# UltronAI/Depth-VO-Feat

Measured on AMD Instinct MI355X. Metric: KITTI 256x832 stereo-seq samples/sec fwd+bwd, higher is better.
Workload: dtype f32

## Files before the change

depth-vo-feat_amd/csrc/conv.hip:

```cpp
#include "dvf_common.h"
#include "conv_op.h"
#include "conv_pipe_host.h"
#include "conv_gather.h"
#include "conv_wgrad.h"
#include "wgrad_pipe.h"

namespace {

__device__ __forceinline__ float act_grad(float g, float yv, int act, float alpha, float beta) {
    if (act == DVF_ACT_RELU) return (yv > 0.f) ? g : 0.f;
    if (act == DVF_ACT_SIGMOID_AFFINE) {
        const float sg = (yv - beta) / alpha;
        return g * alpha * sg * (1.f - sg);
    }
    return g;
}

template <bool VEC>
__global__ __launch_bounds__(256) void act_bwd_kernel(const float *__restrict__ dy, const float *__restrict__ y,
                                                      float *__restrict__ dpre, float *dbias, int C, int HW, int act,
                                                      float alpha, float beta, int chunks, float *part = nullptr, int nper = 0) {
    __shared__ float red[4];
    const int plane = blockIdx.x / chunks, chunk = blockIdx.x - plane * chunks;
    const int c = plane % C;
// ... 117 lines not shown
    }
    return best;
}

struct GatherPlan {
    GatherArgs a;
    int MT, NT, CKH;
    size_t lds;
    dim3 grid;
    int64_t ws_floats;
    bool reduce_kpar;
};

int plan_gather(const ConvOp &op, GatherPlan &pl) {
    const ClassSpec *cls = op.cls;
    const int ncls = op.ncls, Tmax = op.Tmax, TAmax = op.TAmax, TBmax = op.TBmax, OHc = op.OHc, OWc = op.OWc;
    if (ncls < 1 || ncls > 4) return DVF_ERR_INVALID_ARG;
    GatherArgs &a = pl.a;
    a = GatherArgs{};
    for (int s = 0; s < op.nseg; ++s) a.segC[s] = op.segC[s];
    a.nseg = op.nseg; a.w_mode = op.w_mode;
    a.Mtot = op.Mtot; a.Rtot = op.Rtot; a.KK = op.KK; a.m_base = op.m_base; a.M = op.M;
    a.N = op.N; a.IH = op.IH; a.IW = op.IW; a.OH = op.OH; a.OW = op.OW;
    a.act = op.act; a.alpha = op.alpha; a.beta = op.beta;
    a.ncls = ncls; a.OS = cls[0].OS; a.IS = cls[0].IS;
    for (int i = 0, tap0 = 0; i < ncls; ++i) {
        const ClassSpec &c = cls[i];
        const int T = c.TA * c.TB;
        if (tap0 + T > 52) return DVF_ERR_INVALID_ARG;
        a.cls[i] = ClassDev{c.py, c.px, c.by, c.bx, c.TA, c.TB, c.OHc, c.OWc, tap0};
        for (int t = 0; t < T; ++t) a.tapmap[tap0 + t] = c.tapmap[t];
        tap0 += T;
    }
    const int maxBW = ((64 - 1) * cls[0].IS + TBmax > 128) ? 32 : 64;
    const int MT = a.M > 32 ? 2 : 1;
    int NT = 2;
    TilePlan tp = plan_tiles(OHc, OWc, NT, maxBW);
    int64_t nblk = (int64_t)cdiv(OWc, tp.TGX << tp.lsw) * cdiv(OHc, tp.TGY << tp.lsh) * cdiv(a.M, 32 * MT) * a.N * ncls;
    if (nblk < 768) {
        NT = 1;
        tp = plan_tiles(OHc, OWc, NT, maxBW);
        nblk = (int64_t)cdiv(OWc, tp.TGX << tp.lsw) * cdiv(OHc, tp.TGY << tp.lsh) * cdiv(a.M, 32 * MT) * a.N * ncls;
    }
    const int mtiles = cdiv(a.M, 32 * MT);
    a.lsw = tp.lsw; a.lsh = tp.lsh; a.TGX = tp.TGX;
    a.BW = tp.TGX << tp.lsw; a.BH = tp.TGY << tp.lsh;
    if ((a.BW - 1) * a.IS + TBmax > 128) return DVF_ERR_UNSUPPORTED;
    a.tilesX = cdiv(OWc, a.BW);
    a.tilesY = cdiv(OHc, a.BH);
    const int PH = (a.BH - 1) * a.IS + TAmax, PW = (a.BW - 1) * a.IS + TBmax, PWH = (PW + 1) / 2;
    a.PSmax = PH * ((a.IS == 2) ? 2 * PWH : PW);
    a.Tmax = Tmax;
    const int COTP = 32 * MT + 1;
    int maxc = 0;
    for (int s = 0; s < a.nseg; ++s) maxc = a.segC[s] > maxc ? a.segC[s] : maxc;
    auto lds_bytes = [&](int CK) {
        const int WD = (a.w_mode == 0 ? CK : 32 * MT) * a.KK;
        return ((size_t)CK * a.PSmax + (size_t)Tmax * CK * COTP + WD + Tmax + 64) * 4;
    };
    int CK = 16;
    static const size_t g_lds_cap = (dvf_tune("DVF_G_LDS_KB") ? atoi(dvf_tune("DVF_G_LDS_KB")) : 40) * 1024;
    while (CK > 2 && lds_bytes(CK) > g_lds_cap) CK >>= 1;
    while (CK > 2 && CK / 2 >= maxc) CK >>= 1;
    if (lds_bytes(CK) > 64 * 1024) return DVF_ERR_UNSUPPORTED;
    a.WD = (a.w_mode == 0 ? CK : 32 * MT) * a.KK;
    a.NCH = 0;
    for (int s = 0; s < a.nseg; ++s) a.NCH += cdiv(a.segC[s], CK);
    int KS = 1;
    if (nblk < 384) KS = (int)((512 + nblk - 1) / nblk);
    if (KS > a.NCH) KS = a.NCH;
    if (KS < 1) KS = 1;
    if ((int64_t)a.N * KS * ncls > 65535) return DVF_ERR_UNSUPPORTED;
    a.KS = KS;
    for (int s2 = 0; s2 < a.nseg; ++s2)
        if ((int64_t)a.N * a.segC[s2] * a.IH * a.IW * 4 >= ((int64_t)1 << 31) - 16) return DVF_ERR_UNSUPPORTED;
    if ((int64_t)a.Mtot * a.Rtot * a.KK * 4 >= ((int64_t)1 << 31) - 16) return DVF_ERR_UNSUPPORTED;
    pl.MT = MT; pl.NT = NT; pl.CKH = CK / 2; pl.lds = lds_bytes(CK);
    pl.grid = dim3(a.tilesX * a.tilesY, mtiles, a.N * KS * ncls);
    pl.ws_floats = (op.covers && KS > 1) ? (int64_t)KS * a.N * a.M * a.OH * a.OW : 0;
    pl.reduce_kpar = false;
    return DVF_OK;
}

template <int MT, int NT>
int launch_gather_ck(const GatherArgs &a, const GatherPlan &pl, hipStream_t st) {
    switch (pl.CKH) {
        case 1: conv_gather_kernel<MT, NT, 1><<<pl.grid, 256, pl.lds, st>>>(a); break;
        case 2: conv_gather_kernel<MT, NT, 2><<<pl.grid, 256, pl.lds, st>>>(a); break;
        case 4: conv_gather_kernel<MT, NT, 4><<<pl.grid, 256, pl.lds, st>>>(a); break;
        case 8: conv_gather_kernel<MT, NT, 8><<<pl.grid, 256, pl.lds, st>>>(a); break;
        default: return DVF_ERR_UNSUPPORTED;
    }
    DVF_LAUNCH_CHECK();
    return DVF_OK;
}

int run_gather(const ConvOp &op, const GatherPlan &pl, const ConvIO &io, const float *w, float *ws, int64_t ws_floats,
               hipStream_t st) {
    GatherArgs a = pl.a;
    for (int s = 0; s < a.nseg; ++s) a.in[s] = io.in[s];
    a.w = w; a.bias = io.bias; a.mask = io.mask;
    int rc = prepare_output(a, out_mode_of(op.covers, a.KS, ws, ws_floats, pl.ws_floats), io.out, ws, st);
    if (rc) return rc;
    if (const char *e = dvf_tune("DVF_DBG")) a.dbg = atoi(e);
    if (pl.MT == 2 && pl.NT == 2) rc = launch_gather_ck<2, 2>(a, pl, st);
    else if (pl.MT == 2) rc = launch_gather_ck<2, 1>(a, pl, st);
    else if (pl.NT == 2) rc = launch_gather_ck<1, 2>(a, pl, st);
    else rc = launch_gather_ck<1, 1>(a, pl, st);
    if (rc) return rc;
    dvf_plan_note(DVF_K_GATHER, pl.MT, pl.NT, 1, 2 * pl.CKH, 0, a.KS, 1, 1, 256, (int)pl.lds, a.out_mode | (a.ncls << 4));
    return finish_output(a, pl.reduce_kpar, ws, io.out, st);
}

enum FwdDirect { FWD_NONE, FWD_HEAD, FWD_HEAD_WIDE, FWD_DCONVT };
FwdDirect fwd_direct(const dvf_conv_desc *d, int nseg) {
    if (dvf_head_applicable(d, nseg)) return FWD_HEAD;
    if (dvf_head_wide_applicable(d, nseg)) return FWD_HEAD_WIDE;
    if (dvf_dconvt_applicable(d, nseg)) return FWD_DCONVT;
    return FWD_NONE;
}

int fwd_unpacked(const dvf_conv_desc *d, const ConvOp &op, const ConvIO &io, const int *seg_channels, int nseg, const float *w,
                 float *ws, int64_t ws_floats, hipStream_t st) {
    switch (fwd_direct(d, nseg)) {
        case FWD_HEAD: return dvf_head_fwd(d, io.in[0], w, io.bias, io.out, st);
        case FWD_HEAD_WIDE: return dvf_head_fwd_segs(d, io.in, seg_channels, nseg, w, io.bias, io.out, st);
        case FWD_DCONVT: return dvf_dconvt_fwd(d, io.in[0], w, io.bias, io.out, st);
        case FWD_NONE: break;
    }
    GatherPlan pl;
    const int rc = plan_gather(op, pl);
    return rc ? rc : run_gather(op, pl, io, w, ws, ws_floats, st);
}

int dgrad_unpacked(const dvf_conv_desc *d, const ConvOp &op, const ConvIO &io, const float *w, float *ws, int64_t ws_floats,
                   hipStream_t st) {
    if (dvf_head_seg_dgrad_applicable(d, op.M))
        return dvf_head_seg_dgrad(d, io.in[0], w, io.out, op.m_base, op.M, st, io.mask);
    GatherPlan pl;
    const int rc = plan_gather(op, pl);
    return rc ? rc : run_gather(op, pl, io, w, ws, ws_floats, st);
}

int64_t unpacked_ws_floats(const ConvOp &op, bool direct) {
    if (direct) return 0;
    GatherPlan pl;
    const int rc = plan_gather(op, pl);
    return rc ? rc : pl.ws_floats;
}

struct DgradSeg {
    int s, off;
    ConvOp op;
    bool packed;
    PipePlan plan;
    int64_t packed_off;
};

template <class F>
int for_each_dgrad_seg(const dvf_conv_desc *d, const int *seg_channels, int nseg, bool use_pipe, F visit) {
    DgradSeg v;
    v.off = 0; v.packed_off = 0;
    for (v.s = 0; v.s < nseg; ++v.s) {
        int rc = make_dgrad_op(d, v.off, seg_channels[v.s], v.op);
        v.packed = false;
        if (use_pipe) {
            if (rc) return rc;
            rc = plan_pipe(v.op, v.plan);
            if (rc && rc != DVF_ERR_UNSUPPORTED) return rc;
            v.packed = !rc;
        }
        rc = visit(v);
        if (rc) return rc;
        if (v.packed) v.packed_off += v.plan.packed_floats;
        v.off += seg_channels[v.s];
    }
    return DVF_OK;
}

int64_t conv_sizes(const dvf_conv_desc *d, const int *seg_channels, int nseg, int op_kind, bool want_ws) {
    int rc = check_desc(d);
    if (rc) return rc;
    rc = check_segs(d, seg_channels, nseg);
    if (rc) return rc;
    if (op_kind == 0) {
        if (!want_ws && dvf_dconvt_applicable(d, nseg)) return DVF_ERR_UNSUPPORTED;
        ConvOp op;
        PipePlan pl;
        rc = make_fwd_op(d, seg_channels, nseg, op);
        if (rc) return rc;
        rc = plan_pipe(op, pl);
        if (rc == DVF_ERR_UNSUPPORTED && want_ws) return unpacked_ws_floats(op, fwd_direct(d, nseg) != FWD_NONE);
        return rc ? rc : (want_ws ? pl.ws_floats : pl.packed_floats);
    }
    if (op_kind != 1) return DVF_ERR_INVALID_ARG;
    int64_t total = 0, wmax = 0;
    int nsup = 0;
    rc = for_each_dgrad_seg(d, seg_channels, nseg, true, [&](const DgradSeg &v) -> int {
        int64_t wf = 0;
        if (v.packed) {
            total += v.plan.packed_floats;
            wf = v.plan.ws_floats;
            ++nsup;
        } else if (want_ws) {
            wf = unpacked_ws_floats(v.op, dvf_head_seg_dgrad_applicable(d, v.op.M));
            if (wf < 0) return (int)wf;
        }
        wmax = wf > wmax ? wf : wmax;
        return DVF_OK;
    });
    if (rc) return rc;
    if (!nsup && !want_ws) return DVF_ERR_UNSUPPORTED;
    return want_ws ? wmax : total;
}

WgradArgs wgrad_args(const dvf_conv_desc *d, const float *const *in_segs, const int *seg_channels, int s, const float *dpre,
                     float *dw) {
    int off = 0;
    for (int i = 0; i < s; ++i) off += seg_channels[i];
    const int segc = s < 0 ? d->C_in : seg_channels[s];
    WgradArgs a{};
    a.KK = d->KH * d->KW; a.KH = d->KH; a.KW = d->KW; a.N = d->N; a.S = d->stride; a.pad = d->pad; a.G = dw;
    if (!d->transposed) {
        a.P = dpre; a.PCtot = d->C_out; a.m_base = 0; a.M = d->C_out; a.GH = d->H_out; a.GW = d->W_out;
// ... 227 lines not shown
                float beta, int accumulate_dbias, float *ws, int64_t ws_floats, void *stream) {
    if (!dy || (act != DVF_ACT_NONE && !y) || N <= 0 || C <= 0 || HW <= 0) return DVF_ERR_INVALID_ARG;
    if (!dpre && !dbias) return DVF_OK;
    hipStream_t st = dvf_stream(stream);
    if (dbias && !accumulate_dbias && hipMemsetAsync(dbias, 0, sizeof(float) * C, st) != hipSuccess) return DVF_ERR_LAUNCH;
    const bool vec = (HW % 4 == 0) && ((reinterpret_cast<uintptr_t>(dy) | reinterpret_cast<uintptr_t>(y) |
                                        reinterpret_cast<uintptr_t>(dpre)) % 16 == 0);
    const bool sums_only = !dpre && act == DVF_ACT_NONE;
    const int chunks = sums_only ? bias_sum_chunks(N, C, HW) : act_bwd_chunks(N, C, HW, dbias != nullptr);
    const int64_t planes = (int64_t)N * C;
    float *part = (dbias && ws && ws_floats >= dvf_act_bwd_ws_floats(N, C, HW)) ? ws : nullptr;
    if (sums_only) {
        const int per = ((vec ? HW >> 2 : HW) + chunks - 1) / chunks;
        const int threads = per <= 256 ? 64 : per <= 8192 ? 256 : 1024;
        if (vec) bias_sum_kernel<true><<<(unsigned)(planes * chunks), threads, 0, st>>>(dy, dbias, C, HW, chunks, part, N * chunks);
        else bias_sum_kernel<false><<<(unsigned)(planes * chunks), threads, 0, st>>>(dy, dbias, C, HW, chunks, part, N * chunks);
    } else if (vec) act_bwd_kernel<true><<<(unsigned)(planes * chunks), 256, 0, st>>>(dy, y, dpre, dbias, C, HW, act, alpha, beta, chunks, part, N * chunks);
    else act_bwd_kernel<false><<<(unsigned)(planes * chunks), 256, 0, st>>>(dy, y, dpre, dbias, C, HW, act, alpha, beta, chunks, part, N * chunks);
    DVF_LAUNCH_CHECK();
    if (part) {
        bias_finish_kernel<<<C, 64, 0, st>>>(part, dbias, N * chunks);
        DVF_LAUNCH_CHECK();
    }
    return DVF_OK;
}


int64_t dvf_conv2d_packed_floats(const dvf_conv_desc *d, const int *seg_channels, int nseg, int op_kind) {
    return conv_sizes(d, seg_channels, nseg, op_kind, false);
}

int64_t dvf_conv2d_ws_floats(const dvf_conv_desc *d, const int *seg_channels, int nseg, int op_kind) {
    return conv_sizes(d, seg_channels, nseg, op_kind, true);
}

int dvf_conv2d_pack(const dvf_conv_desc *d, const int *seg_channels, int nseg, int op_kind, const float *w, float *packed,
                    void *stream) {
    int rc = check_desc(d);
    if (rc) return rc;
    rc = check_segs(d, seg_channels, nseg);
    if (rc) return rc;
    if (!w || !packed) return DVF_ERR_INVALID_ARG;
    hipStream_t st = dvf_stream(stream);
    if (op_kind == 0) {
        ConvOp op;
        PipePlan pl;
        rc = make_fwd_op(d, seg_channels, nseg, op);
        if (!rc) rc = plan_pipe(op, pl);
        return rc ? rc : launch_pack(op, pl, w, packed, st);
    }
    if (op_kind != 1) return DVF_ERR_INVALID_ARG;
    return for_each_dgrad_seg(d, seg_channels, nseg, true, [&](const DgradSeg &v) -> int {
        return v.packed ? launch_pack(v.op, v.plan, w, packed + v.packed_off, st) : DVF_OK;
    });
}

int dvf_conv2d_fwd(const dvf_conv_desc *d, const float *const *in_segs, const int *seg_channels, int nseg,
                   const float *packed, const float *w, const float *bias, float *out, float *ws, int64_t ws_floats,
                   void *stream) {
    dvf_plan_reset();
    int rc = check_desc(d);
    if (rc) return rc;
    rc = check_segs(d, seg_channels, nseg);
    if (rc) return rc;
    if (!in_segs || !w || !out) return DVF_ERR_INVALID_ARG;
    for (int s = 0; s < nseg; ++s)
        if (!in_segs[s]) return DVF_ERR_INVALID_ARG;
    hipStream_t st = dvf_stream(stream);
    const ConvIO io{in_segs, bias, out, nullptr};
    ConvOp op;
    rc = make_fwd_op(d, seg_channels, nseg, op);
    if (packed && !rc) {
        PipePlan pl;
        rc = plan_pipe(op, pl);
        if (!rc) rc = run_pipe(op, pl, io, packed, ws, ws_floats, st);
        if (rc != DVF_ERR_UNSUPPORTED) return rc;
    }
    return fwd_unpacked(d, op, io, seg_channels, nseg, w, ws, ws_floats, st);
}

int dvf_conv2d_dgrad(const dvf_conv_desc *d, const float *dpre, const float *packed, const float *w, float *const *din_segs,
                     const int *seg_channels, int nseg, float *ws, int64_t ws_floats, const float *const *mask_segs,
                     void *stream) {
    dvf_plan_reset();
    int rc = check_desc(d);
    if (rc) return rc;
    rc = check_segs(d, seg_channels, nseg);
    if (rc) return rc;
    if (!dpre || !w || !din_segs) return DVF_ERR_INVALID_ARG;
    hipStream_t st = dvf_stream(stream);
    auto mask = [&](int s) -> const float * { return mask_segs ? mask_segs[s] : nullptr; };
    if (dvf_head_dgrad_applicable(d, nseg) || (dvf_head_applicable(d, nseg) && !packed))
        return din_segs[0] ? dvf_head_dgrad(d, dpre, w, din_segs[0], st, mask(0)) : DVF_OK;
    return for_each_dgrad_seg(d, seg_channels, nseg, packed != nullptr, [&](const DgradSeg &v) -> int {
        if (!din_segs[v.s]) return DVF_OK;
        const ConvIO io{&dpre, nullptr, din_segs[v.s], mask(v.s)};
        int r = v.packed ? run_pipe(v.op, v.plan, io, packed + v.packed_off, ws, ws_floats, st) : DVF_ERR_UNSUPPORTED;
        if (r == DVF_ERR_UNSUPPORTED) r = dgrad_unpacked(d, v.op, io, w, ws, ws_floats, st);
        return r;
    });
}

int dvf_conv2d_pack_jobs(const dvf_conv_desc *d, const int *seg_channels, int nseg, int op_kind, const float *w, float *packed,
                         void *jobs_host, int max_jobs, int *blocks_out, int *lds_bytes_out) {
    static_assert(sizeof(PackArgs) <= DVF_PACK_JOB_BYTES, "DVF_PACK_JOB_BYTES too small");
    int rc = check_desc(d);
    if (rc) return rc;
    rc = check_segs(d, seg_channels, nseg);
    if (rc) return rc;
    if (!w || !packed || !jobs_host || !blocks_out || max_jobs < 1) return DVF_ERR_INVALID_ARG;
    char *out = static_cast<char *>(jobs_host);
    int njobs = 0;
    auto emit = [&](const ConvOp &op, const PipePlan &pl, float *dst) {
        const PackArgs job = pack_job(op, pl, w, dst, &blocks_out[njobs]);
        memset(out + (size_t)njobs * DVF_PACK_JOB_BYTES, 0, DVF_PACK_JOB_BYTES);
        memcpy(out + (size_t)njobs * DVF_PACK_JOB_BYTES, &job, sizeof(job));
        if (lds_bytes_out && (int)pl.pack_lds > *lds_bytes_out) *lds_bytes_out = (int)pl.pack_lds;
        ++njobs;
    };
    if (op_kind == 0) {
        ConvOp op;
        PipePlan pl;
        rc = make_fwd_op(d, seg_channels, nseg, op);
        if (!rc) rc = plan_pipe(op, pl);
        if (rc) return rc;
        emit(op, pl, packed);
        return njobs;
    }
    if (op_kind != 1) return DVF_ERR_INVALID_ARG;
    rc = for_each_dgrad_seg(d, seg_channels, nseg, true, [&](const DgradSeg &v) -> int {
        if (njobs >= max_jobs) return DVF_ERR_INVALID_ARG;
        if (v.packed) emit(v.op, v.plan, packed + v.packed_off);
        return DVF_OK;
    });
    return rc ? rc : njobs;
}

int dvf_conv2d_pack_batch(const void *jobs_dev, const int *block_prefix_dev, const int *block_job_dev, int njobs,
                          int total_blocks, int lds_bytes, void *stream) {
    if (!jobs_dev || !block_prefix_dev || njobs < 1 || total_blocks < 1 || lds_bytes < 4 || lds_bytes > 64 * 1024)
        return DVF_ERR_INVALID_ARG;
    static_assert(DVF_PACK_JOB_BYTES % alignof(PackArgs) == 0, "job stride");
    static_assert(sizeof(PackArgs) == DVF_PACK_JOB_BYTES, "job stride");
    conv_pack_batch_kernel<<<total_blocks, 256, lds_bytes, dvf_stream(stream)>>>(
        static_cast<const PackArgs *>(jobs_dev), block_prefix_dev, block_job_dev, njobs);
    DVF_LAUNCH_CHECK();
    return DVF_OK;
}

#ifdef DVF_TUNING
int dvf_tuning_read_stamps(unsigned long long *out, int max_blocks) {
    if (!out || !g_stamp_buf) return 0;
    const int nb = g_stamp_blocks < max_blocks ? g_stamp_blocks : max_blocks;
    if (hipDeviceSynchronize() != hipSuccess) return DVF_ERR_LAUNCH;
    if (hipMemcpy(out, g_stamp_buf, (size_t)nb * 64, hipMemcpyDeviceToHost) != hipSuccess) return DVF_ERR_LAUNCH;
    return nb;
}
#endif

}
```

depth-vo-feat_amd/csrc/conv_epilogue.h:

```cpp
#pragma once
#include "dvf_common.h"

namespace dvfp {

typedef float f32x16 __attribute__((ext_vector_type(16)));

enum OutMode {
    OUT_FUSED = 0,
    OUT_ATOMIC = 1,
    OUT_WS = 2
};

template <int ACT>
__device__ __forceinline__ float apply_act(float t, float alpha, float beta) {
    if constexpr (ACT == DVF_ACT_RELU) return fmaxf(t, 0.f);
    else if constexpr (ACT == DVF_ACT_SIGMOID_AFFINE) return alpha * (1.f / (1.f + expf(-t))) + beta;
    else return t;
}
__device__ __forceinline__ float apply_act(float v, int act, float alpha, float beta) {
    if (act == DVF_ACT_RELU) return apply_act<DVF_ACT_RELU>(v, alpha, beta);
    if (act == DVF_ACT_SIGMOID_AFFINE) return apply_act<DVF_ACT_SIGMOID_AFFINE>(v, alpha, beta);
    return v;
}

template <int MT, int NT, class Pix, class Bias>
__device__ __forceinline__ void store_tile(const f32x16 (&acc)[MT][NT], float *out, const float *mask, int out_mode, int act,
                                           float alpha, float beta, int m0, int kh, int M, int64_t HW, Pix pix, Bias bias_at) {
    auto store_all = [&](auto modec, auto actc, auto fullc) __attribute__((always_inline)) {
        constexpr int MODE = decltype(modec)::value, ACT = decltype(actc)::value;
        constexpr bool FULL = decltype(fullc)::value;
        float bv[MT][16];
        if constexpr (MODE == 0) {
#pragma unroll
            for (int m = 0; m < MT; ++m)
#pragma unroll
                for (int r = 0; r < 16; ++r) bv[m][r] = bias_at(m * 32 + (r & 3) + 8 * (r >> 2));
        }
#pragma unroll
        for (int i = 0; i < NT; ++i) {
            int64_t off;
            const bool pok = pix(i, off);
            float *pbase = out + off;
            float mk[MT][16];
            if constexpr (MODE == 3) {
#pragma unroll
                for (int m = 0; m < MT; ++m)
#pragma unroll
                    for (int r = 0; r < 16; ++r) {
                        const int ml = m * 32 + (r & 3) + 8 * (r >> 2);
                        const bool ok = pok && (FULL || m0 + 4 * kh + ml < M);
                        mk[m][r] = mask[ok ? off + (int64_t)ml * HW : 0];
                    }
            }
            if (pok) {
#pragma unroll
                for (int m = 0; m < MT; ++m) {
#pragma unroll
                    for (int r = 0; r < 16; ++r) {
                        const int ml = m * 32 + (r & 3) + 8 * (r >> 2);
                        if (FULL || m0 + 4 * kh + ml < M) {
                            float *op = pbase + (int64_t)ml * HW;
                            const float v = acc[m][i][r];
                            if constexpr (MODE == 3) *op = mk[m][r] > 0.f ? v : 0.f;
                            else if constexpr (MODE == 0) *op = apply_act<ACT>(v + bv[m][r], alpha, beta);
                            else if constexpr (MODE == 1) atomicAdd(op, v);
                            else *op = v;
                        }
                    }
                }
            }
        }
    };
    using std::integral_constant;
    auto by_full = [&](auto modec, auto actc) __attribute__((always_inline)) {
        if (m0 + 32 * MT <= M) store_all(modec, actc, std::true_type{});
        else store_all(modec, actc, std::false_type{});
    };
    if (out_mode == OUT_FUSED && mask) by_full(integral_constant<int, 3>{}, integral_constant<int, DVF_ACT_NONE>{});
    else if (out_mode == OUT_WS) by_full(integral_constant<int, 2>{}, integral_constant<int, DVF_ACT_NONE>{});
    else if (out_mode == OUT_ATOMIC) by_full(integral_constant<int, 1>{}, integral_constant<int, DVF_ACT_NONE>{});
    else if (act == DVF_ACT_RELU) by_full(integral_constant<int, 0>{}, integral_constant<int, DVF_ACT_RELU>{});
    else if (act == DVF_ACT_SIGMOID_AFFINE) by_full(integral_constant<int, 0>{}, integral_constant<int, DVF_ACT_SIGMOID_AFFINE>{});
    else by_full(integral_constant<int, 0>{}, integral_constant<int, DVF_ACT_NONE>{});
}

}
```

depth-vo-feat_amd/csrc/conv_gather.h:

```cpp
#pragma once
#include "dvf_common.h"
#include "conv_pipe.h"

namespace {

using dvfp::f32x16;
using dvfp::tensor_rsrc;
using dvfp::OOB;
using dvfp::bload;
using dvfp::store_tile;

struct ClassDev { int py, px, by, bx, TA, TB, OHc, OWc, tap0; };

struct GatherArgs {
    const float *in[DVF_MAX_SEGS];
    int segC[DVF_MAX_SEGS];
    int nseg;
    const float *w;
    int w_mode;
    int Mtot, Rtot, KK, m_base, M;
    const float *bias;
    float *out;
    int N, IH, IW, OH, OW;
    int OS, IS;
    int ncls;
    ClassDev cls[4];
    int act;
    float alpha, beta;
    int KS, NCH, out_mode, dbg;
    int64_t ws_slice;
    int lsw, lsh, TGX, BW, BH, tilesX, tilesY;
    int PSmax, Tmax, WD;
    int tapmap[52];
    const float *mask;
};

template <int MT, int NT, int CKH>
__global__ __launch_bounds__(256) void conv_gather_kernel(const GatherArgs a) {
    constexpr int CK = 2 * CKH, COTP = 32 * MT + 1;
    extern __shared__ __attribute__((aligned(16))) float smem[];
    float *patch = smem;
    float *wl = smem + CK * a.PSmax;
    int *wdec = reinterpret_cast<int *>(wl + a.Tmax * CK * COTP);
    int *tapB = wdec + a.WD;
    int *inv = tapB + a.Tmax;
    const int tid = threadIdx.x, lane = tid & 63, nl = lane & 31, kh = lane >> 5;
    const int wave = __builtin_amdgcn_readfirstlane(tid >> 6);
    const int zc = blockIdx.z % a.ncls, zr = blockIdx.z / a.ncls;
    const int n = zr / a.KS, ks = zr - n * a.KS;
    const ClassDev c = a.cls[zc];
    const int tX = blockIdx.x % a.tilesX, tY = blockIdx.x / a.tilesX;
    const int oy0 = tY * a.BH, ox0 = tX * a.BW;
    if (oy0 >= c.OHc || ox0 >= c.OWc) return;
    const int m0 = blockIdx.y * (32 * MT);
    const int SW = 1 << a.lsw, SH = 1 << a.lsh;
    const int pxl = nl & (SW - 1), pyl = nl >> a.lsw;
    const int T = c.TA * c.TB;
    const int PH = (a.BH - 1) * a.IS + c.TA, PW = (a.BW - 1) * a.IS + c.TB, PWH = (PW + 1) >> 1;
    const int RS = (a.IS == 2) ? 2 * PWH : PW, PS = PH * RS;

    for (int e = tid; e < 64; e += 256) inv[e] = -1;
    __syncthreads();
    for (int t = tid; t < T; t += 256) {
        inv[a.tapmap[c.tap0 + t]] = t;
        const int ta = t / c.TB, tb = t - ta * c.TB;
        tapB[t] = ta * RS + ((a.IS == 2) ? ((tb & 1) * PWH + (tb >> 1)) : tb);
    }
    __syncthreads();
    {
        const int nE = (a.w_mode == 0 ? CK : 32 * MT) * a.KK;
        for (int e = tid; e < nE; e += 256) {
            const int hi = e / a.KK, t = inv[e - hi * a.KK];
            int d = -1;
            if (t >= 0) d = (hi << 24) | (a.w_mode == 0 ? (t * CK + hi) * COTP : t * CK * COTP + hi);
            wdec[e] = d;
        }
    }

    int boff[NT], opy[NT], opx[NT];
#pragma unroll
    for (int i = 0; i < NT; ++i) {
        const int q = wave * NT + i, tx = q % a.TGX, ty = q / a.TGX;
        opy[i] = ty * SH + pyl;
        opx[i] = tx * SW + pxl;
        boff[i] = kh * PS + (opy[i] * a.IS) * RS + opx[i];
    }
    f32x16 acc[MT][NT];
#pragma unroll
    for (int m = 0; m < MT; ++m)
#pragma unroll
        for (int i = 0; i < NT; ++i)
#pragma unroll
            for (int r = 0; r < 16; ++r) acc[m][i][r] = 0.f;

    const int iy0 = oy0 * a.IS + c.by, ix0 = ox0 * a.IS + c.bx;
    const bool npass2 = PW > 64;
    unsigned pcol_off[2];
    int pcol_dst[2];
#pragma unroll
    for (int ps = 0; ps < 2; ++ps) {
        const int cc = lane + 64 * ps, ix = ix0 + cc;
        pcol_off[ps] = (cc < PW && ix >= 0 && ix < a.IW) ? ((unsigned)ix << 2) : OOB;
        pcol_dst[ps] = (cc < PW) ? ((a.IS == 2) ? ((cc & 1) * PWH + (cc >> 1)) : cc) : -1;
    }
    const __amdgpu_buffer_rsrc_t rs_w = tensor_rsrc(a.w);
    const int g_begin = (int)(((int64_t)a.NCH * ks) / a.KS), g_end = (int)(((int64_t)a.NCH * (ks + 1)) / a.KS);
    int seg = 0, seg_first = 0, r_seg = 0;
    for (int g = g_begin; g < g_end; ++g) {
        while (true) {
            const int nchs = (a.segC[seg] + CK - 1) / CK;
            if (g < seg_first + nchs) break;
            seg_first += nchs;
            r_seg += a.segC[seg];
            ++seg;
        }
        const int c0 = (g - seg_first) * CK;
        const int nch = min(CK, a.segC[seg] - c0);
        __syncthreads();
        if (!DVF_DBG(a, 1)) {
            const __amdgpu_buffer_rsrc_t rs_in = tensor_rsrc(a.in[seg]);
// ... 44 lines not shown
                        const bool mok = m0 + m < a.M;
                        v[k] = bload(rs_w, mok ? voff : OOB, mok ? wb + (unsigned)m * rowstep : 0u);
                    }
                    if (use) {
#pragma unroll
                        for (int k = 0; k < 8 * MT; ++k) wl[off + wave + 4 * k] = v[k];
                    }
                }
            } else {
                const int nE = 32 * MT * a.KK;
                const unsigned wb = (unsigned)((r0 * a.Mtot + a.m_base + m0) * a.KK) << 2;
                const unsigned rowstep = (unsigned)(a.Mtot * a.KK) << 2;
                constexpr int RK = (CK + 3) / 4;
                for (int e0 = lane; e0 < nE; e0 += 256) {
                    int d[4];
                    float v[4][RK];
#pragma unroll
                    for (int jj = 0; jj < 4; ++jj) {
                        const int e = e0 + 64 * jj;
                        d[jj] = (e < nE) ? wdec[e] : -1;
                    }
#pragma unroll
                    for (int jj = 0; jj < 4; ++jj) {
                        const int e = e0 + 64 * jj;
                        const unsigned voff = ((d[jj] >= 0) && (m0 + (d[jj] >> 24) < a.M)) ? ((unsigned)e << 2) : OOB;
#pragma unroll
                        for (int k = 0; k < RK; ++k) {
                            const int rr = wave + 4 * k;
                            const bool rok = rr < nch;
                            v[jj][k] = bload(rs_w, rok ? voff : OOB, rok ? wb + (unsigned)rr * rowstep : 0u);
                        }
                    }
#pragma unroll
                    for (int jj = 0; jj < 4; ++jj) {
                        if (d[jj] < 0) continue;
#pragma unroll
                        for (int k = 0; k < RK; ++k) {
                            const int rr = wave + 4 * k;
                            if (rr < CK) wl[(d[jj] & 0xFFFFFF) + rr * COTP] = v[jj][k];
                        }
                    }
                }
            }
        }
        __syncthreads();
        if (!DVF_DBG(a, 4)) {
            float af[2][CKH][MT], bf[2][CKH][NT];
            auto load = [&](auto bufc, int t) {
                constexpr int buf = decltype(bufc)::value;
                const int tb_off = tapB[t];
                const int wo = (t * CK + kh) * COTP + nl;
#pragma unroll
                for (int cp = 0; cp < CKH; ++cp) {
#pragma unroll
                    for (int m = 0; m < MT; ++m) af[buf][cp][m] = wl[wo + cp * 2 * COTP + m * 32];
#pragma unroll
                    for (int i = 0; i < NT; ++i) bf[buf][cp][i] = patch[boff[i] + tb_off + cp * 2 * PS];
                }
            };
            auto mma = [&](auto bufc) {
                constexpr int buf = decltype(bufc)::value;
#pragma unroll
                for (int cp = 0; cp < CKH; ++cp)
#pragma unroll
                    for (int m = 0; m < MT; ++m)
#pragma unroll
                        for (int i = 0; i < NT; ++i)
                            acc[m][i] = __builtin_amdgcn_mfma_f32_32x32x2f32(af[buf][cp][m], bf[buf][cp][i], acc[m][i], 0, 0, 0);
            };
            using B0 = std::integral_constant<int, 0>;
            using B1 = std::integral_constant<int, 1>;
            load(B0{}, 0);
            for (int t = 0; t < T; t += 2) {
                if (t + 1 < T) load(B1{}, t + 1);
                mma(B0{});
                if (t + 1 < T) {
                    if (t + 2 < T) load(B0{}, t + 2);
                    mma(B1{});
                }
            }
        }
    }
    const int64_t HWo = (int64_t)a.OH * a.OW;
    store_tile<MT, NT>(
        acc, a.out + (a.out_mode == dvfp::OUT_WS ? (int64_t)ks * a.ws_slice : 0), a.mask, a.out_mode, a.act, a.alpha, a.beta, m0, kh, a.M, HWo,
        [&](int i, int64_t &off) __attribute__((always_inline)) {
            const int oy = oy0 + opy[i], ox = ox0 + opx[i];
            const int Y = oy * a.OS + c.py, X = ox * a.OS + c.px;
            off = ((int64_t)n * a.M + m0 + 4 * kh) * HWo + (int64_t)Y * a.OW + X;
            return (oy < c.OHc) && (ox < c.OWc) && (Y < a.OH) && (X < a.OW);
        },
        [&](int ml) __attribute__((always_inline)) {
            const int mm = m0 + ml + 4 * kh;
            return (a.bias && mm < a.M) ? a.bias[mm] : 0.f;
        });
}

}
```

depth-vo-feat_amd/csrc/conv_head.h:

```cpp
#pragma once
#include "dvf_common.h"
bool dvf_head_applicable(const dvf_conv_desc *d, int nseg);
bool dvf_head_fwd_applicable(const dvf_conv_desc *d, int nseg);
bool dvf_head_dgrad_applicable(const dvf_conv_desc *d, int nseg);
int dvf_head_fwd(const dvf_conv_desc *d, const float *in, const float *w, const float *bias, float *out, hipStream_t st);
bool dvf_head_wide_applicable(const dvf_conv_desc *d, int nseg);
int dvf_head_fwd_segs(const dvf_conv_desc *d, const float *const *in_segs, const int *seg_channels, int nseg, const float *w,
                      const float *bias, float *out, hipStream_t st);
int dvf_head_dgrad(const dvf_conv_desc *d, const float *dpre, const float *w, float *din, hipStream_t st, const float *mask = nullptr);
int dvf_head_wgrad(const dvf_conv_desc *d, const float *in, const float *dpre, float *dw, int accumulate, hipStream_t st,
                   float *ws = nullptr, int64_t ws_floats = 0);
int64_t dvf_head_wgrad_ws_floats(const dvf_conv_desc *d);
bool dvf_head_seg_dgrad_applicable(const dvf_conv_desc *d, int segc);
int dvf_head_seg_dgrad(const dvf_conv_desc *d, const float *dpre, const float *w, float *din, int seg_off, int segc,
                       hipStream_t st, const float *mask = nullptr);
bool dvf_dconvt_applicable(const dvf_conv_desc *d, int nseg);
int dvf_dconvt_fwd(const dvf_conv_desc *d, const float *in, const float *w, const float *bias, float *out, hipStream_t st);
```

depth-vo-feat_amd/csrc/conv_head.hip:

```cpp
#include "conv_head.h"
#include "conv_epilogue.h"

namespace {

using dvfp::apply_act;

constexpr int HT_W = 64, HT_H = 4;
constexpr int HP_W = HT_W + 2, HP_H = HT_H + 2;
constexpr int HCK = 8;

__device__ __forceinline__ void stage_tile(float *lds, const float *__restrict__ src, int64_t plane, int nch, int H, int W,
                                           int y0, int x0) {
    for (int e = threadIdx.x; e < nch * HP_H * HP_W; e += 256) {
        const int ch = e / (HP_H * HP_W), r = e - ch * (HP_H * HP_W), py = r / HP_W, px = r - py * HP_W;
        const int y = y0 + py - 1, x = x0 + px - 1;
        lds[e] = (y >= 0 && y < H && x >= 0 && x < W) ? src[ch * plane + (int64_t)y * W + x] : 0.f;
    }
}

template <int ROWS, int MO, class WK>
__device__ __forceinline__ void taps9(const float (&v)[ROWS + 2][3], WK wk, float (&acc)[ROWS][MO]) {
#pragma unroll
    for (int m = 0; m < MO; ++m)
#pragma unroll
        for (int k = 0; k < 9; ++k) {
            const float w = wk(m, k);
#pragma unroll
            for (int r = 0; r < ROWS; ++r) acc[r][m] = fmaf(w, v[k / 3 + r][k % 3], acc[r][m]);
        }
}

constexpr int FT_H = 8;
constexpr int HEAD_MAX_SEGS = 3;
struct HeadSegs {
    const float *p[HEAD_MAX_SEGS];
    int c[HEAD_MAX_SEGS];
    int n;
};
template <int MO, int HCKT, int FTH>
__global__ __launch_bounds__(256) void head_fwd_kernel(const HeadSegs in, const float *__restrict__ w,
                                                       const float *__restrict__ bias, float *__restrict__ out, int C, int H,
                                                       int W, int tilesX, int act, float alpha, float beta, int ws_m, int ws_c,
                                                       int flip, const float *__restrict__ mask) {
    constexpr int ROWS = FTH / 4, FPH = FTH + 2, FPN = FPH * HP_W, FLD = (FPN + 255) / 256;
    extern __shared__ __attribute__((aligned(16))) float wsh[];
    float *tile = wsh + ((MO * C * 9 + 3) & ~3);
    for (int e = threadIdx.x; e < MO * C * 9; e += 256) {
        const int m = e / (C * 9), r = e - m * (C * 9), c = r / 9, k = r - c * 9;
        const float wv = w[(int64_t)m * ws_m + (int64_t)c * ws_c + (flip ? 8 - k : k)];
        if (MO == 16) wsh[(c * MO + m) * 9 + k] = wv;
        else wsh[e] = wv;
    }
    const int n = blockIdx.y, tY = blockIdx.x / tilesX, tX = blockIdx.x - tY * tilesX;
    const int y0 = tY * FTH, x0 = tX * HT_W;
    const int lx = threadIdx.x & (HT_W - 1), ly = (threadIdx.x >> 6) * ROWS;
    const int64_t plane = (int64_t)H * W;
    int soff[FLD];
#pragma unroll
    for (int i = 0; i < FLD; ++i) {
        const int e = threadIdx.x + 256 * i, py = e / HP_W, px = e - py * HP_W;
        const int y = y0 + py - 1, x = x0 + px - 1;
        soff[i] = (e < FPN && y >= 0 && y < H && x >= 0 && x < W) ? y * W + x : -1;
    }
    float acc[ROWS][MO];
#pragma unroll
    for (int m = 0; m < MO; ++m)
#pragma unroll
        for (int r = 0; r < ROWS; ++r) acc[r][m] = bias ? bias[m] : 0.f;
    float stg[HCKT][FLD];
    static_assert(HEAD_MAX_SEGS == 3, "segment select below");
    auto seg_ptr = [&](int sg) { return sg == 0 ? in.p[0] : sg == 1 ? in.p[1] : in.p[2]; };
    auto seg_ch = [&](int sg) { return sg == 0 ? in.c[0] : sg == 1 ? in.c[1] : in.c[2]; };
    auto issue = [&](int sg, int cs) {
        const int sc = seg_ch(sg), nch = min(HCKT, sc - cs);
        const float *src = seg_ptr(sg) + ((int64_t)n * sc + cs) * plane;
#pragma unroll
        for (int ch = 0; ch < HCKT; ++ch)
#pragma unroll
            for (int i = 0; i < FLD; ++i) stg[ch][i] = (ch < nch && soff[i] >= 0) ? src[ch * plane + soff[i]] : 0.f;
    };
    issue(0, 0);
    int sg = 0, cs = 0, cg = 0;
    while (sg < in.n) {
        const int nch = min(HCKT, seg_ch(sg) - cs);
        int sg2 = sg, cs2 = cs + HCKT;
        if (cs2 >= seg_ch(sg)) { ++sg2; cs2 = 0; }
        __syncthreads();
#pragma unroll
        for (int ch = 0; ch < HCKT; ++ch)
#pragma unroll
            for (int i = 0; i < FLD; ++i) {
                const int e = threadIdx.x + 256 * i;
                if (e < FPN) tile[ch * FPN + e] = stg[ch][i];
            }
        __syncthreads();
        if (sg2 < in.n) issue(sg2, cs2);
        auto hood = [&](int ch, float (&v)[ROWS + 2][3]) __attribute__((always_inline)) {
            const float *t = tile + ch * FPN + ly * HP_W + lx;
#pragma unroll
            for (int a = 0; a < ROWS + 2; ++a)
#pragma unroll
                for (int b = 0; b < 3; ++b) v[a][b] = t[a * HP_W + b];
        };
        if constexpr (MO != 16) {
            auto wlds = [&](int c) __attribute__((always_inline)) {
                return [=](int m, int k) __attribute__((always_inline)) { return wsh[(m * C + c) * 9 + k]; };
            };
            float part[3][ROWS][MO];
#pragma unroll
            for (int q = 0; q < 3; ++q)
#pragma unroll
                for (int r = 0; r < ROWS; ++r)
#pragma unroll
                    for (int m = 0; m < MO; ++m) part[q][r][m] = 0.f;
            int ch = 0;
            for (; ch + 4 <= nch; ch += 4) {
                float v4[4][ROWS + 2][3];
#pragma unroll
                for (int q = 0; q < 4; ++q) hood(ch + q, v4[q]);
#pragma unroll
                for (int q = 0; q < 4; ++q)
#pragma unroll
                    for (int m = 0; m < MO; ++m) {
                        const float *wm = wsh + (m * C + cg + ch + q) * 9;
#pragma unroll
                        for (int k = 0; k < 9; ++k) {
                            const float wk = wm[k];
#pragma unroll
                            for (int r = 0; r < ROWS; ++r) {
                                if (q == 0) acc[r][m] = fmaf(wk, v4[q][k / 3 + r][k % 3], acc[r][m]);
                                else part[q - 1][r][m] = fmaf(wk, v4[q][k / 3 + r][k % 3], part[q - 1][r][m]);
                            }
                        }
                    }
            }
            for (; ch < nch; ++ch) {
                float v[ROWS + 2][3];
                hood(ch, v);
                taps9<ROWS, MO>(v, wlds(cg + ch), acc);
            }
#pragma unroll
            for (int r = 0; r < ROWS; ++r)
#pragma unroll
                for (int m = 0; m < MO; ++m) acc[r][m] += (part[0][r][m] + part[1][r][m]) + part[2][r][m];
        } else {
            for (int ch = 0; ch < nch; ++ch) {
                float v[ROWS + 2][3];
                hood(ch, v);
                typedef float f4h __attribute__((ext_vector_type(4)));
                const f4h *wq = reinterpret_cast<const f4h *>(wsh + (cg + ch) * (MO * 9));
                f4h wr[MO * 9 / 4];
#pragma unroll
                for (int q = 0; q < MO * 9 / 4; ++q) wr[q] = wq[q];
                taps9<ROWS, MO>(v, [&](int m, int k) __attribute__((always_inline)) { return wr[(m * 9 + k) >> 2][(m * 9 + k) & 3]; }, acc);
            }
        }
        cg += nch; sg = sg2; cs = cs2;
    }
    const int x = x0 + lx;
#pragma unroll
    for (int r = 0; r < ROWS; ++r) {
        const int y = y0 + ly + r;
        if (y < H && x < W) {
            if (mask) {
#pragma unroll
                for (int m = 0; m < MO; ++m) {
                    const int64_t idx = ((int64_t)n * MO + m) * plane + (int64_t)y * W + x;
                    out[idx] = mask[idx] > 0.f ? acc[r][m] : 0.f;
                }
            } else {
#pragma unroll
                for (int m = 0; m < MO; ++m)
                    out[((int64_t)n * MO + m) * plane + (int64_t)y * W + x] = apply_act(acc[r][m], act, alpha, beta);
            }
        }
    }
}

template <int MO>
__global__ __launch_bounds__(256) void head_dgrad_kernel(const float *__restrict__ dpre, const float *__restrict__ w,
                                                         float *__restrict__ din, int C, int H, int W, int tilesX,
                                                         const float *__restrict__ mask) {
    __shared__ float tile[MO * HP_H * HP_W];
    extern __shared__ __attribute__((aligned(16))) float wsh[];
    constexpr int WPC = (MO * 9 + 3) & ~3;
    for (int e = threadIdx.x; e < C * MO * 9; e += 256) {
        const int c = e / (MO * 9), r = e - c * (MO * 9), m = r / 9, k = r - m * 9;
        wsh[c * WPC + r] = w[((int64_t)m * C + c) * 9 + k];
    }
    const int n = blockIdx.y, tY = blockIdx.x / tilesX, tX = blockIdx.x - tY * tilesX;
    const int y0 = tY * HT_H, x0 = tX * HT_W;
    const int lx = threadIdx.x & (HT_W - 1), ly = threadIdx.x >> 6;
    const int64_t plane = (int64_t)H * W;
    stage_tile(tile, dpre + (int64_t)n * MO * plane, plane, MO, H, W, y0, x0);
    __syncthreads();
    float g[MO][9];
#pragma unroll
    for (int m = 0; m < MO; ++m)
#pragma unroll
        for (int a = 0; a < 3; ++a)
#pragma unroll
            for (int b = 0; b < 3; ++b) g[m][a * 3 + b] = tile[m * (HP_H * HP_W) + (ly + 2 - a) * HP_W + (lx + 2 - b)];
    const int y = y0 + ly, x = x0 + lx;
    if (y >= H || x >= W) return;
    const int64_t base = (int64_t)n * C * plane + (int64_t)y * W + x;
    float *dst = din + base;
    const float *mk = mask ? mask + base : nullptr;
    for (int c0 = 0; c0 < C; c0 += 4) {
        float sv[4], mv[4];
#pragma unroll
        for (int q = 0; q < 4; ++q) {
            const int c = min(c0 + q, C - 1);
            mv[q] = mk ? mk[c * plane] : 1.f;
            const float *wc = wsh + c * WPC;
            float s = 0.f;
#pragma unroll
            for (int m = 0; m < MO; ++m)
#pragma unroll
                for (int k = 0; k < 9; ++k) s = fmaf(wc[m * 9 + k], g[m][k], s);
            sv[q] = s;
        }
#pragma unroll
        for (int q = 0; q < 4; ++q)
            if (c0 + q < C) dst[(c0 + q) * plane] = (mv[q] > 0.f) ? sv[q] : 0.f;
    }
}

template <bool VEC>
__device__ __forceinline__ void hw_load4(const float *__restrict__ p, int x0, int W, bool ok, float (&v)[4]) {
    if (VEC) {
        typedef float f4 __attribute__((ext_vector_type(4)));
        f4 t = {0.f, 0.f, 0.f, 0.f};
        if (ok) t = *reinterpret_cast<const f4 *>(p);
#pragma unroll
        for (int j = 0; j < 4; ++j) v[j] = t[j];
    } else {
#pragma unroll
        for (int j = 0; j < 4; ++j) v[j] = (ok && x0 + j < W) ? p[j] : 0.f;
    }
}

template <int MO, int CCH, bool VEC>
__global__ __launch_bounds__(256) void head_wgrad_kernel(const float *__restrict__ in, const float *__restrict__ dpre,
                                                         float *dw, int C, int H, int W, int RS, int xgroups, int segs,
                                                         int64_t units, float *part = nullptr) {
    constexpr int A = CCH * 9 * MO;
    __shared__ float red[4 * A];
    const int c0 = blockIdx.x * CCH;
    const int64_t plane = (int64_t)H * W;
    const int upi = segs * xgroups;
    float acc[CCH][9][MO];
#pragma unroll
    for (int c = 0; c < CCH; ++c)
#pragma unroll
        for (int t = 0; t < 9; ++t)
#pragma unroll
            for (int m = 0; m < MO; ++m) acc[c][t][m] = 0.f;
    for (int64_t ub = blockIdx.y; ub * 256 < units; ub += gridDim.y) {
        const int64_t u = ub * 256 + threadIdx.x;
        const bool live = u < units;
        const int n = live ? (int)(u / upi) : 0, q = live ? (int)(u - (int64_t)n * upi) : 0;
        const int seg = q / xgroups, xg = q - seg * xgroups;
        const int y0 = seg * RS, y1 = min(H, y0 + RS), x0 = xg * 4;
        const float *ip = in + ((int64_t)n * C + c0) * plane + x0;
        const float *dp = dpre + (int64_t)n * MO * plane + x0;
        const bool lok = x0 > 0, rok = x0 + 4 < W;
        auto load_in = [&](int r, float (&x)[CCH][6]) __attribute__((always_inline)) {
            const bool ok = live && r >= 0 && r < H;
            const int64_t ro = (int64_t)r * W;
#pragma unroll
            for (int c = 0; c < CCH; ++c) {
                const bool okc = ok && c0 + c < C;
                const float *p = ip + c * plane + ro;
                float v[4];
                hw_load4<VEC>(p, x0, W, okc, v);
                x[c][0] = (okc && lok) ? p[-1] : 0.f;
#pragma unroll
                for (int j = 0; j < 4; ++j) x[c][1 + j] = v[j];
                x[c][5] = (okc && rok) ? p[4] : 0.f;
            }
        };
        auto load_dp = [&](int y, float (&g)[MO][4]) __attribute__((always_inline)) {
            const bool ok = live && y >= y0 && y < y1;
#pragma unroll
            for (int m = 0; m < MO; ++m) hw_load4<VEC>(dp + m * plane + (int64_t)y * W, x0, W, ok, g[m]);
        };
        float d[3][MO][4], dn[MO][4], xc[CCH][6], xn[CCH][6];
#pragma unroll
        for (int m = 0; m < MO; ++m)
#pragma unroll
            for (int j = 0; j < 4; ++j) d[0][m][j] = d[1][m][j] = 0.f;
        load_dp(y0, d[2]);
        load_in(y0 - 1, xc);
        for (int i = 0; i < RS + 2; ++i) {
            const int r = y0 - 1 + i;
            load_in(i + 1 < RS + 2 ? r + 1 : H, xn);
            load_dp(r + 2, dn);
#pragma unroll
            for (int c = 0; c < CCH; ++c)
#pragma unroll
                for (int ta = 0; ta < 3; ++ta)
#pragma unroll
                    for (int tb = 0; tb < 3; ++tb)
#pragma unroll
                        for (int m = 0; m < MO; ++m)
#pragma unroll
                            for (int j = 0; j < 4; ++j)
// ... 78 lines not shown
            for (int a = 0; a < K; ++a) {
                const int dy = (a + 1) & 1;
                const int ry = 1 + ((dy + 1 - a) >> 1);
#pragma unroll
                for (int b = 0; b < K; ++b) {
                    const int dx = (b + 1) & 1;
                    const int rx = 1 + ((dx + 1 - b) >> 1);
                    const int f = co * K * K + a * K + b;
                    acc[dy][dx][co] = fmaf(wq[f >> 2][f & 3], v[ry][rx], acc[dy][dx][co]);
                }
            }
        }
        ip += plane;
    }
    if (!inside) return;
    const int64_t oplane = (int64_t)OH * OW;
    float *op = out + (int64_t)n * CO * oplane;
#pragma unroll
    for (int dy = 0; dy < 2; ++dy) {
        const int Y = 2 * y + dy;
        if (Y >= OH) continue;
        const int X = 2 * x;
#pragma unroll
        for (int co = 0; co < CO; ++co) {
            float r0 = apply_act(acc[dy][0][co], act, alpha, beta), r1 = apply_act(acc[dy][1][co], act, alpha, beta);
            float *q = op + co * oplane + (int64_t)Y * OW + X;
            if (X + 1 < OW && (OW & 1) == 0) {
                typedef float f2 __attribute__((ext_vector_type(2)));
                f2 t; t.x = r0; t.y = r1;
                *reinterpret_cast<f2 *>(q) = t;
            } else {
                if (X < OW) q[0] = r0;
                if (X + 1 < OW) q[1] = r1;
            }
        }
    }
}

}

bool dvf_head_applicable(const dvf_conv_desc *d, int nseg) {
    return nseg == 1 && !d->transposed && d->KH == 3 && d->KW == 3 && d->stride == 1 && d->pad == 1 && d->C_out >= 1 &&
           d->C_out <= 4 && d->H_out == d->H_in && d->W_out == d->W_in && d->C_in >= 4 && d->C_in * d->C_out <= 1024 &&
           dvf_tune("DVF_NO_HEAD") == nullptr;
}
bool dvf_head_fwd_applicable(const dvf_conv_desc *d, int nseg) {
    static const int maxc = dvf_tune("DVF_HEAD_FWD_MAXC") ? atoi(dvf_tune("DVF_HEAD_FWD_MAXC")) : 127;
    return dvf_head_applicable(d, nseg) && d->C_in <= maxc;
}
bool dvf_head_dgrad_applicable(const dvf_conv_desc *d, int nseg) {
    static const int maxc = dvf_tune("DVF_HEAD_DGRAD_MAXC") ? atoi(dvf_tune("DVF_HEAD_DGRAD_MAXC")) : 32;
    return dvf_head_applicable(d, nseg) && d->C_in <= maxc;
}

bool dvf_dconvt_applicable(const dvf_conv_desc *d, int nseg) {
    const bool k3 = d->KH == 3 && d->KW == 3, k4 = d->KH == 4 && d->KW == 4;
    return nseg == 1 && d->transposed && d->stride == 2 && d->pad == 1 && (k3 || k4) && d->C_out == 16 &&
           d->C_in >= 8 && d->C_in <= 64 && d->H_out <= 2 * d->H_in && d->W_out <= 2 * d->W_in &&
           (int64_t)d->H_in * d->W_in >= 64 * 64 && (int64_t)d->N * d->C_out * d->H_out * d->W_out < ((int64_t)1 << 31) &&
           dvf_tune("DVF_NO_DCONVT") == nullptr;
}

int dvf_dconvt_fwd(const dvf_conv_desc *d, const float *in, const float *w, const float *bias, float *out, hipStream_t st) {
    const dim3 grid(cdiv(d->W_in, 64), cdiv(d->H_in, 4), d->N);
    const size_t lds = (size_t)d->C_in * d->C_out * d->KH * d->KW * 4;
    if ((reinterpret_cast<uintptr_t>(w) & 15) != 0 || lds > 64 * 1024) return DVF_ERR_UNSUPPORTED;
#define DCONVT(CO, K) dconvt_s2_fwd_kernel<CO, K><<<grid, 256, lds, st>>>(in, w, bias, out, d->C_in, d->H_in, d->W_in, d->H_out, d->W_out, d->act, d->alpha, d->beta)
    if (d->KH == 3) DCONVT(16, 3);
    else DCONVT(16, 4);
#undef DCONVT
    DVF_LAUNCH_CHECK();
    dvf_plan_note(DVF_K_DCONVT_FWD, d->C_out, d->KH);
    return DVF_OK;
}

#define HEAD_CASE(N, ...) case N: { constexpr int MO = N; __VA_ARGS__; } break;
#define HEAD_DISPATCH(MOV, CALL, ...)             \
    switch (MOV) {                               \
        HEAD_CASE(1, CALL) HEAD_CASE(2, CALL) HEAD_CASE(3, CALL) HEAD_CASE(4, CALL) __VA_ARGS__ \
        default: return DVF_ERR_UNSUPPORTED;     \
    }

static int head_fwd_launch(int MOv, const HeadSegs &in, const float *w, const float *bias, float *out, int C, int N, int H, int W,
                           int act, float alpha, float beta, int ws_m, int ws_c, int flip, const float *mask, hipStream_t st) {
    const bool lowres = (int64_t)N * H * W <= (int64_t)4 * 64 * 208 && MOv <= 4 && C >= 32;
    const int FTH = lowres ? 4 : FT_H, HCKT = lowres ? 32 : HCK;
    const int tilesX = cdiv(W, HT_W), tilesY = cdiv(H, FTH);
    const dim3 grid(tilesX * tilesY, N);
    const size_t lds = ((size_t)((MOv * C * 9 + 3) & ~3) + (size_t)HCKT * (FTH + 2) * HP_W) * 4;
#define HEAD_FWD_GO(HC, FH) head_fwd_kernel<MO, HC, FH><<<grid, 256, lds, st>>>(in, w, bias, out, C, H, W, tilesX, act, alpha, beta, ws_m, ws_c, flip, mask)
    if (lowres) {
        static bool big[5] = {false, false, false, false, false};
        HEAD_DISPATCH(MOv, {
            if (lds > 64 * 1024 && !big[MO]) {
                if (hipFuncSetAttribute(reinterpret_cast<const void *>(&head_fwd_kernel<MO, 32, 4>), hipFuncAttributeMaxDynamicSharedMemorySize, 160 * 1024) != hipSuccess) return DVF_ERR_LAUNCH;
                big[MO] = true;
            }
            HEAD_FWD_GO(32, 4); });
    } else {
        HEAD_DISPATCH(MOv, (HEAD_FWD_GO(8, 8)), HEAD_CASE(16, (HEAD_FWD_GO(8, 8))));
    }
#undef HEAD_FWD_GO
    DVF_LAUNCH_CHECK();
    return DVF_OK;
}

int dvf_head_fwd(const dvf_conv_desc *d, const float *in, const float *w, const float *bias, float *out, hipStream_t st) {
    const int one = d->C_in;
    return dvf_head_fwd_segs(d, &in, &one, 1, w, bias, out, st);
}

bool dvf_head_wide_applicable(const dvf_conv_desc *d, int nseg) {
    return nseg >= 1 && nseg <= HEAD_MAX_SEGS && !d->transposed && d->KH == 3 && d->KW == 3 && d->stride == 1 && d->pad == 1 &&
           d->C_out == 16 && d->C_in <= 24 && d->H_out == d->H_in && d->W_out == d->W_in &&
           (int64_t)d->H_in * d->W_in >= 64 * 64 && dvf_tune("DVF_NO_HEAD") == nullptr && dvf_tune("DVF_NO_WIDE_HEAD") == nullptr;
}

int dvf_head_fwd_segs(const dvf_conv_desc *d, const float *const *in_segs, const int *seg_channels, int nseg, const float *w,
                      const float *bias, float *out, hipStream_t st) {
    HeadSegs in{};
    for (int s = 0; s < HEAD_MAX_SEGS; ++s) { in.p[s] = s < nseg ? in_segs[s] : in_segs[0]; in.c[s] = s < nseg ? seg_channels[s] : 0; }
    in.n = nseg;
    const int rc = head_fwd_launch(d->C_out, in, w, bias, out, d->C_in, d->N, d->H_in, d->W_in, d->act, d->alpha, d->beta,
                                   d->C_in * 9, 9, 0, nullptr, st);
    if (rc) return rc;
    dvf_plan_note(DVF_K_HEAD_FWD, d->C_out, nseg);
    return DVF_OK;
}

bool dvf_head_seg_dgrad_applicable(const dvf_conv_desc *d, int segc) {
    const bool narrow = segc >= 1 && segc <= 4 && d->C_out >= 4 && d->C_out * segc <= 1024;
    const bool wide = segc == 16 && d->C_out <= 24 && (int64_t)d->H_in * d->W_in >= 64 * 64 &&
                      dvf_tune("DVF_NO_WIDE_HEAD") == nullptr;
    return !d->transposed && d->KH == 3 && d->KW == 3 && d->stride == 1 && d->pad == 1 && (narrow || wide) &&
           d->H_out == d->H_in && d->W_out == d->W_in && dvf_tune("DVF_NO_HEAD") == nullptr;
}

int dvf_head_seg_dgrad(const dvf_conv_desc *d, const float *dpre, const float *w, float *din, int seg_off, int segc,
                       hipStream_t st, const float *mask) {
    const float *wseg = w + (int64_t)seg_off * 9;
    HeadSegs in{};
    for (int s = 0; s < HEAD_MAX_SEGS; ++s) { in.p[s] = dpre; in.c[s] = s == 0 ? d->C_out : 0; }
    in.n = 1;
    const int rc = head_fwd_launch(segc, in, wseg, nullptr, din, d->C_out, d->N, d->H_in, d->W_in, DVF_ACT_NONE, 1.f, 0.f, 9,
                                   d->C_in * 9, 1, mask, st);
    if (rc) return rc;
    dvf_plan_note(DVF_K_HEAD_SEG_DGRAD, segc);
    return DVF_OK;
}

int dvf_head_dgrad(const dvf_conv_desc *d, const float *dpre, const float *w, float *din, hipStream_t st, const float *mask) {
    const int tilesX = cdiv(d->W_in, HT_W), tilesY = cdiv(d->H_in, HT_H);
    const dim3 grid(tilesX * tilesY, d->N);
    HEAD_DISPATCH(d->C_out, (head_dgrad_kernel<MO><<<grid, 256, (size_t)d->C_in * ((MO * 9 + 3) & ~3) * 4, st>>>(
                                dpre, w, din, d->C_in, d->H_in, d->W_in, tilesX, mask)));
    DVF_LAUNCH_CHECK();
    dvf_plan_note(DVF_K_HEAD_DGRAD, d->C_out);
    return DVF_OK;
}

struct HeadWgradGrid { int cch, RS, xgroups, segs, chunks, groups; int64_t units; };
static HeadWgradGrid head_wgrad_grid(const dvf_conv_desc *d) {
    HeadWgradGrid g;
    g.xgroups = cdiv(d->W_in, 4);
    auto blocks = [&](int cch, int rs) {
        return (int64_t)cdiv(d->C_in, cch) * (((int64_t)d->N * cdiv(d->H_in, rs) * g.xgroups + 255) / 256);
    };
    const int min_blocks = 400, max_blocks = 1024;
    g.cch = (d->C_out <= 2 && blocks(4, 8) >= 512) ? 4 : 2;
    g.RS = 8;
    if (const char *t = dvf_tune("DVF_HEAD_WG_CCH")) g.cch = (atoi(t) == 4 && d->C_out <= 2) ? 4 : 2;
    while (g.RS > 2 && blocks(g.cch, g.RS) < min_blocks) g.RS >>= 1;
    if (const char *t = dvf_tune("DVF_HEAD_WG_RS")) g.RS = atoi(t) > 0 ? atoi(t) : g.RS;
    g.segs = cdiv(d->H_in, g.RS);
    g.units = (int64_t)d->N * g.segs * g.xgroups;
    g.chunks = cdiv(d->C_in, g.cch);
    const int64_t nub = (g.units + 255) / 256;
    int64_t groups = max_blocks / g.chunks;
    if (groups < 1) groups = 1;
    if (groups > nub) groups = nub;
    g.groups = (int)groups;
    return g;
}

int64_t dvf_head_wgrad_ws_floats(const dvf_conv_desc *d) {
    return (int64_t)head_wgrad_grid(d).groups * d->C_out * d->C_in * 9;
}

int dvf_head_wgrad(const dvf_conv_desc *d, const float *in, const float *dpre, float *dw, int accumulate, hipStream_t st,
                   float *ws, int64_t ws_floats) {
    if (!accumulate && hipMemsetAsync(dw, 0, sizeof(float) * (size_t)d->C_out * d->C_in * 9, st) != hipSuccess)
        return DVF_ERR_LAUNCH;
    const HeadWgradGrid g = head_wgrad_grid(d);
    const dim3 grid(g.chunks, g.groups);
    float *part = (ws && ws_floats >= dvf_head_wgrad_ws_floats(d)) ? ws : nullptr;
    const bool vec = d->W_in % 4 == 0 && ((reinterpret_cast<uintptr_t>(in) | reinterpret_cast<uintptr_t>(dpre)) & 15) == 0;
#define HEAD_WGRAD_GO(CCH, VEC) head_wgrad_kernel<MO, CCH, VEC><<<grid, 256, 0, st>>>(in, dpre, dw, d->C_in, d->H_in, d->W_in, g.RS, g.xgroups, g.segs, g.units, part)
    HEAD_DISPATCH(d->C_out, {
        if (MO <= 2 && g.cch == 4) { if (vec) HEAD_WGRAD_GO((MO <= 2 ? 4 : 2), true); else HEAD_WGRAD_GO((MO <= 2 ? 4 : 2), false); }
        else { if (vec) HEAD_WGRAD_GO(2, true); else HEAD_WGRAD_GO(2, false); } });
#undef HEAD_WGRAD_GO
    DVF_LAUNCH_CHECK();
    if (part) {
        const int n = d->C_out * d->C_in * 9;
        head_wgrad_finish_kernel<<<(n + 255) / 256, 256, 0, st>>>(part, dw, n, g.groups);
        DVF_LAUNCH_CHECK();
    }
    dvf_plan_note(DVF_K_HEAD_WGRAD, d->C_out, part ? 1 : 0);
    return DVF_OK;
}
```

depth-vo-feat_amd/csrc/conv_op.h:

```cpp
#pragma once
#include "dvf_common.h"
#include "conv_head.h"

namespace {

inline int ilog2(int v) { int l = 0; while ((1 << l) < v) ++l; return l; }
inline int roundup(int v, int q) { return (v + q - 1) / q * q; }

struct ClassSpec { int OS, py, px, IS, by, bx, TA, TB, OHc, OWc; int tapmap[49]; };

struct ConvOp {
    int nseg, segC[DVF_MAX_SEGS];
    int w_mode;
    int Mtot, Rtot, KK, m_base, M;
    int N, IH, IW, OH, OW;
    int act;
    float alpha, beta;
    ClassSpec cls[4];
    int ncls;
    bool covers;
    int Tmax, TAmax, TBmax, OHc, OWc;
    bool head_fwd;
};

struct ConvIO {
    const float *const *in;
    const float *bias;
    float *out;
    const float *mask;
};

int check_desc(const dvf_conv_desc *d) {
    if (!d) return DVF_ERR_INVALID_ARG;
    if (d->N <= 0 || d->C_in <= 0 || d->C_out <= 0 || d->H_in <= 0 || d->W_in <= 0 || d->H_out <= 0 || d->W_out <= 0)
        return DVF_ERR_INVALID_ARG;
    if (d->KH < 1 || d->KW < 1 || d->KH > 7 || d->KW > 7 || (d->stride != 1 && d->stride != 2) || d->pad < 0)
        return DVF_ERR_INVALID_ARG;
    return DVF_OK;
}

int check_segs(const dvf_conv_desc *d, const int *seg_channels, int nseg) {
    if (nseg < 1 || nseg > DVF_MAX_SEGS || !seg_channels) return DVF_ERR_INVALID_ARG;
    int tot = 0;
    for (int s = 0; s < nseg; ++s) {
        if (seg_channels[s] <= 0) return DVF_ERR_INVALID_ARG;
        tot += seg_channels[s];
    }
    return tot == d->C_in ? DVF_OK : DVF_ERR_INVALID_ARG;
}

int class_taps(int c, int S, int pad, int K, int *taps, int *base) {
    int amax = -1;
    for (int a = K - 1; a >= 0; --a)
        if ((c + pad - a) % S == 0) { amax = a; break; }
    if (amax < 0) { *base = 0; return 0; }
    int cnt = 0;
    for (int a = amax; a >= 0; a -= S) taps[cnt++] = a;
    *base = (c + pad - amax) / S;
    return cnt;
}

int scatter_classes(int S, int pad, int KH, int KW, int OH, int OW, ClassSpec *cls, bool *covers_all) {
    int n = 0;
    *covers_all = true;
    for (int cy = 0; cy < S; ++cy)
        for (int cx = 0; cx < S; ++cx) {
            int ta[7], tb[7], by, bx;
            const int na = class_taps(cy, S, pad, KH, ta, &by), nb = class_taps(cx, S, pad, KW, tb, &bx);
            const int OHc = (OH - cy + S - 1) / S, OWc = (OW - cx + S - 1) / S;
            if (OHc <= 0 || OWc <= 0) continue;
            if (na == 0 || nb == 0) { *covers_all = false; continue; }
            ClassSpec &c = cls[n++];
            c = ClassSpec{S, cy, cx, 1, by, bx, na, nb, OHc, OWc, {0}};
            for (int i = 0; i < na; ++i)
                for (int j = 0; j < nb; ++j) c.tapmap[i * nb + j] = ta[i] * KW + tb[j];
        }
    for (int i = 1; i < n; ++i)
        for (int j = i; j > 0 && cls[j].TA * cls[j].TB > cls[j - 1].TA * cls[j - 1].TB; --j) {
            const ClassSpec t = cls[j]; cls[j] = cls[j - 1]; cls[j - 1] = t;
        }
    return n;
}

int set_classes(const dvf_conv_desc *d, bool gather, ConvOp &op) {
    if (gather) {
        op.ncls = 1; op.covers = true;
        op.cls[0] = ClassSpec{1, 0, 0, d->stride, -d->pad, -d->pad, d->KH, d->KW, op.OH, op.OW, {0}};
        for (int t = 0; t < op.KK; ++t) op.cls[0].tapmap[t] = t;
    } else {
        op.ncls = scatter_classes(d->stride, d->pad, d->KH, d->KW, op.OH, op.OW, op.cls, &op.covers);
    }
    op.Tmax = op.TAmax = op.TBmax = op.OHc = op.OWc = 0;
    for (int i = 0; i < op.ncls; ++i) {
        const ClassSpec &c = op.cls[i];
        op.Tmax = max(op.Tmax, c.TA * c.TB); op.TAmax = max(op.TAmax, c.TA); op.TBmax = max(op.TBmax, c.TB);
        op.OHc = max(op.OHc, c.OHc); op.OWc = max(op.OWc, c.OWc);
    }
    return op.ncls >= 1 ? DVF_OK : DVF_ERR_UNSUPPORTED;
}

int make_fwd_op(const dvf_conv_desc *d, const int *seg_channels, int nseg, ConvOp &op) {
    op = ConvOp{};
    for (int s = 0; s < nseg; ++s) op.segC[s] = seg_channels[s];
    op.nseg = nseg; op.M = d->C_out;
    op.N = d->N; op.IH = d->H_in; op.IW = d->W_in; op.OH = d->H_out; op.OW = d->W_out;
    op.act = d->act; op.alpha = d->alpha; op.beta = d->beta;
    op.KK = d->KH * d->KW; op.m_base = 0; op.Mtot = d->C_out; op.Rtot = d->C_in;
    op.head_fwd = !dvf_head_fwd_applicable(d, nseg) && dvf_head_applicable(d, nseg);
    op.w_mode = d->transposed ? 1 : 0;
    return set_classes(d, !d->transposed, op);
}

// ... 13 lines not shown
```

depth-vo-feat_amd/csrc/conv_pipe.h:

```cpp
#pragma once
#include "dvf_common.h"
#include "conv_epilogue.h"

namespace dvfp {

#ifdef DVF_TUNING
#define DVF_STAMP(a, var) do { if ((a).stamps) asm volatile("s_memtime %0\n\ts_waitcnt lgkmcnt(0)" : "=s"(var) :: "memory"); } while (0)
#define DVF_STAMP_RT(a, var) do { if ((a).stamps) asm volatile("s_memrealtime %0\n\ts_waitcnt lgkmcnt(0)" : "=s"(var) :: "memory"); } while (0)
#define DVF_STAMPS_ON 1
#else
#define DVF_STAMP(a, var) do { } while (0)
#define DVF_STAMP_RT(a, var) do { } while (0)
#define DVF_STAMPS_ON 0
#endif

typedef __attribute__((address_space(3))) void lds_void_t;

__device__ __forceinline__ __amdgpu_buffer_rsrc_t tensor_rsrc(const void *p) {
    const uint64_t v = reinterpret_cast<uint64_t>(p);
    const unsigned lo = __builtin_amdgcn_readfirstlane((unsigned)v), hi = __builtin_amdgcn_readfirstlane((unsigned)(v >> 32));
    return __builtin_amdgcn_make_buffer_rsrc(reinterpret_cast<void *>(((uint64_t)hi << 32) | lo), 0, 0x7FFFFFF0, 0x00020000);
}
constexpr unsigned OOB = 0x80000000u;
__device__ __forceinline__ float bload(__amdgpu_buffer_rsrc_t r, unsigned voff, unsigned soff) {
    return __builtin_bit_cast(float, __builtin_amdgcn_raw_buffer_load_b32(r, voff, soff, 0));
}

struct PClass { int py, px, by, bx, TA, TB, OHc, OWc, SL, NTG; unsigned wp_off; };

struct PipeArgs {
    const float *in[DVF_MAX_SEGS];
    int segC[DVF_MAX_SEGS];
    int nseg;
    const float *wp;
    const float *bias;
    float *out;
    int M, N, IH, IW, OH, OW;
    int OS, IS, ncls;
    PClass cls[4];
    int act;
    float alpha, beta;
    int KS, NCH, out_mode, NG;
    int64_t ws_slice;
    int lsw, lsh, TGX, TGY, BW, BH, BN, tilesX, tilesY;
    int x4;
    int blk;
    int SLmax, PSRmax, NST;
    int dbg;
    unsigned long long *stamps;
    const float *mask;
};

__host__ __device__ inline int pipe_row_stride(int RSu, int SW, int SH, int IS) {
    if (SH == 1 || SW >= 32 || (SW % IS) != 0) return RSu;
    const int mod = 32 / IS, want = (SW / IS) % mod;
    const int padded = RSu + ((want - RSu % mod) + mod) % mod;
    return (padded * 8 <= RSu * 9) ? padded : RSu;
}

struct PipeGeo { int PH, PW, PWH, RS, PSR, NPI, XA; };
__host__ __device__ inline PipeGeo pipe_geo(int BH, int BW, int BN, int IS, int TA, int TB, int SW, int SH, int x4 = 0, int bx = 0) {
    PipeGeo g;
    g.PH = (BH - 1) * IS + TA;
    g.PW = (BW - 1) * IS + TB;
    g.PWH = (g.PW + 1) >> 1;
    g.XA = 0;
    if (x4) {
        g.XA = ((bx % 4) + 4) % 4;
        int rs = (g.XA + g.PW + 3) & ~3;
        if (SH > 1 && SW < 32 && (SW & 3) == 0) {
            int padded = rs;
            while (((padded * IS) & 31) != ((SW * IS) & 31) && padded < rs + 32) padded += 4;
            if (((padded * IS) & 31) == ((SW * IS) & 31) && padded * 8 <= rs * 9) rs = padded;
        }
        g.RS = rs;
        g.PSR = (BN * g.PH * g.RS + 255) & ~255;
        g.NPI = g.PSR >> 8;
        return g;
    }
    g.RS = pipe_row_stride(IS == 2 ? 2 * g.PWH : g.PW, SW, SH, IS);
    g.PSR = (BN * g.PH * g.RS + 63) & ~63;
    g.NPI = g.PSR >> 6;
    return g;
}

template <int V> struct fvec;
template <> struct fvec<1> { typedef float type; };
template <> struct fvec<2> { typedef float type __attribute__((ext_vector_type(2))); };
template <> struct fvec<4> { typedef float type __attribute__((ext_vector_type(4))); };

constexpr int PIPE_THREADS = 384;
constexpr int PIPE_THREADS_4P = 512;
constexpr int PIPE_MAXNPI = 32;

template <int MT, int NT, int WM, int CKH, int TBU, int BLK = 0>
__global__ __launch_bounds__(PIPE_THREADS_4P) void conv_pipe_kernel(const PipeArgs a) {
    constexpr int CK = 2 * CKH, VW = CKH >= 4 ? 4 : CKH, CPG = CKH / VW, MTW = MT * WM;
    constexpr int UNITF = TBU * MTW * 64 * VW;
    typedef typename fvec<VW>::type avec;
    extern __shared__ __attribute__((aligned(16))) float smem[];
    const int stage_floats = a.SLmax + CK * a.PSRmax;
    const int tid = threadIdx.x, lane = tid & 63, nl = lane & 31, kh = lane >> 5;
    const int wave = __builtin_amdgcn_readfirstlane(tid >> 6);
    const int zper = gridDim.z / a.ncls;
    const int zc = blockIdx.z / zper, zr = blockIdx.z - zc * zper;
    const int ng = zr / a.KS, ks = zr - ng * a.KS;
    const PClass c = a.cls[zc];
    const int tX = blockIdx.x % a.tilesX, tY = blockIdx.x / a.tilesX;
    const int oy0 = tY * a.BH, ox0 = tX * a.BW, n0 = ng * a.BN;
    if (oy0 >= c.OHc || ox0 >= c.OWc) return;
    const int mb = blockIdx.y;
    const int SW = 1 << a.lsw, SH = 1 << a.lsh;
    const PipeGeo geo = pipe_geo(a.BH, a.BW, a.BN, a.IS, c.TA, TBU, SW, SH, a.x4, c.bx);
    const int RS = geo.RS, PSR = geo.PSR, PWH = geo.PWH;
    const int g_begin = (int)(((int64_t)a.NCH * ks) / a.KS), g_end = (int)(((int64_t)a.NCH * (ks + 1)) / a.KS);
    unsigned long long t_entry = 0, r_entry = 0;
    const int lin_block = (blockIdx.z * gridDim.y + blockIdx.y) * gridDim.x + blockIdx.x;
    DVF_STAMP(a, t_entry);
    DVF_STAMP_RT(a, r_entry);

    if (wave >= 4) {
        auto U = [](int v) __attribute__((always_inline)) { return __builtin_amdgcn_readfirstlane(v); };
        __builtin_amdgcn_s_setprio(3);
        const int nprod = U((int)(blockDim.x >> 6) - 4), pidx = wave - 4;
        const int par = U(nprod == 2 ? pidx : (pidx >> 1));
        const int half = U(nprod == 2 ? 0 : (pidx & 1)), nhalf = U(nprod == 2 ? 1 : 2);
        const int NWP = U(c.SL >> 8);
        const int iy0 = U(oy0 * a.IS + c.by), ix0 = U(ox0 * a.IS + c.bx);
        const int sfl = U(stage_floats), PSRu = U(PSR), NPIu = U(geo.NPI), SLu = U(c.SL), SLmaxu = U(a.SLmax);
        const unsigned wbase = (unsigned)U((int)(c.wp_off + (unsigned)(mb * a.NCH) * (unsigned)c.SL));
        const __amdgpu_buffer_rsrc_t rs_w = tensor_rsrc(a.wp);
        auto issue_w = [&](int g, int st) __attribute__((always_inline)) {
            if (DVF_DBG(a, 2)) return;
            float *wl = smem + st * sfl;
            unsigned so = ((wbase + (unsigned)g * (unsigned)SLu) << 2) + ((unsigned)half << 10);
            float *dst = wl + (half << 8);
            for (int p = half; p < NWP; p += nhalf) {
                __builtin_amdgcn_raw_ptr_buffer_load_lds(rs_w, (lds_void_t *)dst, 16, (unsigned)lane << 4, so, 0, 0);
                so += (unsigned)nhalf << 10;
                dst += nhalf << 8;
            }
        };
        const int D = U(a.NST - 1), nchunks = U(g_end - g_begin), g0 = U(g_begin);
        auto stage_of = [&](int x) __attribute__((always_inline)) { return D == 1 ? (x & 1) : x % 3; };
        if DVF_DBG(a, 8) return;
        for (int x = 0; x < D; ++x)
            if (x < nchunks && (x & 1) == par) issue_w(g0 + x, stage_of(x));

        unsigned pvf[PIPE_MAXNPI];
        unsigned pbn4[PIPE_MAXNPI / 4];
#pragma unroll
        for (int q = 0; q < PIPE_MAXNPI / 4; ++q) pbn4[q] = 0u;
        {
            const int per_img = geo.PH * RS;
            const float inv_img = 1.0f / (float)per_img, inv_rs = 1.0f / (float)RS;
#pragma unroll
            for (int kk = 0; kk < PIPE_MAXNPI; ++kk) {
                pvf[kk] = OOB;
                if (kk < NPIu) {
                    const int p = a.x4 ? (((kk << 6) + lane) << 2) : ((kk << 6) + lane);
                    int bn = (int)((float)p * inv_img);
                    bn += (p - bn * per_img >= per_img) - (p - bn * per_img < 0);
                    const int rem = p - bn * per_img;
                    int row = (int)((float)rem * inv_rs);
                    row += (rem - row * RS >= RS) - (rem - row * RS < 0);
                    const int col = rem - row * RS;
                    int cs = col - geo.XA;
                    bool ok = (bn < a.BN) && (n0 + bn < a.N);
                    if (a.IS == 2 && !a.x4) {
                        cs = col < PWH ? 2 * col : 2 * (col - PWH) + 1;
                        ok = ok && (col < 2 * PWH);
                    }
                    if (!a.x4) ok = ok && (cs < geo.PW);
                    const int iy = iy0 + row, ix = ix0 + cs;
                    ok = ok && (iy >= 0) && (iy < a.IH) && (ix >= 0) && (ix < a.IW);
                    pvf[kk] = ok ? (unsigned)((iy * a.IW + ix) << 2) : OOB;
                    pbn4[kk >> 2] |= (ok ? (unsigned)bn : 0u) << ((kk & 3) * 8);
                }
// ... 209 lines not shown
                if constexpr (u == 0) { load_bj(nbufc, std::integral_constant<int, 2>{}); __builtin_amdgcn_sched_barrier(0); }
            }
            if constexpr (VW > 3) {
                mma_j(bufc, TP{}, uc, std::integral_constant<int, 3>{});
                __builtin_amdgcn_sched_barrier(0);
                if constexpr (u == 0) { load_bj(nbufc, std::integral_constant<int, 3>{}); __builtin_amdgcn_sched_barrier(0); }
            }
        };
        auto unit = [&](auto bufc, auto nbufc, auto pbc) {
            step(bufc, nbufc, pbc, std::integral_constant<int, 0>{});
            if constexpr (TBE > 1) step(bufc, nbufc, pbc, std::integral_constant<int, 1>{});
            if constexpr (TBE > 2) step(bufc, nbufc, pbc, std::integral_constant<int, 2>{});
            if constexpr (TBE > 3) step(bufc, nbufc, pbc, std::integral_constant<int, 3>{});
            if constexpr (TBE > 4) step(bufc, nbufc, pbc, std::integral_constant<int, 4>{});
            if constexpr (TBE > 5) step(bufc, nbufc, pbc, std::integral_constant<int, 5>{});
            if constexpr (TBE > 6) step(bufc, nbufc, pbc, std::integral_constant<int, 6>{});
            advance();
        };
        load_b(B0{});
        load_a(B0{}, 0, std::integral_constant<int, 0>{});
        advance();
        __builtin_amdgcn_sched_barrier(0);
        for (int k = 0; k < NU; k += 2) {
            unit(B0{}, B1{}, std::integral_constant<int, 0>{});
            if (k + 1 < NU) unit(B1{}, B0{}, std::integral_constant<int, TBE & 1>{});
        }
    };

    unsigned long long t_loop0 = 0, t_loop1 = 0, tb0 = 0, tb1 = 0, w_bar = 0;
    DVF_STAMP(a, t_loop0);
    if (!DVF_DBG(a, 8)) {
        int st = 0, since = 0;
        for (int g = g_begin; g < g_end; ++g) {
            DVF_STAMP(a, tb0);
            __syncthreads();
            DVF_STAMP(a, tb1);
            w_bar += tb1 - tb0;
            if (!DVF_DBG(a, 4)) {
                using TBfull = std::integral_constant<int, TBU>;
                using TBless = std::integral_constant<int, (TBU > 1 ? TBU - 1 : 1)>;
                if (a.IS == 2 && !a.x4) consume(st, std::integral_constant<int, 2>{}, TBfull{});
                else if (TBU > 1 && c.TB == TBU - 1 && !DVF_DBG(a, 64)) consume(st, std::integral_constant<int, 1>{}, TBless{});
                else consume(st, std::integral_constant<int, 1>{}, TBfull{});
            }
            if constexpr (BLK) {
                if (++since == a.blk) {
                    since = 0;
#pragma unroll
                    for (int m = 0; m < MT; ++m)
#pragma unroll
                        for (int i = 0; i < NT; ++i) {
                            asum[m][i] += acc[m][i];
#pragma unroll
                            for (int r = 0; r < 16; ++r) acc[m][i][r] = 0.f;
                        }
                }
            }
            st = (st + 1 == a.NST) ? 0 : st + 1;
        }
    }
    if constexpr (BLK) {
#pragma unroll
        for (int m = 0; m < MT; ++m)
#pragma unroll
            for (int i = 0; i < NT; ++i) acc[m][i] += asum[m][i];
    }

    DVF_STAMP(a, t_loop1);
    auto stamp_out = [&]() {
        if (DVF_STAMPS_ON && a.stamps && wave == 0) {
            unsigned long long t_end = 0, r_end = 0;
            asm volatile("s_waitcnt vmcnt(0)" ::: "memory");
            DVF_STAMP(a, t_end);
            DVF_STAMP_RT(a, r_end);
            if (lane == 0) {
                unsigned long long *o = a.stamps + 8 * lin_block;
                o[0] = t_loop0 - t_entry; o[1] = t_loop1 - t_loop0; o[2] = w_bar; o[3] = t_end - t_loop1; o[4] = r_end - r_entry;
            }
        }
    };
    if DVF_DBG(a, 16) { stamp_out(); return; }
    const int m0 = mb * (32 * MTW) + wm * (32 * MT);
    const int64_t HW = (int64_t)a.OH * a.OW;
    if (a.mask && a.out_mode == OUT_FUSED) {
        float *outp = a.out;
#pragma unroll
        for (int i = 0; i < NT; ++i) {
            const int oy = oy0 + opy[i], ox = ox0 + opx[i], n = n0 + opn[i];
            const int Y = oy * a.OS + c.py, X = ox * a.OS + c.px;
            const bool pok = (oy < c.OHc) && (ox < c.OWc) && (Y < a.OH) && (X < a.OW) && (opn[i] < a.BN) && (n < a.N);
            const int64_t base = ((int64_t)n * a.M + m0 + 4 * kh) * HW + (int64_t)Y * a.OW + X;
            float mk[MT][16];
#pragma unroll
            for (int m = 0; m < MT; ++m)
#pragma unroll
                for (int r = 0; r < 16; ++r) {
                    const int ml = m * 32 + (r & 3) + 8 * (r >> 2);
                    const bool ok = pok && (m0 + 4 * kh + ml < a.M);
                    mk[m][r] = a.mask[ok ? base + (int64_t)ml * HW : 0];
                }
#pragma unroll
            for (int m = 0; m < MT; ++m) {
#pragma unroll
                for (int r = 0; r < 16; ++r) {
                    const int ml = m * 32 + (r & 3) + 8 * (r >> 2);
                    if (pok && m0 + 4 * kh + ml < a.M) {
                        outp[base + (int64_t)ml * HW] = mk[m][r] > 0.f ? acc[m][i][r] : 0.f;
                    }
                }
            }
        }
        stamp_out();
        return;
    }
    store_tile<MT, NT>(
        acc, a.out + (a.out_mode == OUT_WS ? (int64_t)ks * a.ws_slice : 0), nullptr, a.out_mode, a.act, a.alpha, a.beta, m0, kh, a.M, HW,
        [&](int i, int64_t &off) __attribute__((always_inline)) {
            const int oy = oy0 + opy[i], ox = ox0 + opx[i], n = n0 + opn[i];
            const int Y = oy * a.OS + c.py, X = ox * a.OS + c.px;
            off = ((int64_t)n * a.M + m0 + 4 * kh) * HW + (int64_t)Y * a.OW + X;
            return (oy < c.OHc) && (ox < c.OWc) && (Y < a.OH) && (X < a.OW) && (opn[i] < a.BN) && (n < a.N);
        },
        [&](int ml) __attribute__((always_inline)) { return bias_lds[wm * (32 * MT) + 4 * kh + ml]; });
    stamp_out();
}

template <int MT, int NT, int WM>
int launch_pipe_family(const PipeArgs &a, int CKH, int TBU, dim3 grid, size_t lds, hipStream_t st, int threads);

template <int MT, int NT, int WM, int CKH, int TBU>
constexpr bool pipe_has_blk() {
#ifdef DVF_TUNING
    return true;
#else
    return MT == 2 && NT == 1 && WM == 1 && CKH >= 4 && TBU >= 2 && TBU <= 4;
#endif
}

template <int MT, int NT, int WM, int CKH, int TBU, int BLK>
inline int launch_pipe_blk(const PipeArgs &a, dim3 grid, size_t lds, hipStream_t st, int threads) {
    static bool big_lds = false;
    if (lds > 64 * 1024 && !big_lds) {
        if (hipFuncSetAttribute(reinterpret_cast<const void *>(&conv_pipe_kernel<MT, NT, WM, CKH, TBU, BLK>),
                                hipFuncAttributeMaxDynamicSharedMemorySize, 160 * 1024) != hipSuccess)
            return DVF_ERR_LAUNCH;
        big_lds = true;
    }
    conv_pipe_kernel<MT, NT, WM, CKH, TBU, BLK><<<grid, threads, lds, st>>>(a);
    return hipGetLastError() == hipSuccess ? DVF_OK : DVF_ERR_LAUNCH;
}

template <int MT, int NT, int WM, int CKH, int TBU>
inline int launch_pipe_one(const PipeArgs &a, dim3 grid, size_t lds, hipStream_t st, int threads) {
    if (a.blk) {
        if constexpr (pipe_has_blk<MT, NT, WM, CKH, TBU>()) return launch_pipe_blk<MT, NT, WM, CKH, TBU, 1>(a, grid, lds, st, threads);
        else return DVF_ERR_UNSUPPORTED;
    }
    return launch_pipe_blk<MT, NT, WM, CKH, TBU, 0>(a, grid, lds, st, threads);
}

template <int MT, int NT, int WM, int CKH>
inline int launch_pipe_tbu(const PipeArgs &a, int TBU, dim3 grid, size_t lds, hipStream_t st, int threads) {
    switch (TBU) {
        case 1: return launch_pipe_one<MT, NT, WM, CKH, 1>(a, grid, lds, st, threads);
        case 2: return launch_pipe_one<MT, NT, WM, CKH, 2>(a, grid, lds, st, threads);
        case 3: return launch_pipe_one<MT, NT, WM, CKH, 3>(a, grid, lds, st, threads);
        case 4: return launch_pipe_one<MT, NT, WM, CKH, 4>(a, grid, lds, st, threads);
        case 5: if constexpr (CKH <= 4 && WM == 1) return launch_pipe_one<MT, NT, WM, CKH, 5>(a, grid, lds, st, threads); else return DVF_ERR_UNSUPPORTED;
        case 7: if constexpr (CKH <= 4 && WM == 1) return launch_pipe_one<MT, NT, WM, CKH, 7>(a, grid, lds, st, threads); else return DVF_ERR_UNSUPPORTED;
        default: return DVF_ERR_UNSUPPORTED;
    }
}

#define DVF_PIPE_FAMILY(MT, NT, WM)                                                                              \
    template <>                                                                                                  \
    int launch_pipe_family<MT, NT, WM>(const PipeArgs &a, int CKH, int TBU, dim3 grid, size_t lds, hipStream_t st, int threads) { \
        switch (CKH) {                                                                                           \
            case 2: return launch_pipe_tbu<MT, NT, WM, 2>(a, TBU, grid, lds, st, threads);                                \
            case 4: return launch_pipe_tbu<MT, NT, WM, 4>(a, TBU, grid, lds, st, threads);                                \
            case 8: return launch_pipe_tbu<MT, NT, WM, 8>(a, TBU, grid, lds, st, threads);                                \
            default: return DVF_ERR_UNSUPPORTED;                                                                 \
        }                                                                                                        \
    }

}
```

depth-vo-feat_amd/csrc/conv_pipe_host.h:

```cpp
#pragma once
#include <string.h>
#include "dvf_common.h"
#include "conv_pipe.h"
#include "conv_op.h"

namespace {

using dvfp::PClass;
using dvfp::PipeArgs;
using dvfp::PipeGeo;
using dvfp::pipe_geo;
using dvfp::PIPE_MAXNPI;
using dvfp::OUT_FUSED;
using dvfp::OUT_ATOMIC;
using dvfp::OUT_WS;

struct alignas(8) PackArgsBody {
    const float *w;
    float *wp;
    int w_mode;
    int Mtot, Rtot, KK, m_base, M;
    int nseg, segC[DVF_MAX_SEGS];
    int ncls, NCH, CK, MB, VW, TBU;
    int TB[4], TA[4];
// ... 60 lines not shown
                if (i0 + j * 256 < total) S[si[j]] = v[j];
        }
    }
    __syncthreads();
    const int CKH = a.CK >> 1, CPG = CKH / a.VW, LV = 64 * a.VW;
    if (a.VW == 4) {
        typedef float f4 __attribute__((ext_vector_type(4)));
        const int lane = tid & 63, kh = lane >> 5, m = lane & 31;
        for (int c = 0; c < a.ncls; ++c) {
            const int TB = a.TB[c], NKU = a.TA[c] * CPG * a.TBU;
            float *dst = a.wp + a.wp_off[c] + (int64_t)(mb * a.NCH + g) * a.SL[c] + (int64_t)mtw * 256 + lane * 4;
            int ku = tid >> 6, u = ku, cpg = 0, ta = 0;
            while (u >= a.TBU) { u -= a.TBU; if (++cpg == CPG) { cpg = 0; ++ta; } }
            for (; ku < NKU; ku += 4) {
                f4 v = {0.f, 0.f, 0.f, 0.f};
                if (u < TB && m < mvalid) {
                    const float *src = S + m * SR + a.tapmap[c][ta * TB + u];
#pragma unroll
                    for (int j = 0; j < 4; ++j) {
                        const int rl = 2 * (cpg * 4 + j) + kh;
                        if (rl < nch) v[j] = src[rl * a.KK];
                    }
                }
                *reinterpret_cast<f4 *>(dst + (int64_t)ku * MTW * 256) = v;
                u += 4;
                while (u >= a.TBU) { u -= a.TBU; if (++cpg == CPG) { cpg = 0; ++ta; } }
            }
        }
        return;
    }
    const int x = tid & (LV - 1), kstep = 256 / LV;
    const int lane = x / a.VW, j = x - lane * a.VW, kh = lane >> 5, m = lane & 31;
    for (int c = 0; c < a.ncls; ++c) {
        const int TB = a.TB[c], NKU = a.TA[c] * CPG * a.TBU;
        float *dst = a.wp + a.wp_off[c] + (int64_t)(mb * a.NCH + g) * a.SL[c] + (int64_t)mtw * LV + x;
        int ku = tid / LV, u = ku, cpg = 0, ta = 0;
        while (u >= a.TBU) { u -= a.TBU; if (++cpg == CPG) { cpg = 0; ++ta; } }
        for (; ku < NKU; ku += kstep) {
            const int rl = 2 * (cpg * a.VW + j) + kh;
            float v = 0.f;
            if (u < TB && rl < nch && m < mvalid) v = S[m * SR + rl * a.KK + a.tapmap[c][ta * TB + u]];
            dst[(int64_t)ku * MTW * LV] = v;
            u += kstep;
            while (u >= a.TBU) { u -= a.TBU; if (++cpg == CPG) { cpg = 0; ++ta; } }
        }
    }
}

__global__ __launch_bounds__(256) void conv_pack_kernel(const PackArgs a) {
    extern __shared__ float S[];
    pack_block(a, blockIdx.x, blockIdx.y, S);
}

__global__ __launch_bounds__(256) void conv_pack_batch_kernel(const PackArgs *jobs, const int *prefix, const int *block_job,
                                                              int njobs) {
    extern __shared__ float S[];
    const int b = blockIdx.x;
    int lo = 0;
    if (block_job) {
        lo = block_job[b];
    } else {
        int hi = njobs;
        while (hi - lo > 1) {
            const int mid = (lo + hi) >> 1;
            if (prefix[mid] <= b) lo = mid; else hi = mid;
        }
    }
    const PackArgs &a = jobs[lo];
    const int local = b - prefix[lo];
    pack_block(a, local % a.NCH, local / a.NCH, S);
}

__global__ void bias_act_kernel(float *y, const float *bias, int C, int64_t HW, int64_t total, int act, float alpha,
                                float beta) {
    for (int64_t i = (int64_t)blockIdx.x * blockDim.x + threadIdx.x; i < total; i += (int64_t)gridDim.x * blockDim.x) {
        const int c = (int)((i / HW) % C);
        float v = y[i];
        if (bias) v += bias[c];
        y[i] = dvfp::apply_act(v, act, alpha, beta);
    }
}

__global__ void splitk_reduce_kernel(const float *ws, float *out, const float *bias, int KS, int64_t slice, int C, int64_t HW,
                                     int act, float alpha, float beta) {
    for (int64_t i = (int64_t)blockIdx.x * blockDim.x + threadIdx.x; i < slice; i += (int64_t)gridDim.x * blockDim.x) {
        float v = ws[i];
        for (int k = 1; k < KS; ++k) v += ws[i + k * slice];
        if (bias) v += bias[(int)((i / HW) % C)];
        out[i] = dvfp::apply_act(v, act, alpha, beta);
    }
}

__global__ __launch_bounds__(256) void splitk_reduce_mask_kernel(const float *ws, float *out, const float *mask, int KS,
                                                                 int64_t slice, int HW, int chunks) {
    const int plane = blockIdx.x / chunks, chunk = blockIdx.x - plane * chunks;
    const int per = (HW + chunks - 1) / chunks;
    const int lo = chunk * per, hi = min(HW, lo + per);
    const int64_t base = (int64_t)plane * HW;
    for (int e = lo + threadIdx.x; e < hi; e += 256) {
        const int64_t i = base + e;
        float v = ws[i];
        for (int k = 1; k < KS; ++k) v += ws[i + k * slice];
        out[i] = mask[i] > 0.f ? v : 0.f;
    }
}

__global__ __launch_bounds__(256) void splitk_reduce_kpar_kernel(const float *ws, float *out, const float *bias, const float *mask,
                                                                 int KS, int64_t slice, int C, int HW, int act, float alpha,
                                                                 float beta) {
    __shared__ float part[3][64];
    const int lane = threadIdx.x & 63, kq = threadIdx.x >> 6;
    const int k0 = (KS * kq) >> 2, k1 = (KS * (kq + 1)) >> 2;
    const int64_t i0 = (int64_t)blockIdx.x * 64, i = i0 + lane;
    float v = 0.f;
    if (i < slice) {
        const float *p = ws + i + (int64_t)k0 * slice;
#pragma unroll 8
        for (int k = k0; k < k1; ++k, p += slice) v += *p;
    }
    if (kq) part[kq - 1][lane] = v;
    __syncthreads();
    if (kq) return;
    if (i >= slice) return;
    v = ((v + part[0][lane]) + part[1][lane]) + part[2][lane];
    if (mask) {
        out[i] = mask[i] > 0.f ? v : 0.f;
        return;
    }
    if (bias) v += bias[(int)((i / HW) % C)];
    out[i] = dvfp::apply_act(v, act, alpha, beta);
}

inline int out_mode_of(bool covers, int KS, const float *ws, int64_t ws_floats, int64_t plan_ws_floats) {
    if (!covers) return OUT_ATOMIC;
    if (KS <= 1) return OUT_FUSED;
    return (ws && ws_floats >= plan_ws_floats) ? OUT_WS : OUT_ATOMIC;
}

template <class Args>
int prepare_output(Args &a, int mode, float *out, float *ws, hipStream_t st) {
    const int64_t total = (int64_t)a.N * a.M * a.OH * a.OW;
    a.out_mode = mode;
    a.out = out;
    if (mode == OUT_WS) { a.out = ws; a.ws_slice = total; }
    if (mode == OUT_ATOMIC && hipMemsetAsync(out, 0, sizeof(float) * total, st) != hipSuccess) return DVF_ERR_LAUNCH;
    return DVF_OK;
}

template <class Args>
int finish_output(const Args &a, bool kpar, const float *ws, float *out, hipStream_t st) {
    const int64_t HW = (int64_t)a.OH * a.OW, total = (int64_t)a.N * a.M * HW, nb = (total + 255) / 256;
    if (a.out_mode == OUT_WS && kpar) {
        splitk_reduce_kpar_kernel<<<(unsigned)((total + 63) / 64), 256, 0, st>>>(ws, out, a.bias, a.mask, a.KS, total, a.M, (int)HW,
                                                                                a.act, a.alpha, a.beta);
        DVF_LAUNCH_CHECK();
    } else if (a.out_mode == OUT_WS && a.mask) {
        int chunks = 1;
        const int64_t planes = (int64_t)a.N * a.M;
        while (planes * chunks < 1024 && HW / (chunks * 2) >= 256) chunks *= 2;
        splitk_reduce_mask_kernel<<<(unsigned)(planes * chunks), 256, 0, st>>>(ws, out, a.mask, a.KS, total, (int)HW, chunks);
        DVF_LAUNCH_CHECK();
    } else if (a.out_mode == OUT_WS) {
        splitk_reduce_kernel<<<(int)(nb > 4096 ? 4096 : nb), 256, 0, st>>>(ws, out, a.bias, a.KS, total, a.M, HW, a.act,
                                                                          a.alpha, a.beta);
        DVF_LAUNCH_CHECK();
    } else if (a.out_mode == OUT_ATOMIC && (a.bias || a.act != DVF_ACT_NONE)) {
        bias_act_kernel<<<(int)(nb > 2048 ? 2048 : nb), 256, 0, st>>>(out, a.bias, a.M, HW, total, a.act, a.alpha, a.beta);
        DVF_LAUNCH_CHECK();
    }
    if (a.out_mode == OUT_ATOMIC && a.mask)
        return dvf_act_bwd(out, a.mask, out, nullptr, a.N, a.M, (int)HW, DVF_ACT_RELU, 1.f, 0.f, 1, nullptr, 0, st);
    return DVF_OK;
}

#ifdef DVF_TUNING
constexpr size_t STAMP_MAX_BLOCKS = 16384;
unsigned long long *g_stamp_buf = nullptr;
int g_stamp_blocks = 0;
#endif
struct PipePlan {
    PipeArgs a;
    int MT, NT, WM, CKH, TBU, threads;
    size_t lds;
    dim3 grid;
    int64_t packed_floats;
    int64_t ws_floats;
    bool reduce_kpar;
    size_t pack_lds;
};

struct PipeOverride { int on, MT, NT, WM, CK, KS, BN, NST; };
inline PipeOverride pipe_override() {
    PipeOverride o{0, 0, 0, 0, 0, 0, 0, 0};
    if (const char *e = dvf_tune("DVF_PIPE_PLAN"))
        if (sscanf(e, "%d,%d,%d,%d,%d,%d,%d", &o.MT, &o.NT, &o.WM, &o.CK, &o.KS, &o.BN, &o.NST) >= 1) o.on = 1;
    return o;
}

struct PipeTiles { int lsw, lsh, TGX, TGY, TGN, BN; double cov; };
inline PipeTiles pipe_tiles(int OHc, int OWc, int N, int ntile, int BNwant, int IS, int TBmax) {
    PipeTiles best{5, 0, 1, ntile, 1, 1, 1e30};
    for (int lsn = 0; lsn <= 5; ++lsn) {
        const int SN = 1 << lsn;
        for (int lsw = 5 - lsn; lsw >= 0; --lsw) {
            const int lsh = 5 - lsn - lsw, SW = 1 << lsw, SH = 1 << lsh;
            for (int TGN = 1; TGN <= ntile; TGN *= 2) {
                const int BN = SN * TGN;
                if (BN != BNwant) continue;
                for (int TGX = 1; TGX * TGN <= ntile; TGX *= 2) {
                    const int TGY = ntile / (TGX * TGN), BW = TGX * SW, BH = TGY * SH;
                    if ((BW - 1) * IS + TBmax > 160) continue;
                    const double cov = (double)cdiv(OWc, BW) * BW * cdiv(OHc, BH) * BH * cdiv(N, BN) * BN;
                    const double narrow = (SW >= 16 ? 0.0 : (SW == 8 ? 0.12 : 0.3)) + (BW >= 32 ? 0.0 : 0.08);
                    const double cost = cov * (1.0 + narrow + 0.02 * lsh + 0.02 * lsn) + 1e-3 * (BW + BH);
                    if (cost < best.cov) best = PipeTiles{lsw, lsh, TGX, TGY, TGN, BN, cost};
                }
            }
        }
    }
    return best;
}


int plan_pipe(const ConvOp &op, PipePlan &pl) {
    if (op.ncls < 1) return DVF_ERR_UNSUPPORTED;
    const ClassSpec *cls = op.cls;
    const int ncls = op.ncls, Tmax = op.Tmax, TAmax = op.TAmax, TBmax = op.TBmax, OHc = op.OHc, OWc = op.OWc;
    const bool head_fwd = op.head_fwd;
    PipeArgs &a = pl.a;
    a = PipeArgs{};
    for (int s = 0; s < op.nseg; ++s) a.segC[s] = op.segC[s];
    a.nseg = op.nseg; a.M = op.M;
    a.N = op.N; a.IH = op.IH; a.IW = op.IW; a.OH = op.OH; a.OW = op.OW;
    a.act = op.act; a.alpha = op.alpha; a.beta = op.beta;
    a.ncls = ncls; a.OS = cls[0].OS; a.IS = cls[0].IS;
    const PipeOverride ov = pipe_override();
    static const int smallm = dvf_tune("DVF_PIPE_SMALLM") ? atoi(dvf_tune("DVF_PIPE_SMALLM")) : 0;
    int ctot = 0;
    for (int s = 0; s < a.nseg; ++s) ctot += a.segC[s];
    static const int headc = dvf_tune("DVF_PIPE_HEADC") ? atoi(dvf_tune("DVF_PIPE_HEADC")) : 128;
    const bool wide_head = head_fwd && a.M <= 4 && ncls == 1 && ctot >= headc && Tmax == 9;
    const bool small_ok = a.M > 16 || wide_head || (!(smallm & 8) && a.M <= 16 && ncls > 1) ||
                          ((smallm & 2) && a.M <= 16) || ((smallm & 4) && a.M > 16);
    if (a.M <= 32 && !ov.on && !small_ok) return DVF_ERR_UNSUPPORTED;
    if (ov.on && ov.KS < 0) return DVF_ERR_UNSUPPORTED;
    int maxc = 0;
    for (int s = 0; s < a.nseg; ++s) maxc = a.segC[s] > maxc ? a.segC[s] : maxc;
// ... 46 lines not shown
        Depth d{0, 0, 3, 0, 0};
        for (int i = 0; i < ncls; ++i) {
            const PipeGeo g = pipe_geo(a.BH, a.BW, a.BN, a.IS, cls[i].TA, TBU, SW, SH, x4, cls[i].bx);
            if (g.NPI > PIPE_MAXNPI) return d;
            d.PSRmax = g.PSR > d.PSRmax ? g.PSR : d.PSRmax;
        }
        auto lds_bytes = [&](int CK) { return ((size_t)d.NST * (slab(CK, TAmax) + (size_t)CK * d.PSRmax) + MB) * 4; };
        int CK = TBU >= 5 ? 8 : 16;
        while (CK > 4 && lds_bytes(CK) > PIPE_LDS_BUDGET) CK >>= 1;
        while (CK > 4 && CK / 2 >= maxc) CK >>= 1;
        if (lds_bytes(CK) > PIPE_LDS_BUDGET) {
            d.NST = 2;
            if (lds_bytes(CK) > PIPE_LDS_BUDGET && PIPE_LDS_BUDGET < 150 * 1024) {
                d.NST = 3;
                if (lds_bytes(CK) > 150 * 1024) d.NST = 2;
                if (lds_bytes(CK) > 150 * 1024) return d;
            }
        }
        if (ov.on && ov.CK) { CK = ov.CK; d.NST = 3; if (lds_bytes(CK) > 150 * 1024) d.NST = 2; }
        if (ov.on && ov.NST) d.NST = ov.NST;
        if ((CK != 4 && CK != 8 && CK != 16) || lds_bytes(CK) > 150 * 1024) return d;
        d.ok = 1; d.CK = CK; d.lds = lds_bytes(CK);
        return d;
    };
    int want_x4 = (a.IW % 4 == 0 && (a.BW * a.IS) % 4 == 0) ? 1 : 0;
    if (const char *e = dvf_tune("DVF_PIPE_X4")) want_x4 = want_x4 && atoi(e) != 0;
    const Depth d1 = depth_for(0), d4 = want_x4 ? depth_for(1) : Depth{0, 0, 3, 0, 0};
    static const bool x4_force = dvf_tune("DVF_PIPE_X4") && atoi(dvf_tune("DVF_PIPE_X4")) == 2;
    const bool use4 = d4.ok && (!d1.ok || x4_force || (d4.CK >= d1.CK && d4.NST >= d1.NST));
    const Depth dd = use4 ? d4 : d1;
    if (!dd.ok) return DVF_ERR_UNSUPPORTED;
    a.x4 = use4 ? 1 : 0;
    a.PSRmax = dd.PSRmax;
    const int CK = dd.CK, NST = dd.NST;
    a.NST = NST;
    a.SLmax = slab(CK, TAmax);
    a.NCH = 0;
    for (int s = 0; s < a.nseg; ++s) a.NCH += cdiv(a.segC[s], CK);
    const int mblocks = cdiv(a.M, MB);
    unsigned off = 0;
    for (int i = 0; i < ncls; ++i) {
        const ClassSpec &c = cls[i];
        const int SL = slab(CK, c.TA);
        a.cls[i] = PClass{c.py, c.px, c.by, c.bx, c.TA, c.TB, c.OHc, c.OWc, SL, c.TA, off};
        const int64_t nf = (int64_t)mblocks * a.NCH * SL;
        if ((int64_t)off + nf >= ((int64_t)1 << 29)) return DVF_ERR_UNSUPPORTED;
        off += (unsigned)nf;
    }
    pl.packed_floats = off;
    int KS = KS0;
    if (ov.on && ov.KS) KS = ov.KS;
    if (KS > a.NCH) KS = a.NCH;
    if (KS < 1) KS = 1;
    if ((int64_t)a.NG * KS * ncls > 65535) return DVF_ERR_UNSUPPORTED;
    a.KS = KS;
    pl.ws_floats = (op.covers && KS > 1) ? (int64_t)KS * a.N * a.M * a.OH * a.OW : 0;
    pl.reduce_kpar = KS >= 8 && (int64_t)a.OH * a.OW < ((int64_t)1 << 30);
    for (int s2 = 0; s2 < a.nseg; ++s2)
        if ((int64_t)a.N * a.segC[s2] * a.IH * a.IW * 4 >= ((int64_t)1 << 31) - 16) return DVF_ERR_UNSUPPORTED;
    pl.MT = MT; pl.NT = NT; pl.WM = WM; pl.CKH = CK / 2; pl.TBU = TBU; pl.lds = dd.lds;
    pl.pack_lds = (size_t)32 * ((CK * op.KK) | 1) * sizeof(float);
    if (pl.pack_lds > 64 * 1024) return DVF_ERR_UNSUPPORTED;
    pl.grid = dim3(a.tilesX * a.tilesY, mblocks, a.NG * KS * ncls);
    {
        const int per_chunk = CK * TAmax * TBmax;
        const int64_t kseq = (int64_t)cdiv(a.NCH, KS) * per_chunk;
        static const int blk_knob = dvf_tune("DVF_PIPE_BLK") ? atoi(dvf_tune("DVF_PIPE_BLK")) : -1;
        static const int blk_terms = dvf_tune("DVF_PIPE_BLKT") ? atoi(dvf_tune("DVF_PIPE_BLKT")) : 0;
        const bool deep = MT == 2 && NT == 1 && WM == 1 && CK >= 8 && TBU >= 2 && TBU <= 4 && kseq >= 512 &&
                          ((int64_t)pl.grid.x * pl.grid.y * pl.grid.z <= 256 || pl.lds > 76 * 1024);
        int every = blk_terms > 0 ? (blk_terms + per_chunk / 2) / per_chunk : 1;
        if (every < 1) every = 1;
        a.blk = blk_knob == 0 ? 0 : blk_knob > 0 ? blk_knob : blk_terms > 0 ? (kseq >= 384 ? every : 0) : (deep ? 1 : 0);
    }
    {
        const int64_t nblocks_total = (int64_t)pl.grid.x * pl.grid.y * pl.grid.z;
        static const bool no4p = dvf_tune("DVF_PIPE_NO4P") != nullptr;
        static const int mt1_4p = dvf_tune("DVF_PIPE_MT1_4P") ? atoi(dvf_tune("DVF_PIPE_MT1_4P")) : 1;
        pl.threads = (!no4p && (pl.lds > 76 * 1024 || nblocks_total <= 256 || (MT == 1 && mt1_4p))) ? dvfp::PIPE_THREADS_4P : dvfp::PIPE_THREADS;
    }
    return DVF_OK;
}

int launch_pipe(const PipeArgs &a, const PipePlan &pl, hipStream_t st) {
    using dvfp::launch_pipe_family;
    if (pl.WM == 2) {
        if (pl.NT != 1) return DVF_ERR_UNSUPPORTED;
        return pl.MT == 2 ? launch_pipe_family<2, 1, 2>(a, pl.CKH, pl.TBU, pl.grid, pl.lds, st, pl.threads)
                          : launch_pipe_family<1, 1, 2>(a, pl.CKH, pl.TBU, pl.grid, pl.lds, st, pl.threads);
    }
    if (pl.WM != 1) return DVF_ERR_UNSUPPORTED;
    if (pl.MT == 2 && pl.NT == 2) return DVF_ERR_UNSUPPORTED;
    if (pl.MT == 2) return launch_pipe_family<2, 1, 1>(a, pl.CKH, pl.TBU, pl.grid, pl.lds, st, pl.threads);
    if (pl.NT == 2) return launch_pipe_family<1, 2, 1>(a, pl.CKH, pl.TBU, pl.grid, pl.lds, st, pl.threads);
    return launch_pipe_family<1, 1, 1>(a, pl.CKH, pl.TBU, pl.grid, pl.lds, st, pl.threads);
}

int run_pipe(const ConvOp &op, const PipePlan &pl, const ConvIO &io, const float *packed, float *ws, int64_t ws_floats,
             hipStream_t st) {
    PipeArgs a = pl.a;
    for (int s = 0; s < a.nseg; ++s) {
        a.in[s] = io.in[s];
        if (a.x4 && (reinterpret_cast<uintptr_t>(a.in[s]) & 15)) return DVF_ERR_UNSUPPORTED;
    }
    a.wp = packed; a.bias = io.bias; a.mask = io.mask;
    const int mode = out_mode_of(op.covers, a.KS, ws, ws_floats, pl.ws_floats);
    int rc = prepare_output(a, mode, io.out, ws, st);
    if (rc) return rc;
    if (const char *e = dvf_tune("DVF_DBG")) a.dbg = atoi(e);
    a.stamps = nullptr;
#ifdef DVF_TUNING
    if (dvf_tune("DVF_STAMPS")) {
        const size_t nb = (size_t)pl.grid.x * pl.grid.y * pl.grid.z;
        if (!g_stamp_buf && hipMalloc(&g_stamp_buf, STAMP_MAX_BLOCKS * 64) != hipSuccess) return DVF_ERR_LAUNCH;
        if (nb <= STAMP_MAX_BLOCKS) {
            if (hipMemsetAsync(g_stamp_buf, 0, nb * 64, st) != hipSuccess) return DVF_ERR_LAUNCH;
            a.stamps = g_stamp_buf;
            g_stamp_blocks = (int)nb;
        }
    }
#endif
    dvf_plan_note(DVF_K_PIPE, pl.MT, pl.NT, pl.WM, 2 * pl.CKH, pl.TBU, a.KS, a.BN, a.NST, pl.threads, (int)pl.lds, mode | (a.ncls << 4) | (a.x4 << 8) | ((a.blk ? 1 : 0) << 9));
    if (dvf_tune("DVF_PIPE_DEBUG"))
        fprintf(stderr, "[pipe] M %d chunks %d N %d out %dx%d cls %d | MT %d NT %d WM %d CK %d TBU %d KS %d BN %d tile %dx%d "
                "(sub %dx%d) grid %ux%ux%u lds %zu x%d mode %d\n", a.M, a.NCH, a.N, a.OH, a.OW, a.ncls, pl.MT, pl.NT, pl.WM,
                2 * pl.CKH, pl.TBU, a.KS, a.BN, a.BH, a.BW, 1 << a.lsh, 1 << a.lsw, pl.grid.x, pl.grid.y, pl.grid.z, pl.lds, a.NST, mode);
    rc = launch_pipe(a, pl, st);
    return rc ? rc : finish_output(a, pl.reduce_kpar, ws, io.out, st);
}

PackArgs pack_job(const ConvOp &op, const PipePlan &pl, const float *w, float *packed, int *blocks) {
    const PipeArgs &a = pl.a;
    PackArgs p{};
    p.w = w; p.wp = packed; p.w_mode = op.w_mode; p.Mtot = op.Mtot; p.Rtot = op.Rtot; p.KK = op.KK;
    p.m_base = op.m_base; p.M = a.M; p.nseg = a.nseg;
    for (int s = 0; s < a.nseg; ++s) p.segC[s] = a.segC[s];
    p.ncls = op.ncls; p.NCH = a.NCH; p.CK = 2 * pl.CKH; p.MB = 32 * pl.MT * pl.WM; p.VW = pl.CKH >= 4 ? 4 : pl.CKH;
    p.TBU = pl.TBU;
    for (int c = 0; c < op.ncls; ++c) {
        p.SL[c] = a.cls[c].SL;
        p.TB[c] = op.cls[c].TB;
        p.TA[c] = op.cls[c].TA;
        p.wp_off[c] = a.cls[c].wp_off;
        for (int t = 0; t < op.cls[c].TA * op.cls[c].TB; ++t) p.tapmap[c][t] = (signed char)op.cls[c].tapmap[t];
    }
    *blocks = a.NCH * cdiv(a.M, p.MB) * (p.MB >> 5);
    return p;
}

int launch_pack(const ConvOp &op, const PipePlan &pl, const float *w, float *packed, hipStream_t st) {
    int blocks;
    const PackArgs p = pack_job(op, pl, w, packed, &blocks);
    conv_pack_kernel<<<dim3(p.NCH, blocks / p.NCH), 256, pl.pack_lds, st>>>(p);
    DVF_LAUNCH_CHECK();
    return DVF_OK;
}

}
```

depth-vo-feat_amd/csrc/conv_pipe_inst_a.hip:

```cpp
#include "conv_pipe.h"
namespace dvfp {
DVF_PIPE_FAMILY(1, 1, 1)
DVF_PIPE_FAMILY(1, 2, 1)
}
```

depth-vo-feat_amd/csrc/conv_pipe_inst_b.hip:

```cpp
#include "conv_pipe.h"
namespace dvfp {
DVF_PIPE_FAMILY(2, 1, 1)
}
```

depth-vo-feat_amd/csrc/conv_pipe_inst_c.hip:

```cpp
#include "conv_pipe.h"
namespace dvfp {
DVF_PIPE_FAMILY(1, 1, 2)
DVF_PIPE_FAMILY(2, 1, 2)
}
```

depth-vo-feat_amd/dvf/conv.py:

```python
import ctypes
import math
import weakref

import torch
import torch.nn as nn

from . import lib as L


def _c(t):
    return t if (t.dtype == torch.float32 and t.is_contiguous()) else t.float().contiguous()


class _NullCtx:
    def __enter__(self):
        return self

    def __exit__(self, *exc):
        return False


_NULL = _NullCtx()


# ... 62 lines not shown
            g["blocks"] += list(nb[:n])
            g["lds"] = max(g["lds"], lds.value)
        dev = live[0][1].device
        t.setdefault("keep", []).append(t.get("launches"))
        t["launches"] = []
        for _, g in sorted(groups.items()):
            blocks = g["blocks"]
            prefix = [0]
            for b in blocks:
                prefix.append(prefix[-1] + b)
            t["launches"].append({
                "jobs": torch.frombuffer(bytearray(b"".join(g["blobs"])), dtype=torch.uint8).to(dev),
                "prefix": torch.tensor(prefix, dtype=torch.int32, device=dev),
                "block_job": torch.repeat_interleave(torch.arange(len(blocks), dtype=torch.int32),
                                                     torch.tensor(blocks, dtype=torch.int64)).to(dev),
                "njobs": len(blocks), "total": prefix[-1], "lds": g["lds"]})
        t["key"] = key
    for q in t["launches"]:
        L.check(lib.dvf_conv2d_pack_batch(q["jobs"].data_ptr(), q["prefix"].data_ptr(), q["block_job"].data_ptr(), q["njobs"],
                                          q["total"], q["lds"], L.stream()), "dvf_conv2d_pack_batch")
    for r, w in live:
        r[4][1] = _stamp(w)


def _packed_weights(weight, holder, desc, segc, kind, pkey=None, segarr=None):
    cache = holder.__dict__.get("_dvf_pack")
    if cache is None:
        cache = holder.__dict__["_dvf_pack"] = {}
    if pkey is None:
        pkey = (desc.N, desc.H_in, desc.W_in, desc.H_out, desc.W_out, desc.stride, desc.pad, desc.transposed, tuple(segc))
    key = (kind, pkey)
    ent = cache.get(key)
    if ent is None:
        lib = L.lib()
        if segarr is None:
            segarr = L.int_array(segc)
        nf = lib.dvf_conv2d_packed_floats(ctypes.byref(desc), segarr, len(segc), kind)
        wsf = max(int(lib.dvf_conv2d_ws_floats(ctypes.byref(desc), segarr, len(segc), kind)), 0)
        if nf == L.ERR_UNSUPPORTED:
            cache[key] = ent = [None, None, wsf]
        else:
            if nf < 0:
                L.check(int(nf), "dvf_conv2d_packed_floats")
            cache[key] = ent = [torch.zeros(int(nf), device=weight.device, dtype=torch.float32), None, wsf]
            _PACK_REGISTRY.append([weakref.ref(holder), desc, list(segc), kind, ent])
    buf = ent[0]
    if buf is None:
        return None, (_workspace(ent[2], weight.device) if ent[2] else None)
    stamp = (holder.data_ptr(), holder._version, getattr(holder, "_dvf_epoch", 0), L.PACK_EPOCH)
    if ent[1] != stamp:
        with L.timed("conv_pack", 0.0, 8.0 * weight.numel()):
            L.check(L.lib().dvf_conv2d_pack(ctypes.byref(desc), L.int_array(segc), len(segc), kind, L.dev(weight, "weight"),
                                            L.dev(buf), L.stream()), "dvf_conv2d_pack")
        ent[1] = stamp
    return buf, (_workspace(ent[2], weight.device) if ent[2] else None)


DETERMINISTIC = False


def set_deterministic(on=True):
    global DETERMINISTIC
    DETERMINISTIC = bool(on)


def _bias_sums(lib, dy, y, dpre, dbias, N, C, HW, act, alpha, beta, accumulate):
    ws = _workspace(int(lib.dvf_act_bwd_ws_floats(N, C, HW)), dy.device) if (DETERMINISTIC and dbias is not None) else None
    L.check(lib.dvf_act_bwd(L.dev(dy, "grad_out"), L.dev(y), L.dev(dpre), L.dev(dbias), N, C, HW, act, alpha, beta,
                            1 if accumulate else 0, L.dev(ws), ws.numel() if ws is not None else 0, L.stream()), "dvf_act_bwd")


def _wgrad_ws_floats(holder, desc, segc):
    cache = holder.__dict__.setdefault("_dvf_wgws", {})
    key = (desc.N, desc.H_in, desc.W_in, desc.H_out, desc.W_out, desc.stride, desc.pad, desc.transposed, tuple(segc))
    n = cache.get(key)
    if n is None:
        n = int(L.lib().dvf_conv2d_wgrad_ws_floats(ctypes.byref(desc), L.int_array(segc), len(segc)))
        cache[key] = n = max(n, 0)
    return n


GEOM_LOG = None
FUSE_RELU_BWD = True


class ReluTag:
    __slots__ = ()


class _Geo:
    __slots__ = ("desc", "dref", "segc", "segarr", "nseg", "cin0", "cout", "oh", "ow", "macs", "tag", "pkey")

    def __init__(self, weight, cfg, inputs):
        k, stride, pad, opad, transposed, act, alpha, beta, out_hw = cfg[:9]
        N, _, H, W = inputs[0].shape
        self.segc = segc = [int(x.shape[1]) for x in inputs]
        self.nseg, self.cin0 = len(segc), segc[0]
        self.segarr = L.int_array(segc)
        cin = sum(segc)
        self.cout = cout = weight.shape[1] if transposed else weight.shape[0]
        if (weight.shape[0] if transposed else weight.shape[1]) != cin:
            raise ValueError(f"weight {tuple(weight.shape)} does not match {cin} input channels")
        oh, ow = conv_out_size(H, k, stride, pad, opad, transposed), conv_out_size(W, k, stride, pad, opad, transposed)
        if out_hw is not None:
            oh, ow = min(oh, out_hw[0]), min(ow, out_hw[1])
        self.oh, self.ow = oh, ow
        self.desc = L.ConvDesc(N, cin, H, W, cout, oh, ow, k, k, stride, pad, 1 if transposed else 0, act, alpha, beta)
        self.dref = ctypes.byref(self.desc)
        taps = k * k / (stride * stride) if transposed else k * k
        self.macs = float(N) * cout * oh * ow * cin * taps
        self.tag = f"{'T' if transposed else 'C'}{k}x{k}s{stride} {cin}->{cout} in{H}x{W} out{oh}x{ow} N{N}"
        self.pkey = (N, H, W, oh, ow, stride, pad, 1 if transposed else 0, tuple(segc))


class ConvFn(torch.autograd.Function):

    @staticmethod
    def forward(ctx, weight, bias, cfg, *inputs):
        k, stride, pad, opad, transposed, act, alpha, beta, out_hw = cfg[:9]
        ctx.out_tag = cfg[9] if len(cfg) > 9 else None
        ctx.in_tags = [getattr(x, "_dvf_relu_tag", None) for x in inputs]
        ctx.wparam = weight if getattr(weight, "_dvf_grad", None) is not None else None
        ctx.bparam = bias if (bias is not None and getattr(bias, "_dvf_grad", None) is not None) else None
        ctx.holder = weight
        inputs = [_c(x) for x in inputs]
        weight = _c(weight)
        bias = _c(bias) if bias is not None else None
        x0 = inputs[0]
        N, _, H, W = x0.shape
        gkey = (cfg[:9], N, H, W) if len(inputs) == 1 else (cfg[:9], N, H, W) + tuple(x.shape[1] for x in inputs[1:])
        geos = ctx.holder.__dict__.get("_dvf_geo")
        if geos is None:
            geos = ctx.holder.__dict__["_dvf_geo"] = {}
        g = geos.get(gkey)
        if g is None:
            g = geos[gkey] = _Geo(weight, cfg, inputs)
        elif g.cin0 != x0.shape[1]:
            raise ValueError(f"weight {tuple(weight.shape)} does not match {sum(int(x.shape[1]) for x in inputs)} input channels")
        if g.nseg > 1:
            for x in inputs:
                if x.shape[0] != N or x.shape[2] != H or x.shape[3] != W:
                    raise ValueError(f"virtual concat needs equal N,H,W; got {[tuple(t.shape) for t in inputs]}")
        desc, segc, cout, oh, ow = g.desc, g.segc, g.cout, g.oh, g.ow
        if GEOM_LOG is not None:
            GEOM_LOG.append((tuple(segc), cout, tuple(cfg[:9]), (N, H, W), tuple(ctx.needs_input_grad[3:])))
        out = torch.empty((N, cout, oh, ow), device=weight.device, dtype=torch.float32)
        ctx.macs, ctx.tag, ctx.geo = g.macs, g.tag, g
        packed, ws = _packed_weights(weight, ctx.holder, desc, segc, 0, g.pkey, g.segarr)
        if not x0.is_cuda:
            L.dev(x0, "input")
        inarr = (ctypes.c_void_p * g.nseg)(*[x.data_ptr() for x in inputs])
        wsp, wsn = (ws.data_ptr(), ws.numel()) if ws is not None else (None, 0)
        bp = bias.data_ptr() if bias is not None else None
        lib = L.lib()
        with (L.timed("conv_fwd", 2 * g.macs, tag=g.tag) if L.TIMER is not None else _NULL):
            rc = lib.dvf_conv2d_fwd(g.dref, inarr, g.segarr, g.nseg, packed.data_ptr() if packed is not None else None,
                                    weight.data_ptr(), bp, out.data_ptr(), wsp, wsn, L.stream_raw())
            if rc != 0:
                L.check(rc, "dvf_conv2d_fwd")
        if L.PLAN_LOG is not None:
            L.note_plans("fwd")
        ctx.save_for_backward(weight, out, *inputs)
        ctx.desc, ctx.segc, ctx.has_bias, ctx.inarr = desc, segc, bias is not None, inarr
        return out

    @staticmethod
    def backward(ctx, gout):
        weight, out, *inputs = ctx.saved_tensors
        desc, segc, g = ctx.desc, ctx.segc, ctx.geo
        lib = L.lib()
        gout = _c(gout)
        N, cout, oh, ow = out.shape
        nig = ctx.needs_input_grad
        need_w, need_b = nig[0], ctx.has_bias and nig[1]
        need_in = nig[3:]
        timing = L.TIMER is not None
        st = L.stream_raw()
        acc_b = need_b and ctx.bparam is not None
        dbias = (ctx.bparam._dvf_grad if acc_b else torch.empty(cout, device=out.device)) if need_b else None
        fused_out = ctx.out_tag is not None
        if fused_out:
            dpre = gout
        elif desc.act != L.ACT_NONE:
            dpre = torch.empty_like(gout)
            with (L.timed("act_bwd", 0.0, 12.0 * gout.numel()) if timing else _NULL):
                _bias_sums(lib, gout, out, dpre, dbias, N, cout, oh * ow, desc.act, desc.alpha, desc.beta, acc_b)
        else:
            dpre = gout
            if need_b:
                _bias_sums(lib, gout, None, None, dbias, N, cout, oh * ow, L.ACT_NONE, 1.0, 0.0, acc_b)
        if not dpre.is_cuda:
            L.dev(dpre, "grad_out")
        dprep = dpre.data_ptr()
        any_in = True in need_in
        gins = [torch.empty_like(x) if need else None for x, need in zip(inputs, need_in)] if any_in else [None] * g.nseg
        if any_in:
            packed, ws = _packed_weights(weight, ctx.holder, desc, segc, 1, g.pkey, g.segarr)
            wsp, wsn = (ws.data_ptr(), ws.numel()) if ws is not None else (None, 0)
            pp = packed.data_ptr() if packed is not None else None
            ginarr = (ctypes.c_void_p * g.nseg)(*[t.data_ptr() if t is not None else None for t in gins])
            masked = [t is not None and need for t, need in zip(ctx.in_tags, need_in)]
            if timing:
                frac = sum(c for c, need in zip(segc, need_in) if need) / float(sum(segc))
            marr = None
            if True in masked:
                marr = (ctypes.c_void_p * g.nseg)(*[x.data_ptr() if m else None for x, m in zip(inputs, masked)])
            with (L.timed("conv_dgrad", 2 * g.macs * frac, tag=g.tag) if timing else _NULL):
                rc = lib.dvf_conv2d_dgrad(g.dref, dprep, pp, weight.data_ptr(), ginarr, g.segarr, g.nseg, wsp, wsn, marr, st)
                if rc != 0:
                    L.check(rc, "dvf_conv2d_dgrad")
            if L.PLAN_LOG is not None:
                L.note_plans("dgrad")
        dw = None
        if fused_out and need_b and not need_w:
            _bias_sums(lib, dpre, None, None, dbias, N, cout, oh * ow, L.ACT_NONE, 1.0, 0.0, acc_b)
        if need_w:
            arena = ctx.wparam is not None
            dw = ctx.wparam._dvf_grad if arena else torch.empty_like(weight)
            side = ctx.wparam._dvf_owner.fork_wgrad(dpre, *inputs) if arena else None
            wst = side._dvf_raw if side is not None else st
            with (torch.cuda.stream(side) if (side is not None and timing) else _NULL):
                with (L.timed("conv_wgrad", 2 * g.macs, tag=g.tag) if timing else _NULL):
                    wsf = _wgrad_ws_floats(ctx.wparam if arena else weight, desc, segc) if DETERMINISTIC else 0
                    wws = _workspace(wsf, dpre.device, wst, side) if wsf > 0 else None
                    rc = lib.dvf_conv2d_wgrad(g.dref, ctx.inarr, g.segarr, g.nseg, dprep, dw.data_ptr(), 1 if arena else 0,
                                              dbias.data_ptr() if (fused_out and need_b) else None, 1 if acc_b else 0,
                                              wws.data_ptr() if wws is not None else None,
                                              wws.numel() if wws is not None else 0, wst)
                    if rc != 0:
                        L.check(rc, "dvf_conv2d_wgrad")
                    if L.PLAN_LOG is not None:
                        L.note_plans("wgrad")
            if arena:
                ctx.wparam._dvf_owner.grad_ready(ctx.wparam)
                dw = None
        if acc_b:
            ctx.bparam._dvf_owner.grad_ready(ctx.bparam)
            dbias = None
        return (dw, dbias, None, *gins)


class Upsample2xFn(torch.autograd.Function):

    @staticmethod
    def forward(ctx, x, out_hw):
        x = _c(x)
        N, C, H, W = x.shape
        oh, ow = min(2 * H, out_hw[0]), min(2 * W, out_hw[1])
        out = torch.empty((N, C, oh, ow), device=x.device, dtype=torch.float32)
        L.check(L.lib().dvf_resize_bilinear_fwd(L.dev(x, "input"), L.dev(out), N * C, H, W, oh, ow, 0.5, 0.5, L.stream()),
                "dvf_resize_bilinear_fwd")
        ctx.shape = (N, C, H, W, oh, ow)
        return out

    @staticmethod
    def backward(ctx, gout):
        N, C, H, W, oh, ow = ctx.shape
        gin = torch.empty((N, C, H, W), device=gout.device, dtype=torch.float32)
        L.check(L.lib().dvf_upsample2x_bwd(L.dev(_c(gout), "grad_out"), L.dev(gin), N * C, H, W, oh, ow, L.stream()),
                "dvf_upsample2x_bwd")
        return gin, None


class RecipFn(torch.autograd.Function):

    @staticmethod
    def forward(ctx, x, eps):
        x = _c(x)
        y = torch.empty_like(x)
        L.check(L.lib().dvf_recip_fwd(L.dev(x, "input"), L.dev(y), eps, x.numel(), L.stream()), "dvf_recip_fwd")
        ctx.save_for_backward(y)
        return y

    @staticmethod
    def backward(ctx, gy):
        (y,) = ctx.saved_tensors
        gx = torch.empty_like(y)
        L.check(L.lib().dvf_recip_bwd(L.dev(_c(gy), "grad_out"), L.dev(y), L.dev(gx), y.numel(), L.stream()),
                "dvf_recip_bwd")
        return gx, None


class SpatialMeanFn(torch.autograd.Function):

    @staticmethod
    def forward(ctx, x, scale):
        x = _c(x)
        N, C, H, W = x.shape
        out = torch.empty((N, C), device=x.device, dtype=torch.float32)
        L.check(L.lib().dvf_spatial_mean_fwd(L.dev(x, "input"), L.dev(out), N * C, H * W, scale, L.stream()),
                "dvf_spatial_mean_fwd")
        ctx.shape, ctx.scale = (N, C, H, W), scale
        return out

    @staticmethod
# ... 140 lines not shown
```

depth-vo-feat_amd/dvf/lib.py:

```python
import ctypes
import os

import torch

_HERE = os.path.dirname(os.path.abspath(__file__))
LIB_PATH = os.environ.get("DVF_LIB") or os.path.join(_HERE, "libdvf_hip.so")
_lib = None

c_fp = ctypes.c_void_p
c_i = ctypes.c_int
c_u32 = ctypes.c_uint32
c_f = ctypes.c_float
c_i64 = ctypes.c_int64
c_pp = ctypes.POINTER(ctypes.c_void_p)



class ConvDesc(ctypes.Structure):
    _fields_ = [(n, ctypes.c_int) for n in ("N", "C_in", "H_in", "W_in", "C_out", "H_out", "W_out", "KH", "KW",
                                             "stride", "pad", "transposed", "act")] + \
               [("alpha", ctypes.c_float), ("beta", ctypes.c_float)]


c_desc = ctypes.POINTER(ConvDesc)
c_ip = ctypes.POINTER(ctypes.c_int)

ROT_QUAT, PAD_BORDER, ALIGN_CORNERS, POSE_SE3, PIXEL_COORDS, CAFFE_ABSLOSS = 1, 2, 4, 8, 16, 32
ACT_NONE, ACT_RELU, ACT_SIGMOID_AFFINE = 0, 1, 2
MAX_VIEWS, MAX_SEGS = 4, 5
DM_MEDIAN_SCALE, DM_RECLAMP = 1, 2

SIGNATURES = {
    "dvf_version": (c_i, []),
    "dvf_error_string": (ctypes.c_char_p, [c_i]),
    "dvf_build_has_tuning": (c_i, []),
    "dvf_conv2d_last_plans": (c_i, [c_ip, c_i]),
    "dvf_inverse_warp_fwd": (c_i, [c_fp] * 6 + [c_i] * 4 + [c_u32, c_fp]),
    "dvf_inverse_warp_bwd": (c_i, [c_fp] * 10 + [c_i] * 4 + [c_u32, c_fp]),
    "dvf_pose_ws_floats": (c_i64, [c_i, c_i]),
    "dvf_inverse_warp_ordered_ws_floats": (c_i64, [c_i] * 3),
    "dvf_inverse_warp_bwd_ordered": (c_i, [c_fp] * 10 + [c_i] * 4 + [c_u32, c_fp]),
    "dvf_pose_vec2mat_fwd": (c_i, [c_fp, c_fp, c_i, c_u32, c_fp]),
    "dvf_pose_vec2mat_bwd": (c_i, [c_fp] * 4 + [c_i, c_u32, c_fp]),
    "dvf_pixel2cam_fwd": (c_i, [c_fp] * 3 + [c_i] * 3 + [c_fp]),
    "dvf_pixel2cam_bwd": (c_i, [c_fp] * 3 + [c_i] * 3 + [c_fp]),
    "dvf_cam2pixel_fwd": (c_i, [c_fp] * 4 + [c_i] * 3 + [c_u32, c_fp]),
    "dvf_cam2pixel_bwd": (c_i, [c_fp] * 6 + [c_i] * 3 + [c_u32, c_fp]),
    "dvf_photo_loss_fwd": (c_i, [c_fp, c_pp, c_i] + [c_fp] * 8 + [c_i] * 4 + [c_f, c_u32, c_fp]),
    "dvf_photo_partials_floats": (c_i64, [c_i] * 4),
    "dvf_photo_pose_ws_floats": (c_i64, [c_i] * 4),
    "dvf_photo_loss_bwd": (c_i, [c_fp, c_pp, c_i] + [c_fp] * 9 + [c_pp, c_fp, c_fp] + [c_i] * 4 + [c_f, c_u32, c_fp]),
    "dvf_imresize_u8": (c_i, [c_fp, c_i, c_i, c_i, c_fp, c_fp, c_i, c_fp, c_fp, c_i, c_fp, c_fp, c_fp, c_i, c_i, c_fp]),
    "dvf_augment_frames": (c_i, [c_pp, c_pp, c_i, c_fp] + [c_i] * 4 + [c_f, c_fp]),
    "dvf_augment_geometry": (c_i, [c_fp] * 9 + [c_i] * 3 + [c_fp]),
    "dvf_edge_smooth_fwd": (c_i, [c_fp] * 4 + [c_i] * 4 + [c_f, c_f, c_f, c_i, c_fp]),
    "dvf_edge_smooth_partials_floats": (c_i64, [c_i] * 3),
    "dvf_edge_smooth_bwd": (c_i, [c_fp] * 4 + [c_i] * 4 + [c_f, c_f, c_f, c_fp]),
    "dvf_ssim_partials_floats": (c_i64, [c_i] * 3),
    "dvf_ssim_loss_fwd": (c_i, [c_fp] * 3 + [c_i64, c_fp, c_fp] + [c_i] * 4 + [c_f] * 4 + [c_i, c_fp]),
    "dvf_ssim_loss_bwd": (c_i, [c_fp] * 3 + [c_i64] + [c_fp] * 4 + [c_i] * 4 + [c_f] * 4 + [c_fp]),
    "dvf_minreproj_partials_floats": (c_i64, [c_i] * 4),
    "dvf_minreproj_fwd": (c_i, [c_fp, c_pp, c_i, c_i] + [c_fp] * 4 + [c_i] * 4 + [c_f] * 4 + [c_i, c_fp]),
    "dvf_minreproj_bwd": (c_i, [c_fp, c_pp, c_i, c_i, c_fp, c_fp, c_fp, c_pp] + [c_i] * 4 + [c_f] * 4 + [c_fp]),
    "dvf_norm_smooth_partials_floats": (c_i64, [c_i] * 3),
    "dvf_norm_smooth_fwd": (c_i, [c_fp] * 5 + [c_i] * 4 + [c_f, c_f, c_f, c_i, c_fp]),
    "dvf_norm_smooth_bwd": (c_i, [c_fp] * 5 + [c_i] * 4 + [c_f, c_f, c_f, c_fp]),
    "dvf_smooth_loss_fwd": (c_i, [c_fp] * 3 + [c_i] * 3 + [c_f, c_i, c_fp]),
    "dvf_smooth_partials_floats": (c_i64, [c_i] * 3),
    "dvf_smooth_loss_bwd": (c_i, [c_fp] * 3 + [c_i] * 3 + [c_f, c_fp]),
    "dvf_conv2d_fwd": (c_i, [c_desc, c_pp, c_ip, c_i] + [c_fp] * 5 + [c_i64, c_fp]),
    "dvf_conv2d_dgrad": (c_i, [c_desc, c_fp, c_fp, c_fp, c_pp, c_ip, c_i, c_fp, c_i64, c_pp, c_fp]),
    "dvf_conv2d_wgrad": (c_i, [c_desc, c_pp, c_ip, c_i, c_fp, c_fp, c_i, c_fp, c_i, c_fp, c_i64, c_fp]),
    "dvf_conv2d_wgrad_ws_floats": (c_i64, [c_desc, c_ip, c_i]),
    "dvf_conv2d_packed_floats": (c_i64, [c_desc, c_ip, c_i, c_i]),
    "dvf_conv2d_pack": (c_i, [c_desc, c_ip, c_i, c_i, c_fp, c_fp, c_fp]),
    "dvf_conv2d_ws_floats": (c_i64, [c_desc, c_ip, c_i, c_i]),
    "dvf_conv2d_pack_jobs": (c_i, [c_desc, c_ip, c_i, c_i, c_fp, c_fp, c_fp, c_i, c_ip, c_ip]),
    "dvf_conv2d_pack_batch": (c_i, [c_fp, c_fp, c_fp, c_i, c_i, c_i, c_fp]),
    "dvf_act_bwd": (c_i, [c_fp] * 4 + [c_i] * 4 + [c_f, c_f, c_i, c_fp, c_i64, c_fp]),
    "dvf_act_bwd_ws_floats": (c_i64, [c_i, c_i, c_i]),
    "dvf_resize_bilinear_fwd": (c_i, [c_fp, c_fp] + [c_i] * 5 + [c_f, c_f, c_fp]),
    "dvf_upsample2x_bwd": (c_i, [c_fp, c_fp] + [c_i] * 5 + [c_fp]),
    "dvf_upsample_int_fwd": (c_i, [c_fp, c_fp] + [c_i] * 5 + [c_f, c_fp]),
    "dvf_upsample_int_bwd": (c_i, [c_fp] * 3 + [c_i] * 5 + [c_fp]),
    "dvf_recip_fwd": (c_i, [c_fp, c_fp, c_f, c_i64, c_fp]),
    "dvf_recip_bwd": (c_i, [c_fp, c_fp, c_fp, c_i64, c_fp]),
    "dvf_spatial_mean_fwd": (c_i, [c_fp, c_fp, c_i, c_i, c_f, c_fp]),
    "dvf_spatial_mean_bwd": (c_i, [c_fp, c_fp, c_i, c_i, c_f, c_fp]),
    "dvf_area_downsample": (c_i, [c_fp, c_fp] + [c_i] * 5 + [c_fp]),
    "dvf_dwconvt4x4s2_fwd": (c_i, [c_fp] * 5 + [c_i] * 4 + [c_fp]),
    "dvf_dwconvt4x4s2_bwd": (c_i, [c_fp] * 6 + [c_i] * 4 + [c_fp]),
    "dvf_bce_ones_fwd": (c_i, [c_fp, c_fp, c_fp, c_i64, c_i, c_fp]),
    "dvf_bce_ones_bwd": (c_i, [c_fp, c_fp, c_fp, c_i64, c_fp]),
    "dvf_adam_step": (c_i, [c_fp] * 4 + [c_i64, c_fp, c_i] + [c_f] * 5 + [c_fp]),
    "dvf_depth_metrics_ws_floats": (c_i64, [c_i] * 3),
    "dvf_depth_metrics": (c_i, [c_fp] * 4 + [c_i64] + [c_i] * 7 + [c_f] * 4 + [c_u32, c_fp]),
    "dvf_pose_chain": (c_i, [c_fp, c_ip, c_i, c_fp, c_fp]),
    "dvf_odometry_errors_ws_doubles": (c_i64, [c_i]),
    "dvf_odometry_errors": (c_i, [c_fp, c_fp, c_i, c_fp, c_fp, c_i, c_fp, c_i64, c_fp]),
    "dvf_trajectory_align_ws_doubles": (c_i64, [c_i]),
    "dvf_trajectory_align": (c_i, [c_fp, c_fp, c_i, c_i, c_fp, c_fp, c_i64, c_fp]),
    "dvf_trajectory_apply": (c_i, [c_fp, c_fp, c_i, c_i, c_fp, c_fp]),
    "dvf_trajectory_errors_ws_doubles": (c_i64, [c_i]),
    "dvf_trajectory_errors": (c_i, [c_fp, c_fp, c_i, c_fp, c_fp, c_i64, c_fp]),
    "dvf_snippet_errors_ws_doubles": (c_i64, [c_i]),
    "dvf_snippet_errors": (c_i, [c_fp, c_fp, c_i, c_i, c_fp, c_fp, c_i, c_fp, c_i64, c_fp]),
}


def lib():
    global _lib
    if _lib is None:
        if not os.path.exists(LIB_PATH):
            raise RuntimeError(
                f"{LIB_PATH} not found: build it with `make -C depth-vo-feat_amd/csrc` "
                "(or __graft_entry__.build()).  There is no fallback path.")
        L = ctypes.CDLL(LIB_PATH)
        for name, (res, args) in SIGNATURES.items():
            fn = getattr(L, name)
            fn.restype, fn.argtypes = res, args
        _lib = L
    return _lib


def check(rc, what):
    if rc != 0:
        raise RuntimeError(f"{what} failed: {lib().dvf_error_string(rc).decode()} (code {rc})")


_DEV_INDEX = None


def stream():
    global _DEV_INDEX
    if _DEV_INDEX is None:
        _DEV_INDEX = torch.cuda.current_device()
    return ctypes.c_void_p(torch._C._cuda_getCurrentRawStream(_DEV_INDEX))


def stream_raw():
    global _DEV_INDEX
    if _DEV_INDEX is None:
        _DEV_INDEX = torch.cuda.current_device()
    return torch._C._cuda_getCurrentRawStream(_DEV_INDEX)


def dev(t, name="tensor"):
    if t is None:
        return None
    if not t.is_cuda:
        raise RuntimeError(f"{name}: the HIP path needs a CUDA/HIP tensor, got {t.device}; there is no CPU fallback")
    if t.dtype != torch.float32:
        raise TypeError(f"{name}: expected float32, got {t.dtype}")
    if not t.is_contiguous():
# ... 153 lines not shown
```

include/dvf_hip.h:

```cpp
#ifndef DVF_HIP_H
#define DVF_HIP_H

#include <stdint.h>

#ifdef __cplusplus
extern "C" {
#endif

#define DVF_OK 0
#define DVF_ERR_INVALID_ARG (-1)
#define DVF_ERR_LAUNCH (-2)
#define DVF_ERR_UNSUPPORTED (-3)

#define DVF_ROT_QUAT 1u
#define DVF_PAD_BORDER 2u
#define DVF_ALIGN_CORNERS 4u
#define DVF_POSE_SE3 8u
#define DVF_PIXEL_COORDS 16u

#define DVF_CAFFE_ABSLOSS 32u

#define DVF_ACT_NONE 0
#define DVF_ACT_RELU 1
#define DVF_ACT_SIGMOID_AFFINE 2
// ... 17 lines not shown
int64_t dvf_inverse_warp_ordered_ws_floats(int B, int H, int W);
int dvf_inverse_warp_bwd_ordered(const float *img, const float *depth, const float *pose, const float *K,
                                 const float *Kinv, const float *grad_out, float *g_img, float *g_depth,
                                 float *g_pose, float *ws, int B, int C, int H, int W, uint32_t flags,
                                 void *stream);

int dvf_pose_vec2mat_fwd(const float *pose, float *out, int n, uint32_t flags, void *stream);
int dvf_pose_vec2mat_bwd(const float *pose, const float *g_mat, float *g_pose, float *ws, int n, uint32_t flags,
                         void *stream);
int dvf_pixel2cam_fwd(const float *depth, const float *Kinv, float *cam, int B, int H, int W, void *stream);
int dvf_pixel2cam_bwd(const float *Kinv, const float *g_cam, float *g_depth, int B, int H, int W, void *stream);
int dvf_cam2pixel_fwd(const float *cam, const float *rot, const float *tr, float *grid, int B, int H, int W,
                      uint32_t flags, void *stream);
int dvf_cam2pixel_bwd(const float *cam, const float *rot, const float *tr, const float *g_grid, float *g_cam,
                      float *g_rot_tr_ws, int B, int H, int W, uint32_t flags, void *stream);

int dvf_photo_loss_fwd(const float *tgt, const float *const *srcs, int V, const float *depth,
                       const float *pose, const float *K, const float *Kinv, const float *mask,
                       float *loss_out, float *view_loss, float *partials, int B, int C, int H, int W,
                       float in_scale, uint32_t flags, void *stream);
int64_t dvf_photo_partials_floats(int B, int H, int W, int V);
int dvf_photo_loss_bwd(const float *tgt, const float *const *srcs, int V, const float *depth,
                       const float *pose, const float *K, const float *Kinv, const float *mask,
                       const float *grad_loss, float *g_depth, float *g_pose, float *g_tgt,
                       float *const *g_srcs, float *g_mask, float *pose_ws, int B, int C, int H, int W,
                       float in_scale, uint32_t flags, void *stream);
int64_t dvf_photo_pose_ws_floats(int B, int H, int W, int V);

int dvf_imresize_u8(const uint8_t *src_hwc, int IH, int IW, int C, const int *hbounds, const int *hcoef, int hksize,
                    const int *vbounds, const int *vcoef, int vksize, uint8_t *tmp, int *minmax, float *dst_chw, int OH, int OW,
                    void *stream);

int dvf_augment_frames(const float *const *src, float *const *dst, int F, const float *params, int B, int C, int H, int W,
                       float value_max, void *stream);
int dvf_augment_geometry(const float *params, const float *K, const float *Kinv, const float *T_tr, const float *T_se3,
                         float *K_out, float *Kinv_out, float *T_tr_out, float *T_se3_out, int B, int W, int H, void *stream);

int dvf_edge_smooth_fwd(const float *inv_depth, const float *img, float *loss_out, float *partials, int B, int C, int H, int W,
                        float in_scale, float edge_k, float weight, int accumulate, void *stream);
int64_t dvf_edge_smooth_partials_floats(int B, int H, int W);
int dvf_edge_smooth_bwd(const float *inv_depth, const float *img, const float *grad_loss, float *g_inv_depth, int B, int C, int H,
                        int W, float in_scale, float edge_k, float weight, void *stream);

int64_t dvf_ssim_partials_floats(int B, int H, int W);
int dvf_ssim_loss_fwd(const float *tgt, const float *warped, const float *mask, int64_t mask_batch_stride, float *loss_out,
                      float *partials, int B, int C, int H, int W, float in_scale, float alpha, float c1, float c2, int accumulate,
                      void *stream);
int dvf_ssim_loss_bwd(const float *tgt, const float *warped, const float *mask, int64_t mask_batch_stride, const float *grad_loss,
                      float *g_warped, float *g_tgt, float *g_mask, int B, int C, int H, int W, float in_scale, float alpha,
                      float c1, float c2, void *stream);

int64_t dvf_minreproj_partials_floats(int B, int H, int W, int K);
int dvf_minreproj_fwd(const float *tgt, const float *const *cands, int V, int auto_mask, float *loss_out, uint8_t *select,
                      int32_t *counts, float *partials, int B, int C, int H, int W, float in_scale, float alpha, float c1, float c2,
                      int accumulate, void *stream);
int dvf_minreproj_bwd(const float *tgt, const float *const *cands, int V, int auto_mask, const uint8_t *select,
                      const float *grad_loss, float *g_tgt, float *const *g_warped, int B, int C, int H, int W, float in_scale,
                      float alpha, float c1, float c2, void *stream);

int64_t dvf_norm_smooth_partials_floats(int B, int H, int W);
int dvf_norm_smooth_fwd(const float *disp, const float *img, float *loss_out, float *stats, float *partials, int B, int C, int H,
                        int W, float in_scale, float eps, float weight, int accumulate, void *stream);
int dvf_norm_smooth_bwd(const float *disp, const float *img, const float *stats, const float *grad_loss, float *g_disp, int B,
                        int C, int H, int W, float in_scale, float eps, float weight, void *stream);

int dvf_smooth_loss_fwd(const float *map, float *loss_out, float *partials, int N, int H, int W,
                        float weight, int accumulate, void *stream);
int64_t dvf_smooth_partials_floats(int N, int H, int W);
int dvf_smooth_loss_bwd(const float *map, const float *grad_loss, float *g_map, int N, int H, int W,
                        float weight, void *stream);

typedef struct dvf_conv_desc {
    int N, C_in, H_in, W_in, C_out, H_out, W_out, KH, KW, stride, pad, transposed;
    int act;
    float alpha, beta;
} dvf_conv_desc;

int dvf_conv2d_fwd(const dvf_conv_desc *d, const float *const *in_segs, const int *seg_channels, int nseg,
                   const float *packed, const float *w, const float *bias, float *out, float *ws, int64_t ws_floats,
                   void *stream);
int dvf_conv2d_dgrad(const dvf_conv_desc *d, const float *dpre, const float *packed, const float *w, float *const *din_segs,
                     const int *seg_channels, int nseg, float *ws, int64_t ws_floats, const float *const *mask_segs,
                     void *stream);
int64_t dvf_conv2d_wgrad_ws_floats(const dvf_conv_desc *d, const int *seg_channels, int nseg);
int dvf_conv2d_wgrad(const dvf_conv_desc *d, const float *const *in_segs, const int *seg_channels, int nseg,
                     const float *dpre, float *dw, int accumulate, float *dbias, int accumulate_dbias, float *ws,
                     int64_t ws_floats, void *stream);

int64_t dvf_conv2d_packed_floats(const dvf_conv_desc *d, const int *seg_channels, int nseg, int op_kind);
int dvf_conv2d_pack(const dvf_conv_desc *d, const int *seg_channels, int nseg, int op_kind, const float *w, float *packed,
                    void *stream);
int64_t dvf_conv2d_ws_floats(const dvf_conv_desc *d, const int *seg_channels, int nseg, int op_kind);
#define DVF_PACK_JOB_BYTES 512
int dvf_conv2d_pack_jobs(const dvf_conv_desc *d, const int *seg_channels, int nseg, int op_kind, const float *w, float *packed,
                         void *jobs_host, int max_jobs, int *blocks_out, int *lds_bytes_out);
int dvf_conv2d_pack_batch(const void *jobs_dev, const int *block_prefix_dev, const int *block_job_dev, int njobs,
                          int total_blocks, int lds_bytes, void *stream);
int64_t dvf_act_bwd_ws_floats(int N, int C, int HW);
int dvf_act_bwd(const float *dy, const float *y, float *dpre, float *dbias, int N, int C, int HW, int act, float alpha,
                float beta, int accumulate_dbias, float *ws, int64_t ws_floats, void *stream);

int dvf_resize_bilinear_fwd(const float *in, float *out, int planes, int H, int W, int OH, int OW, float scale_h,
                            float scale_w, void *stream);
int dvf_upsample2x_bwd(const float *gout, float *gin, int planes, int H, int W, int OH, int OW, void *stream);
int dvf_upsample_int_fwd(const float *in, float *out, int planes, int H, int W, int factor, int recip, float eps,
                         void *stream);
int dvf_upsample_int_bwd(const float *gout, const float *out, float *gin, int planes, int H, int W, int factor, int recip,
                         void *stream);
int dvf_recip_fwd(const float *x, float *y, float eps, int64_t n, void *stream);
int dvf_recip_bwd(const float *gy, const float *y, float *gx, int64_t n, void *stream);
int dvf_spatial_mean_fwd(const float *in, float *out, int planes, int HW, float scale, void *stream);
int dvf_spatial_mean_bwd(const float *gout, float *gin, int planes, int HW, float scale, void *stream);
int dvf_area_downsample(const float *in, float *out, int planes, int H, int W, int OH, int OW, void *stream);
int dvf_dwconvt4x4s2_fwd(const float *x, const float *w, const float *bias, const float *skip, float *out, int N, int C,
                         int H, int W, void *stream);
int dvf_dwconvt4x4s2_bwd(const float *x, const float *w, const float *dy, float *dx, float *dw, float *db, int N, int C,
                         int H, int W, void *stream);
int dvf_bce_ones_fwd(const float *mask, float *loss_out, float *partials, int64_t n, int accumulate, void *stream);
int dvf_bce_ones_bwd(const float *mask, const float *grad_loss, float *g_mask, int64_t n, void *stream);
int dvf_adam_step(float *param, const float *grad, float *exp_avg, float *exp_avg_sq, int64_t n, float *opt_state,
                  int advance_step, float beta1, float beta2, float eps, float weight_decay, float grad_scale,
                  void *stream);

#define DVF_DM_MEDIAN_SCALE 1u
#define DVF_DM_RECLAMP 2u
int64_t dvf_depth_metrics_ws_floats(int B, int H, int W);
int dvf_depth_metrics(const float *gt, const float *pred, float *out , float *ws, int64_t ws_floats, int B, int H,
                      int W, int y1, int y2, int x1, int x2, float gt_lo, float gt_hi, float clamp_lo, float clamp_hi,
                      uint32_t flags, void *stream);

int dvf_pose_chain(const float *rel , const int *offsets , int S, double *world ,
                   void *stream);
int64_t dvf_odometry_errors_ws_doubles(int n);
int dvf_odometry_errors(const double *gt, const double *res , int n, double *rows ,
                        double *summary , int accumulate, double *ws, int64_t ws_doubles, void *stream);

#define DVF_ALIGN_NONE 0
#define DVF_ALIGN_SCALE 1
#define DVF_ALIGN_SCALE_7DOF 2
#define DVF_ALIGN_6DOF 3
#define DVF_ALIGN_7DOF 4
int64_t dvf_trajectory_align_ws_doubles(int n);
int dvf_trajectory_align(const double *gt, const double *res , int n, int mode, double *transform ,
                         double *ws, int64_t ws_doubles, void *stream);
int dvf_trajectory_apply(const double *res , const double *transform , int n, int copy,
                         double *out , void *stream);
int64_t dvf_trajectory_errors_ws_doubles(int n);
int dvf_trajectory_errors(const double *gt, const double *res , int n, double *out , double *ws,
                          int64_t ws_doubles, void *stream);
int64_t dvf_snippet_errors_ws_doubles(int n);
int dvf_snippet_errors(const double *gt, const double *res , int n, int length, double *rows ,
                       double *summary , int accumulate, double *ws, int64_t ws_doubles, void *stream);

#ifdef __cplusplus
}
#endif
#endif
```

Measured before the change: 649.2.

## Accumulate multi-consumer activation gradients directly in conv dgrad epilogues

When a ReLU-tagged activation feeds several convolutions, the first consumer's dgrad output is parked, and later consumers' dgrad kernels add their contribution into that buffer instead of writing a fresh tensor. This removes the separate autograd gradient-sum pass and one temporary allocation per extra consumer. Accumulating variants are added to the gather, pipe and head kernels, with a host pre-check that falls back when an output mode cannot accumulate. By default only reduce-only (workspace) modes accumulate, and the extra read-modify-write plus added template instantiations bring some cost and complexity.

Result: no change. 647.3 (-0.3%).

```diff
diff --git a/depth-vo-feat_amd/csrc/conv.hip b/depth-vo-feat_amd/csrc/conv.hip
--- a/depth-vo-feat_amd/csrc/conv.hip
+++ b/depth-vo-feat_amd/csrc/conv.hip
@@ -223,25 +223,32 @@
     return DVF_OK;
 }
 
+template <int MT, int NT, int ACC>
+int launch_gather_acc(const GatherArgs &a, const GatherPlan &pl, hipStream_t st) {
+    switch (pl.CKH) {
+        case 1: conv_gather_kernel<MT, NT, 1, ACC><<<pl.grid, 256, pl.lds, st>>>(a); break;
+        case 2: conv_gather_kernel<MT, NT, 2, ACC><<<pl.grid, 256, pl.lds, st>>>(a); break;
+        case 4: conv_gather_kernel<MT, NT, 4, ACC><<<pl.grid, 256, pl.lds, st>>>(a); break;
+        case 8: conv_gather_kernel<MT, NT, 8, ACC><<<pl.grid, 256, pl.lds, st>>>(a); break;
+        default: return DVF_ERR_UNSUPPORTED;
+    }
+    DVF_LAUNCH_CHECK();
+    return DVF_OK;
+}
+
 template <int MT, int NT>
 int launch_gather_ck(const GatherArgs &a, const GatherPlan &pl, hipStream_t st) {
-    switch (pl.CKH) {
-        case 1: conv_gather_kernel<MT, NT, 1><<<pl.grid, 256, pl.lds, st>>>(a); break;
-        case 2: conv_gather_kernel<MT, NT, 2><<<pl.grid, 256, pl.lds, st>>>(a); break;
-        case 4: conv_gather_kernel<MT, NT, 4><<<pl.grid, 256, pl.lds, st>>>(a); break;
-        case 8: conv_gather_kernel<MT, NT, 8><<<pl.grid, 256, pl.lds, st>>>(a); break;
-        default: return DVF_ERR_UNSUPPORTED;
-    }
-    DVF_LAUNCH_CHECK();
-    return DVF_OK;
+    return (a.acc && a.out_mode == OUT_FUSED) ? launch_gather_acc<MT, NT, 1>(a, pl, st) : launch_gather_acc<MT, NT, 0>(a, pl, st);
 }
 
 int run_gather(const ConvOp &op, const GatherPlan &pl, const ConvIO &io, const float *w, float *ws, int64_t ws_floats,
                hipStream_t st) {
     GatherArgs a = pl.a;
     for (int s = 0; s < a.nseg; ++s) a.in[s] = io.in[s];
-    a.w = w; a.bias = io.bias; a.mask = io.mask;
-    int rc = prepare_output(a, out_mode_of(op.covers, a.KS, ws, ws_floats, pl.ws_floats), io.out, ws, st);
+    a.w = w; a.bias = io.bias; a.mask = io.mask; a.acc = io.acc;
+    const int mode = out_mode_of(op.covers, a.KS, ws, ws_floats, pl.ws_floats);
+    if (io.acc && !out_mode_accumulates(mode)) return DVF_ERR_UNSUPPORTED;
+    int rc = prepare_output(a, mode, io.out, ws, st);
     if (rc) return rc;
     if (const char *e = dvf_tune("DVF_DBG")) a.dbg = atoi(e);
     if (pl.MT == 2 && pl.NT == 2) rc = launch_gather_ck<2, 2>(a, pl, st);
@@ -277,10 +284,23 @@
 int dgrad_unpacked(const dvf_conv_desc *d, const ConvOp &op, const ConvIO &io, const float *w, float *ws, int64_t ws_floats,
                    hipStream_t st) {
     if (dvf_head_seg_dgrad_applicable(d, op.M))
-        return dvf_head_seg_dgrad(d, io.in[0], w, io.out, op.m_base, op.M, st, io.mask);
+        return dvf_head_seg_dgrad(d, io.in[0], w, io.out, op.m_base, op.M, st, io.mask, io.acc);
     GatherPlan pl;
     const int rc = plan_gather(op, pl);
     return rc ? rc : run_gather(op, pl, io, w, ws, ws_floats, st);
+}
+
+bool dgrad_seg_accumulates(const dvf_conv_desc *d, const ConvOp &op, bool packed, const PipePlan &plan, const float *dpre,
+                           float *ws, int64_t ws_floats, bool reduce_only) {
+    if (packed && !(plan.a.x4 && (reinterpret_cast<uintptr_t>(dpre) & 15))) {
+        const int mode = out_mode_of(op.covers, plan.a.KS, ws, ws_floats, plan.ws_floats);
+        return reduce_only ? mode == OUT_WS : pipe_accumulates(plan, mode);
+    }
+    if (dvf_head_seg_dgrad_applicable(d, op.M)) return !reduce_only;
+    GatherPlan pl;
+    if (plan_gather(op, pl)) return true;
+    const int mode = out_mode_of(op.covers, pl.a.KS, ws, ws_floats, pl.ws_floats);
+    return reduce_only ? mode == OUT_WS : out_mode_accumulates(mode);
 }
 
 int64_t unpacked_ws_floats(const ConvOp &op, bool direct) {
@@ -674,6 +694,12 @@
 int dvf_conv2d_dgrad(const dvf_conv_desc *d, const float *dpre, const float *packed, const float *w, float *const *din_segs,
                      const int *seg_channels, int nseg, float *ws, int64_t ws_floats, const float *const *mask_segs,
                      void *stream) {
+    return dvf_conv2d_dgrad_acc(d, dpre, packed, w, din_segs, seg_channels, nseg, ws, ws_floats, mask_segs, nullptr, stream);
+}
+
+int dvf_conv2d_dgrad_acc(const dvf_conv_desc *d, const float *dpre, const float *packed, const float *w, float *const *din_segs,
+                         const int *seg_channels, int nseg, float *ws, int64_t ws_floats, const float *const *mask_segs,
+                         const int *acc_segs, void *stream) {
     dvf_plan_reset();
     int rc = check_desc(d);
     if (rc) return rc;
@@ -682,11 +708,24 @@
     if (!dpre || !w || !din_segs) return DVF_ERR_INVALID_ARG;
     hipStream_t st = dvf_stream(stream);
     auto mask = [&](int s) -> const float * { return mask_segs ? mask_segs[s] : nullptr; };
-    if (dvf_head_dgrad_applicable(d, nseg) || (dvf_head_applicable(d, nseg) && !packed))
-        return din_segs[0] ? dvf_head_dgrad(d, dpre, w, din_segs[0], st, mask(0)) : DVF_OK;
+    auto acc = [&](int s) -> int { return (acc_segs && acc_segs[s]) ? 1 : 0; };
+    auto reduce_only = [&](int s) -> bool { return acc_segs && acc_segs[s] == 2; };
+    if (dvf_head_dgrad_applicable(d, nseg) || (dvf_head_applicable(d, nseg) && !packed)) {
+        if (din_segs[0] && reduce_only(0)) return DVF_ERR_UNSUPPORTED;
+        return din_segs[0] ? dvf_head_dgrad(d, dpre, w, din_segs[0], st, mask(0), acc(0)) : DVF_OK;
+    }
+    bool any_acc = false;
+    for (int s = 0; s < nseg; ++s) any_acc = any_acc || (din_segs[s] && acc(s));
+    if (any_acc) {
+        rc = for_each_dgrad_seg(d, seg_channels, nseg, packed != nullptr, [&](const DgradSeg &v) -> int {
+            if (!din_segs[v.s] || !acc(v.s)) return DVF_OK;
+            return dgrad_seg_accumulates(d, v.op, v.packed, v.plan, dpre, ws, ws_floats, reduce_only(v.s)) ? DVF_OK : DVF_ERR_UNSUPPORTED;
+        });
+        if (rc) return rc;
+    }
     return for_each_dgrad_seg(d, seg_channels, nseg, packed != nullptr, [&](const DgradSeg &v) -> int {
         if (!din_segs[v.s]) return DVF_OK;
-        const ConvIO io{&dpre, nullptr, din_segs[v.s], mask(v.s)};
+        const ConvIO io{&dpre, nullptr, din_segs[v.s], mask(v.s), acc(v.s)};
         int r = v.packed ? run_pipe(v.op, v.plan, io, packed + v.packed_off, ws, ws_floats, st) : DVF_ERR_UNSUPPORTED;
         if (r == DVF_ERR_UNSUPPORTED) r = dgrad_unpacked(d, v.op, io, w, ws, ws_floats, st);
         return r;
diff --git a/depth-vo-feat_amd/csrc/conv_epilogue.h b/depth-vo-feat_amd/csrc/conv_epilogue.h
--- a/depth-vo-feat_amd/csrc/conv_epilogue.h
+++ b/depth-vo-feat_amd/csrc/conv_epilogue.h
@@ -23,7 +23,7 @@
     return v;
 }
 
-template <int MT, int NT, class Pix, class Bias>
+template <int MT, int NT, bool ACCI = false, class Pix, class Bias>
 __device__ __forceinline__ void store_tile(const f32x16 (&acc)[MT][NT], float *out, const float *mask, int out_mode, int act,
                                            float alpha, float beta, int m0, int kh, int M, int64_t HW, Pix pix, Bias bias_at) {
     auto store_all = [&](auto modec, auto actc, auto fullc) __attribute__((always_inline)) {
@@ -41,6 +41,32 @@
             int64_t off;
             const bool pok = pix(i, off);
             float *pbase = out + off;
+            if constexpr (MODE >= 4) {
+#pragma unroll
+                for (int m = 0; m < MT; ++m) {
+                    float pv[16], pm[16];
+#pragma unroll
+                    for (int r = 0; r < 16; ++r) {
+                        const int ml = m * 32 + (r & 3) + 8 * (r >> 2);
+                        const bool ok = pok && (FULL || m0 + 4 * kh + ml < M);
+                        const int64_t idx = ok ? off + (int64_t)ml * HW : 0;
+                        pv[r] = out[idx];
+                        if constexpr (MODE == 5) pm[r] = mask[idx];
+                    }
+                    if (pok) {
+#pragma unroll
+                        for (int r = 0; r < 16; ++r) {
+                            const int ml = m * 32 + (r & 3) + 8 * (r >> 2);
+                            if (FULL || m0 + 4 * kh + ml < M) {
+                                float v = acc[m][i][r];
+                                if constexpr (MODE == 5) v = pm[r] > 0.f ? v : 0.f;
+                                pbase[(int64_t)ml * HW] = pv[r] + v;
+                            }
+                        }
+                    }
+                }
+                continue;
+            }
             float mk[MT][16];
             if constexpr (MODE == 3) {
 #pragma unroll
@@ -76,6 +102,11 @@
         if (m0 + 32 * MT <= M) store_all(modec, actc, std::true_type{});
         else store_all(modec, actc, std::false_type{});
     };
+    if constexpr (ACCI) {
+        if (mask) by_full(integral_constant<int, 5>{}, integral_constant<int, DVF_ACT_NONE>{});
+        else by_full(integral_constant<int, 4>{}, integral_constant<int, DVF_ACT_NONE>{});
+        return;
+    }
     if (out_mode == OUT_FUSED && mask) by_full(integral_constant<int, 3>{}, integral_constant<int, DVF_ACT_NONE>{});
     else if (out_mode == OUT_WS) by_full(integral_constant<int, 2>{}, integral_constant<int, DVF_ACT_NONE>{});
     else if (out_mode == OUT_ATOMIC) by_full(integral_constant<int, 1>{}, integral_constant<int, DVF_ACT_NONE>{});
diff --git a/depth-vo-feat_amd/csrc/conv_gather.h b/depth-vo-feat_amd/csrc/conv_gather.h
--- a/depth-vo-feat_amd/csrc/conv_gather.h
+++ b/depth-vo-feat_amd/csrc/conv_gather.h
@@ -33,9 +33,10 @@
     int PSmax, Tmax, WD;
     int tapmap[52];
     const float *mask;
+    int acc;
 };
 
-template <int MT, int NT, int CKH>
+template <int MT, int NT, int CKH, int ACC = 0>
 __global__ __launch_bounds__(256) void conv_gather_kernel(const GatherArgs a) {
     constexpr int CK = 2 * CKH, COTP = 32 * MT + 1;
     extern __shared__ __attribute__((aligned(16))) float smem[];
@@ -246,7 +247,7 @@
         }
     }
     const int64_t HWo = (int64_t)a.OH * a.OW;
-    store_tile<MT, NT>(
+    store_tile<MT, NT, ACC != 0>(
         acc, a.out + (a.out_mode == dvfp::OUT_WS ? (int64_t)ks * a.ws_slice : 0), a.mask, a.out_mode, a.act, a.alpha, a.beta, m0, kh, a.M, HWo,
         [&](int i, int64_t &off) __attribute__((always_inline)) {
             const int oy = oy0 + opy[i], ox = ox0 + opx[i];
diff --git a/depth-vo-feat_amd/csrc/conv_head.h b/depth-vo-feat_amd/csrc/conv_head.h
--- a/depth-vo-feat_amd/csrc/conv_head.h
+++ b/depth-vo-feat_amd/csrc/conv_head.h
@@ -7,12 +7,13 @@
 bool dvf_head_wide_applicable(const dvf_conv_desc *d, int nseg);
 int dvf_head_fwd_segs(const dvf_conv_desc *d, const float *const *in_segs, const int *seg_channels, int nseg, const float *w,
                       const float *bias, float *out, hipStream_t st);
-int dvf_head_dgrad(const dvf_conv_desc *d, const float *dpre, const float *w, float *din, hipStream_t st, const float *mask = nullptr);
+int dvf_head_dgrad(const dvf_conv_desc *d, const float *dpre, const float *w, float *din, hipStream_t st, const float *mask = nullptr,
+                   int acc = 0);
 int dvf_head_wgrad(const dvf_conv_desc *d, const float *in, const float *dpre, float *dw, int accumulate, hipStream_t st,
                    float *ws = nullptr, int64_t ws_floats = 0);
 int64_t dvf_head_wgrad_ws_floats(const dvf_conv_desc *d);
 bool dvf_head_seg_dgrad_applicable(const dvf_conv_desc *d, int segc);
 int dvf_head_seg_dgrad(const dvf_conv_desc *d, const float *dpre, const float *w, float *din, int seg_off, int segc,
-                       hipStream_t st, const float *mask = nullptr);
+                       hipStream_t st, const float *mask = nullptr, int acc = 0);
 bool dvf_dconvt_applicable(const dvf_conv_desc *d, int nseg);
 int dvf_dconvt_fwd(const dvf_conv_desc *d, const float *in, const float *w, const float *bias, float *out, hipStream_t st);
diff --git a/depth-vo-feat_amd/csrc/conv_head.hip b/depth-vo-feat_amd/csrc/conv_head.hip
--- a/depth-vo-feat_amd/csrc/conv_head.hip
+++ b/depth-vo-feat_amd/csrc/conv_head.hip
@@ -41,7 +41,7 @@
 __global__ __launch_bounds__(256) void head_fwd_kernel(const HeadSegs in, const float *__restrict__ w,
                                                        const float *__restrict__ bias, float *__restrict__ out, int C, int H,
                                                        int W, int tilesX, int act, float alpha, float beta, int ws_m, int ws_c,
-                                                       int flip, const float *__restrict__ mask) {
+                                                       int flip, const float *__restrict__ mask, int accf) {
     constexpr int ROWS = FTH / 4, FPH = FTH + 2, FPN = FPH * HP_W, FLD = (FPN + 255) / 256;
     extern __shared__ __attribute__((aligned(16))) float wsh[];
     float *tile = wsh + ((MO * C * 9 + 3) & ~3);
@@ -162,7 +162,18 @@
     for (int r = 0; r < ROWS; ++r) {
         const int y = y0 + ly + r;
         if (y < H && x < W) {
-            if (mask) {
+            if (accf) {
+                float pv[MO], mv[MO];
+#pragma unroll
+                for (int m = 0; m < MO; ++m) {
+                    const int64_t idx = ((int64_t)n * MO + m) * plane + (int64_t)y * W + x;
+                    pv[m] = out[idx];
+                    mv[m] = mask ? mask[idx] : 1.f;
+                }
+#pragma unroll
+                for (int m = 0; m < MO; ++m)
+                    out[((int64_t)n * MO + m) * plane + (int64_t)y * W + x] = pv[m] + (mv[m] > 0.f ? acc[r][m] : 0.f);
+            } else if (mask) {
 #pragma unroll
                 for (int m = 0; m < MO; ++m) {
                     const int64_t idx = ((int64_t)n * MO + m) * plane + (int64_t)y * W + x;
@@ -180,7 +191,7 @@
 template <int MO>
 __global__ __launch_bounds__(256) void head_dgrad_kernel(const float *__restrict__ dpre, const float *__restrict__ w,
                                                          float *__restrict__ din, int C, int H, int W, int tilesX,
-                                                         const float *__restrict__ mask) {
+                                                         const float *__restrict__ mask, int accf) {
     __shared__ float tile[MO * HP_H * HP_W];
     extern __shared__ __attribute__((aligned(16))) float wsh[];
     constexpr int WPC = (MO * 9 + 3) & ~3;
@@ -207,11 +218,12 @@
     float *dst = din + base;
     const float *mk = mask ? mask + base : nullptr;
     for (int c0 = 0; c0 < C; c0 += 4) {
-        float sv[4], mv[4];
+        float sv[4], mv[4], pv[4];
 #pragma unroll
         for (int q = 0; q < 4; ++q) {
             const int c = min(c0 + q, C - 1);
             mv[q] = mk ? mk[c * plane] : 1.f;
+            pv[q] = accf ? dst[c * plane] : 0.f;
             const float *wc = wsh + c * WPC;
             float s = 0.f;
 #pragma unroll
@@ -222,7 +234,10 @@
         }
 #pragma unroll
         for (int q = 0; q < 4; ++q)
-            if (c0 + q < C) dst[(c0 + q) * plane] = (mv[q] > 0.f) ? sv[q] : 0.f;
+            if (c0 + q < C) {
+                const float v = (mv[q] > 0.f) ? sv[q] : 0.f;
+                dst[(c0 + q) * plane] = accf ? pv[q] + v : v;
+            }
     }
 }
 
@@ -467,13 +482,13 @@
     }
 
 static int head_fwd_launch(int MOv, const HeadSegs &in, const float *w, const float *bias, float *out, int C, int N, int H, int W,
-                           int act, float alpha, float beta, int ws_m, int ws_c, int flip, const float *mask, hipStream_t st) {
+                           int act, float alpha, float beta, int ws_m, int ws_c, int flip, const float *mask, int accf, hipStream_t st) {
     const bool lowres = (int64_t)N * H * W <= (int64_t)4 * 64 * 208 && MOv <= 4 && C >= 32;
     const int FTH = lowres ? 4 : FT_H, HCKT = lowres ? 32 : HCK;
     const int tilesX = cdiv(W, HT_W), tilesY = cdiv(H, FTH);
     const dim3 grid(tilesX * tilesY, N);
     const size_t lds = ((size_t)((MOv * C * 9 + 3) & ~3) + (size_t)HCKT * (FTH + 2) * HP_W) * 4;
-#define HEAD_FWD_GO(HC, FH) head_fwd_kernel<MO, HC, FH><<<grid, 256, lds, st>>>(in, w, bias, out, C, H, W, tilesX, act, alpha, beta, ws_m, ws_c, flip, mask)
+#define HEAD_FWD_GO(HC, FH) head_fwd_kernel<MO, HC, FH><<<grid, 256, lds, st>>>(in, w, bias, out, C, H, W, tilesX, act, alpha, beta, ws_m, ws_c, flip, mask, accf)
     if (lowres) {
         static bool big[5] = {false, false, false, false, false};
         HEAD_DISPATCH(MOv, {
@@ -507,7 +522,7 @@
     for (int s = 0; s < HEAD_MAX_SEGS; ++s) { in.p[s] = s < nseg ? in_segs[s] : in_segs[0]; in.c[s] = s < nseg ? seg_channels[s] : 0; }
     in.n = nseg;
     const int rc = head_fwd_launch(d->C_out, in, w, bias, out, d->C_in, d->N, d->H_in, d->W_in, d->act, d->alpha, d->beta,
-                                   d->C_in * 9, 9, 0, nullptr, st);
+                                   d->C_in * 9, 9, 0, nullptr, 0, st);
     if (rc) return rc;
     dvf_plan_note(DVF_K_HEAD_FWD, d->C_out, nseg);
     return DVF_OK;
@@ -522,23 +537,23 @@
 }
 
 int dvf_head_seg_dgrad(const dvf_conv_desc *d, const float *dpre, const float *w, float *din, int seg_off, int segc,
-                       hipStream_t st, const float *mask) {
+                       hipStream_t st, const float *mask, int acc) {
     const float *wseg = w + (int64_t)seg_off * 9;
     HeadSegs in{};
     for (int s = 0; s < HEAD_MAX_SEGS; ++s) { in.p[s] = dpre; in.c[s] = s == 0 ? d->C_out : 0; }
     in.n = 1;
     const int rc = head_fwd_launch(segc, in, wseg, nullptr, din, d->C_out, d->N, d->H_in, d->W_in, DVF_ACT_NONE, 1.f, 0.f, 9,
-                                   d->C_in * 9, 1, mask, st);
+                                   d->C_in * 9, 1, mask, acc, st);
     if (rc) return rc;
     dvf_plan_note(DVF_K_HEAD_SEG_DGRAD, segc);
     return DVF_OK;
 }
 
-int dvf_head_dgrad(const dvf_conv_desc *d, const float *dpre, const float *w, float *din, hipStream_t st, const float *mask) {
+int dvf_head_dgrad(const dvf_conv_desc *d, const float *dpre, const float *w, float *din, hipStream_t st, const float *mask, int acc) {
     const int tilesX = cdiv(d->W_in, HT_W), tilesY = cdiv(d->H_in, HT_H);
     const dim3 grid(tilesX * tilesY, d->N);
     HEAD_DISPATCH(d->C_out, (head_dgrad_kernel<MO><<<grid, 256, (size_t)d->C_in * ((MO * 9 + 3) & ~3) * 4, st>>>(
-                                dpre, w, din, d->C_in, d->H_in, d->W_in, tilesX, mask)));
+                                dpre, w, din, d->C_in, d->H_in, d->W_in, tilesX, mask, acc)));
     DVF_LAUNCH_CHECK();
     dvf_plan_note(DVF_K_HEAD_DGRAD, d->C_out);
     return DVF_OK;
diff --git a/depth-vo-feat_amd/csrc/conv_op.h b/depth-vo-feat_amd/csrc/conv_op.h
--- a/depth-vo-feat_amd/csrc/conv_op.h
+++ b/depth-vo-feat_amd/csrc/conv_op.h
@@ -28,6 +28,7 @@
     const float *bias;
     float *out;
     const float *mask;
+    int acc;
 };
 
 int check_desc(const dvf_conv_desc *d) {
diff --git a/depth-vo-feat_amd/csrc/conv_pipe.h b/depth-vo-feat_amd/csrc/conv_pipe.h
--- a/depth-vo-feat_amd/csrc/conv_pipe.h
+++ b/depth-vo-feat_amd/csrc/conv_pipe.h
@@ -49,6 +49,7 @@
     int dbg;
     unsigned long long *stamps;
     const float *mask;
+    int acc;
 };
 
 __host__ __device__ inline int pipe_row_stride(int RSu, int SW, int SH, int IS) {
@@ -93,7 +94,7 @@
 constexpr int PIPE_THREADS_4P = 512;
 constexpr int PIPE_MAXNPI = 32;
 
-template <int MT, int NT, int WM, int CKH, int TBU, int BLK = 0>
+template <int MT, int NT, int WM, int CKH, int TBU, int BLK = 0, int ACC = 0>
 __global__ __launch_bounds__(PIPE_THREADS_4P) void conv_pipe_kernel(const PipeArgs a) {
     constexpr int CK = 2 * CKH, VW = CKH >= 4 ? 4 : CKH, CPG = CKH / VW, MTW = MT * WM;
     constexpr int UNITF = TBU * MTW * 64 * VW;
@@ -469,7 +470,7 @@
     if DVF_DBG(a, 16) { stamp_out(); return; }
     const int m0 = mb * (32 * MTW) + wm * (32 * MT);
     const int64_t HW = (int64_t)a.OH * a.OW;
-    if (a.mask && a.out_mode == OUT_FUSED) {
+    if constexpr (ACC) {
         float *outp = a.out;
 #pragma unroll
         for (int i = 0; i < NT; ++i) {
@@ -477,42 +478,72 @@
             const int Y = oy * a.OS + c.py, X = ox * a.OS + c.px;
             const bool pok = (oy < c.OHc) && (ox < c.OWc) && (Y < a.OH) && (X < a.OW) && (opn[i] < a.BN) && (n < a.N);
             const int64_t base = ((int64_t)n * a.M + m0 + 4 * kh) * HW + (int64_t)Y * a.OW + X;
-            float mk[MT][16];
-#pragma unroll
-            for (int m = 0; m < MT; ++m)
+#pragma unroll
+            for (int m = 0; m < MT; ++m) {
+                float pv[16], mk[16];
 #pragma unroll
                 for (int r = 0; r < 16; ++r) {
                     const int ml = m * 32 + (r & 3) + 8 * (r >> 2);
                     const bool ok = pok && (m0 + 4 * kh + ml < a.M);
-                    mk[m][r] = a.mask[ok ? base + (int64_t)ml * HW : 0];
-                }
-#pragma unroll
-            for (int m = 0; m < MT; ++m) {
+                    const int64_t idx = ok ? base + (int64_t)ml * HW : 0;
+                    pv[r] = outp[idx];
+                    mk[r] = a.mask ? a.mask[idx] : 1.f;
+                }
 #pragma unroll
                 for (int r = 0; r < 16; ++r) {
                     const int ml = m * 32 + (r & 3) + 8 * (r >> 2);
-                    if (pok && m0 + 4 * kh + ml < a.M) {
-                        outp[base + (int64_t)ml * HW] = mk[m][r] > 0.f ? acc[m][i][r] : 0.f;
+                    if (pok && m0 + 4 * kh + ml < a.M)
+                        outp[base + (int64_t)ml * HW] = pv[r] + (mk[r] > 0.f ? acc[m][i][r] : 0.f);
+                }
+            }
+        }
+        stamp_out();
+    } else {
+        if (a.mask && a.out_mode == OUT_FUSED) {
+            float *outp = a.out;
+#pragma unroll
+            for (int i = 0; i < NT; ++i) {
+                const int oy = oy0 + opy[i], ox = ox0 + opx[i], n = n0 + opn[i];
+                const int Y = oy * a.OS + c.py, X = ox * a.OS + c.px;
+                const bool pok = (oy < c.OHc) && (ox < c.OWc) && (Y < a.OH) && (X < a.OW) && (opn[i] < a.BN) && (n < a.N);
+                const int64_t base = ((int64_t)n * a.M + m0 + 4 * kh) * HW + (int64_t)Y * a.OW + X;
+                float mk[MT][16];
+#pragma unroll
+                for (int m = 0; m < MT; ++m)
+#pragma unroll
+                    for (int r = 0; r < 16; ++r) {
+                        const int ml = m * 32 + (r & 3) + 8 * (r >> 2);
+                        const bool ok = pok && (m0 + 4 * kh + ml < a.M);
+                        mk[m][r] = a.mask[ok ? base + (int64_t)ml * HW : 0];
                     }
-                }
-            }
-        }
+#pragma unroll
+                for (int m = 0; m < MT; ++m) {
+#pragma unroll
+                    for (int r = 0; r < 16; ++r) {
+                        const int ml = m * 32 + (r & 3) + 8 * (r >> 2);
+                        if (pok && m0 + 4 * kh + ml < a.M) {
+                            outp[base + (int64_t)ml * HW] = mk[m][r] > 0.f ? acc[m][i][r] : 0.f;
+                        }
+                    }
+                }
+            }
+            stamp_out();
+            return;
+        }
+        store_tile<MT, NT>(
+            acc, a.out + (a.out_mode == OUT_WS ? (int64_t)ks * a.ws_slice : 0), nullptr, a.out_mode, a.act, a.alpha, a.beta, m0, kh, a.M, HW,
+            [&](int i, int64_t &off) __attribute__((always_inline)) {
+                const int oy = oy0 + opy[i], ox = ox0 + opx[i], n = n0 + opn[i];
+                const int Y = oy * a.OS + c.py, X = ox * a.OS + c.px;
+                off = ((int64_t)n * a.M + m0 + 4 * kh) * HW + (int64_t)Y * a.OW + X;
+                return (oy < c.OHc) && (ox < c.OWc) && (Y < a.OH) && (X < a.OW) && (opn[i] < a.BN) && (n < a.N);
+            },
+            [&](int ml) __attribute__((always_inline)) { return bias_lds[wm * (32 * MT) + 4 * kh + ml]; });
         stamp_out();
-        return;
-    }
-    store_tile<MT, NT>(
-        acc, a.out + (a.out_mode == OUT_WS ? (int64_t)ks * a.ws_slice : 0), nullptr, a.out_mode, a.act, a.alpha, a.beta, m0, kh, a.M, HW,
-        [&](int i, int64_t &off) __attribute__((always_inline)) {
-            const int oy = oy0 + opy[i], ox = ox0 + opx[i], n = n0 + opn[i];
-            const int Y = oy * a.OS + c.py, X = ox * a.OS + c.px;
-            off = ((int64_t)n * a.M + m0 + 4 * kh) * HW + (int64_t)Y * a.OW + X;
-            return (oy < c.OHc) && (ox < c.OWc) && (Y < a.OH) && (X < a.OW) && (opn[i] < a.BN) && (n < a.N);
-        },
-        [&](int ml) __attribute__((always_inline)) { return bias_lds[wm * (32 * MT) + 4 * kh + ml]; });
-    stamp_out();
-}
-
-template <int MT, int NT, int WM>
+    }
+}
+
+template <int MT, int NT, int WM, int ACC = 0>
 int launch_pipe_family(const PipeArgs &a, int CKH, int TBU, dim3 grid, size_t lds, hipStream_t st, int threads);
 
 template <int MT, int NT, int WM, int CKH, int TBU>
@@ -524,48 +555,48 @@
 #endif
 }
 
-template <int MT, int NT, int WM, int CKH, int TBU, int BLK>
+template <int MT, int NT, int WM, int CKH, int TBU, int BLK, int ACC>
 inline int launch_pipe_blk(const PipeArgs &a, dim3 grid, size_t lds, hipStream_t st, int threads) {
     static bool big_lds = false;
     if (lds > 64 * 1024 && !big_lds) {
-        if (hipFuncSetAttribute(reinterpret_cast<const void *>(&conv_pipe_kernel<MT, NT, WM, CKH, TBU, BLK>),
+        if (hipFuncSetAttribute(reinterpret_cast<const void *>(&conv_pipe_kernel<MT, NT, WM, CKH, TBU, BLK, ACC>),
                                 hipFuncAttributeMaxDynamicSharedMemorySize, 160 * 1024) != hipSuccess)
             return DVF_ERR_LAUNCH;
         big_lds = true;
     }
-    conv_pipe_kernel<MT, NT, WM, CKH, TBU, BLK><<<grid, threads, lds, st>>>(a);
+    conv_pipe_kernel<MT, NT, WM, CKH, TBU, BLK, ACC><<<grid, threads, lds, st>>>(a);
     return hipGetLastError() == hipSuccess ? DVF_OK : DVF_ERR_LAUNCH;
 }
 
-template <int MT, int NT, int WM, int CKH, int TBU>
+template <int MT, int NT, int WM, int CKH, int TBU, int ACC>
 inline int launch_pipe_one(const PipeArgs &a, dim3 grid, size_t lds, hipStream_t st, int threads) {
     if (a.blk) {
-        if constexpr (pipe_has_blk<MT, NT, WM, CKH, TBU>()) return launch_pipe_blk<MT, NT, WM, CKH, TBU, 1>(a, grid, lds, st, threads);
+        if constexpr (pipe_has_blk<MT, NT, WM, CKH, TBU>()) return launch_pipe_blk<MT, NT, WM, CKH, TBU, 1, ACC>(a, grid, lds, st, threads);
         else return DVF_ERR_UNSUPPORTED;
     }
-    return launch_pipe_blk<MT, NT, WM, CKH, TBU, 0>(a, grid, lds, st, threads);
-}
-
-template <int MT, int NT, int WM, int CKH>
+    return launch_pipe_blk<MT, NT, WM, CKH, TBU, 0, ACC>(a, grid, lds, st, threads);
+}
+
+template <int MT, int NT, int WM, int CKH, int ACC>
 inline int launch_pipe_tbu(const PipeArgs &a, int TBU, dim3 grid, size_t lds, hipStream_t st, int threads) {
     switch (TBU) {
-        case 1: return launch_pipe_one<MT, NT, WM, CKH, 1>(a, grid, lds, st, threads);
-        case 2: return launch_pipe_one<MT, NT, WM, CKH, 2>(a, grid, lds, st, threads);
-        case 3: return launch_pipe_one<MT, NT, WM, CKH, 3>(a, grid, lds, st, threads);
-        case 4: return launch_pipe_one<MT, NT, WM, CKH, 4>(a, grid, lds, st, threads);
-        case 5: if constexpr (CKH <= 4 && WM == 1) return launch_pipe_one<MT, NT, WM, CKH, 5>(a, grid, lds, st, threads); else return DVF_ERR_UNSUPPORTED;
-        case 7: if constexpr (CKH <= 4 && WM == 1) return launch_pipe_one<MT, NT, WM, CKH, 7>(a, grid, lds, st, threads); else return DVF_ERR_UNSUPPORTED;
+        case 1: return launch_pipe_one<MT, NT, WM, CKH, 1, ACC>(a, grid, lds, st, threads);
+        case 2: return launch_pipe_one<MT, NT, WM, CKH, 2, ACC>(a, grid, lds, st, threads);
+        case 3: return launch_pipe_one<MT, NT, WM, CKH, 3, ACC>(a, grid, lds, st, threads);
+        case 4: return launch_pipe_one<MT, NT, WM, CKH, 4, ACC>(a, grid, lds, st, threads);
+        case 5: if constexpr (CKH <= 4 && WM == 1) return launch_pipe_one<MT, NT, WM, CKH, 5, ACC>(a, grid, lds, st, threads); else return DVF_ERR_UNSUPPORTED;
+        case 7: if constexpr (CKH <= 4 && WM == 1) return launch_pipe_one<MT, NT, WM, CKH, 7, ACC>(a, grid, lds, st, threads); else return DVF_ERR_UNSUPPORTED;
         default: return DVF_ERR_UNSUPPORTED;
     }
 }
 
-#define DVF_PIPE_FAMILY(MT, NT, WM)                                                                              \
+#define DVF_PIPE_FAMILY(MT, NT, WM, ACC)                                                                            \
     template <>                                                                                                  \
-    int launch_pipe_family<MT, NT, WM>(const PipeArgs &a, int CKH, int TBU, dim3 grid, size_t lds, hipStream_t st, int threads) { \
+    int launch_pipe_family<MT, NT, WM, ACC>(const PipeArgs &a, int CKH, int TBU, dim3 grid, size_t lds, hipStream_t st, int threads) { \
         switch (CKH) {                                                                                           \
-            case 2: return launch_pipe_tbu<MT, NT, WM, 2>(a, TBU, grid, lds, st, threads);                                \
-            case 4: return launch_pipe_tbu<MT, NT, WM, 4>(a, TBU, grid, lds, st, threads);                                \
-            case 8: return launch_pipe_tbu<MT, NT, WM, 8>(a, TBU, grid, lds, st, threads);                                \
+            case 2: return launch_pipe_tbu<MT, NT, WM, 2, ACC>(a, TBU, grid, lds, st, threads);                                \
+            case 4: return launch_pipe_tbu<MT, NT, WM, 4, ACC>(a, TBU, grid, lds, st, threads);                                \
+            case 8: return launch_pipe_tbu<MT, NT, WM, 8, ACC>(a, TBU, grid, lds, st, threads);                                \
             default: return DVF_ERR_UNSUPPORTED;                                                                 \
         }                                                                                                        \
     }
diff --git a/depth-vo-feat_amd/csrc/conv_pipe_host.h b/depth-vo-feat_amd/csrc/conv_pipe_host.h
--- a/depth-vo-feat_amd/csrc/conv_pipe_host.h
+++ b/depth-vo-feat_amd/csrc/conv_pipe_host.h
@@ -166,32 +166,36 @@
 }
 
 __global__ void splitk_reduce_kernel(const float *ws, float *out, const float *bias, int KS, int64_t slice, int C, int64_t HW,
-                                     int act, float alpha, float beta) {
+                                     int act, float alpha, float beta, int accf) {
     for (int64_t i = (int64_t)blockIdx.x * blockDim.x + threadIdx.x; i < slice; i += (int64_t)gridDim.x * blockDim.x) {
+        const float pv = accf ? out[i] : 0.f;
         float v = ws[i];
         for (int k = 1; k < KS; ++k) v += ws[i + k * slice];
         if (bias) v += bias[(int)((i / HW) % C)];
-        out[i] = dvfp::apply_act(v, act, alpha, beta);
+        v = dvfp::apply_act(v, act, alpha, beta);
+        out[i] = accf ? pv + v : v;
     }
 }
 
 __global__ __launch_bounds__(256) void splitk_reduce_mask_kernel(const float *ws, float *out, const float *mask, int KS,
-                                                                 int64_t slice, int HW, int chunks) {
+                                                                 int64_t slice, int HW, int chunks, int accf) {
     const int plane = blockIdx.x / chunks, chunk = blockIdx.x - plane * chunks;
     const int per = (HW + chunks - 1) / chunks;
     const int lo = chunk * per, hi = min(HW, lo + per);
     const int64_t base = (int64_t)plane * HW;
     for (int e = lo + threadIdx.x; e < hi; e += 256) {
         const int64_t i = base + e;
+        const float pv = accf ? out[i] : 0.f;
         float v = ws[i];
         for (int k = 1; k < KS; ++k) v += ws[i + k * slice];
-        out[i] = mask[i] > 0.f ? v : 0.f;
+        v = mask[i] > 0.f ? v : 0.f;
+        out[i] = accf ? pv + v : v;
     }
 }
 
 __global__ __launch_bounds__(256) void splitk_reduce_kpar_kernel(const float *ws, float *out, const float *bias, const float *mask,
                                                                  int KS, int64_t slice, int C, int HW, int act, float alpha,
-                                                                 float beta) {
+                                                                 float beta, int accf) {
     __shared__ float part[3][64];
     const int lane = threadIdx.x & 63, kq = threadIdx.x >> 6;
     const int k0 = (KS * kq) >> 2, k1 = (KS * (kq + 1)) >> 2;
@@ -206,13 +210,16 @@
     __syncthreads();
     if (kq) return;
     if (i >= slice) return;
+    const float pv = accf ? out[i] : 0.f;
     v = ((v + part[0][lane]) + part[1][lane]) + part[2][lane];
     if (mask) {
-        out[i] = mask[i] > 0.f ? v : 0.f;
+        v = mask[i] > 0.f ? v : 0.f;
+        out[i] = accf ? pv + v : v;
         return;
     }
     if (bias) v += bias[(int)((i / HW) % C)];
-    out[i] = dvfp::apply_act(v, act, alpha, beta);
+    v = dvfp::apply_act(v, act, alpha, beta);
+    out[i] = accf ? pv + v : v;
 }
 
 inline int out_mode_of(bool covers, int KS, const float *ws, int64_t ws_floats, int64_t plan_ws_floats) {
@@ -220,6 +227,8 @@
     if (KS <= 1) return OUT_FUSED;
     return (ws && ws_floats >= plan_ws_floats) ? OUT_WS : OUT_ATOMIC;
 }
+
+inline bool out_mode_accumulates(int mode) { return mode == OUT_FUSED || mode == OUT_WS; }
 
 template <class Args>
 int prepare_output(Args &a, int mode, float *out, float *ws, hipStream_t st) {
@@ -236,17 +245,17 @@
     const int64_t HW = (int64_t)a.OH * a.OW, total = (int64_t)a.N * a.M * HW, nb = (total + 255) / 256;
     if (a.out_mode == OUT_WS && kpar) {
         splitk_reduce_kpar_kernel<<<(unsigned)((total + 63) / 64), 256, 0, st>>>(ws, out, a.bias, a.mask, a.KS, total, a.M, (int)HW,
-                                                                                a.act, a.alpha, a.beta);
+                                                                                a.act, a.alpha, a.beta, a.acc);
         DVF_LAUNCH_CHECK();
     } else if (a.out_mode == OUT_WS && a.mask) {
         int chunks = 1;
         const int64_t planes = (int64_t)a.N * a.M;
         while (planes * chunks < 1024 && HW / (chunks * 2) >= 256) chunks *= 2;
-        splitk_reduce_mask_kernel<<<(unsigned)(planes * chunks), 256, 0, st>>>(ws, out, a.mask, a.KS, total, (int)HW, chunks);
+        splitk_reduce_mask_kernel<<<(unsigned)(planes * chunks), 256, 0, st>>>(ws, out, a.mask, a.KS, total, (int)HW, chunks, a.acc);
         DVF_LAUNCH_CHECK();
     } else if (a.out_mode == OUT_WS) {
         splitk_reduce_kernel<<<(int)(nb > 4096 ? 4096 : nb), 256, 0, st>>>(ws, out, a.bias, a.KS, total, a.M, HW, a.act,
-                                                                          a.alpha, a.beta);
+                                                                          a.alpha, a.beta, a.acc);
         DVF_LAUNCH_CHECK();
     } else if (a.out_mode == OUT_ATOMIC && (a.bias || a.act != DVF_ACT_NONE)) {
         bias_act_kernel<<<(int)(nb > 2048 ? 2048 : nb), 256, 0, st>>>(out, a.bias, a.M, HW, total, a.act, a.alpha, a.beta);
@@ -459,8 +468,16 @@
     return DVF_OK;
 }
 
+inline bool pipe_accumulates(const PipePlan &pl, int mode) { return out_mode_accumulates(mode) && !(mode == OUT_FUSED && pl.WM != 1); }
+
 int launch_pipe(const PipeArgs &a, const PipePlan &pl, hipStream_t st) {
     using dvfp::launch_pipe_family;
+    if (a.acc && a.out_mode == OUT_FUSED) {
+        if (pl.WM != 1 || (pl.MT == 2 && pl.NT == 2)) return DVF_ERR_UNSUPPORTED;
+        if (pl.MT == 2) return launch_pipe_family<2, 1, 1, 1>(a, pl.CKH, pl.TBU, pl.grid, pl.lds, st, pl.threads);
+        if (pl.NT == 2) return launch_pipe_family<1, 2, 1, 1>(a, pl.CKH, pl.TBU, pl.grid, pl.lds, st, pl.threads);
+        return launch_pipe_family<1, 1, 1, 1>(a, pl.CKH, pl.TBU, pl.grid, pl.lds, st, pl.threads);
+    }
     if (pl.WM == 2) {
         if (pl.NT != 1) return DVF_ERR_UNSUPPORTED;
         return pl.MT == 2 ? launch_pipe_family<2, 1, 2>(a, pl.CKH, pl.TBU, pl.grid, pl.lds, st, pl.threads)
@@ -480,8 +497,9 @@
         a.in[s] = io.in[s];
         if (a.x4 && (reinterpret_cast<uintptr_t>(a.in[s]) & 15)) return DVF_ERR_UNSUPPORTED;
     }
-    a.wp = packed; a.bias = io.bias; a.mask = io.mask;
+    a.wp = packed; a.bias = io.bias; a.mask = io.mask; a.acc = io.acc;
     const int mode = out_mode_of(op.covers, a.KS, ws, ws_floats, pl.ws_floats);
+    if (io.acc && !pipe_accumulates(pl, mode)) return DVF_ERR_UNSUPPORTED;
     int rc = prepare_output(a, mode, io.out, ws, st);
     if (rc) return rc;
     if (const char *e = dvf_tune("DVF_DBG")) a.dbg = atoi(e);
diff --git a/depth-vo-feat_amd/csrc/conv_pipe_inst_a.hip b/depth-vo-feat_amd/csrc/conv_pipe_inst_a.hip
--- a/depth-vo-feat_amd/csrc/conv_pipe_inst_a.hip
+++ b/depth-vo-feat_amd/csrc/conv_pipe_inst_a.hip
@@ -1,5 +1,5 @@
 #include "conv_pipe.h"
 namespace dvfp {
-DVF_PIPE_FAMILY(1, 1, 1)
-DVF_PIPE_FAMILY(1, 2, 1)
+DVF_PIPE_FAMILY(1, 1, 1, 0)
+DVF_PIPE_FAMILY(1, 2, 1, 0)
 }
diff --git a/depth-vo-feat_amd/csrc/conv_pipe_inst_b.hip b/depth-vo-feat_amd/csrc/conv_pipe_inst_b.hip
--- a/depth-vo-feat_amd/csrc/conv_pipe_inst_b.hip
+++ b/depth-vo-feat_amd/csrc/conv_pipe_inst_b.hip
@@ -1,4 +1,4 @@
 #include "conv_pipe.h"
 namespace dvfp {
-DVF_PIPE_FAMILY(2, 1, 1)
+DVF_PIPE_FAMILY(2, 1, 1, 0)
 }
diff --git a/depth-vo-feat_amd/csrc/conv_pipe_inst_c.hip b/depth-vo-feat_amd/csrc/conv_pipe_inst_c.hip
--- a/depth-vo-feat_amd/csrc/conv_pipe_inst_c.hip
+++ b/depth-vo-feat_amd/csrc/conv_pipe_inst_c.hip
@@ -1,5 +1,5 @@
 #include "conv_pipe.h"
 namespace dvfp {
-DVF_PIPE_FAMILY(1, 1, 2)
-DVF_PIPE_FAMILY(2, 1, 2)
+DVF_PIPE_FAMILY(1, 1, 2, 0)
+DVF_PIPE_FAMILY(2, 1, 2, 0)
 }
diff --git a/depth-vo-feat_amd/csrc/conv_pipe_inst_d.hip b/depth-vo-feat_amd/csrc/conv_pipe_inst_d.hip
--- /dev/null
+++ b/depth-vo-feat_amd/csrc/conv_pipe_inst_d.hip
@@ -0,0 +1,5 @@
+#include "conv_pipe.h"
+namespace dvfp {
+DVF_PIPE_FAMILY(1, 1, 1, 1)
+DVF_PIPE_FAMILY(1, 2, 1, 1)
+}
diff --git a/depth-vo-feat_amd/csrc/conv_pipe_inst_e.hip b/depth-vo-feat_amd/csrc/conv_pipe_inst_e.hip
--- /dev/null
+++ b/depth-vo-feat_amd/csrc/conv_pipe_inst_e.hip
@@ -0,0 +1,4 @@
+#include "conv_pipe.h"
+namespace dvfp {
+DVF_PIPE_FAMILY(2, 1, 1, 1)
+}
diff --git a/depth-vo-feat_amd/dvf/conv.py b/depth-vo-feat_amd/dvf/conv.py
--- a/depth-vo-feat_amd/dvf/conv.py
+++ b/depth-vo-feat_amd/dvf/conv.py
@@ -168,10 +168,18 @@
 
 GEOM_LOG = None
 FUSE_RELU_BWD = True
+ACCUMULATE_DGRAD = True
+ACCUMULATE_FUSED = False
+ACC_STATS = {"accumulated": 0, "fallbacks": 0}
+_graph_task_id = getattr(torch._C, "_current_graph_task_id", None)
 
 
 class ReluTag:
-    __slots__ = ()
+    __slots__ = ("consumers", "park")
+
+    def __init__(self):
+        self.consumers = 0
+        self.park = None
 
 
 class _Geo:
@@ -206,6 +214,9 @@
         k, stride, pad, opad, transposed, act, alpha, beta, out_hw = cfg[:9]
         ctx.out_tag = cfg[9] if len(cfg) > 9 else None
         ctx.in_tags = [getattr(x, "_dvf_relu_tag", None) for x in inputs]
+        for t, need in zip(ctx.in_tags, ctx.needs_input_grad[3:]):
+            if t is not None and need:
+                t.consumers += 1
         ctx.wparam = weight if getattr(weight, "_dvf_grad", None) is not None else None
         ctx.bparam = bias if (bias is not None and getattr(bias, "_dvf_grad", None) is not None) else None
         ctx.holder = weight
@@ -266,6 +277,7 @@
         dbias = (ctx.bparam._dvf_grad if acc_b else torch.empty(cout, device=out.device)) if need_b else None
         fused_out = ctx.out_tag is not None
         if fused_out:
+            ctx.out_tag.park = None
             dpre = gout
         elif desc.act != L.ACT_NONE:
             dpre = torch.empty_like(gout)
@@ -280,6 +292,22 @@
         dprep = dpre.data_ptr()
         any_in = True in need_in
         gins = [torch.empty_like(x) if need else None for x, need in zip(inputs, need_in)] if any_in else [None] * g.nseg
+        roles, tid = None, -1
+        if any_in and ACCUMULATE_DGRAD and _graph_task_id is not None:
+            for i, t in enumerate(ctx.in_tags):
+                if t is None or not need_in[i] or t.consumers < 2:
+                    continue
+                if roles is None:
+                    roles, tid = [0] * g.nseg, _graph_task_id()
+                p = t.park
+                if tid < 0 or ctx.in_tags.count(t) > 1:
+                    t.park = (tid, st, None)
+                elif p is None or p[0] != tid:
+                    roles[i] = 1
+                elif p[2] is not None and p[1] == st:
+                    roles[i], gins[i] = 2, p[2]
+                else:
+                    t.park = (tid, st, None)
         if any_in:
             packed, ws = _packed_weights(weight, ctx.holder, desc, segc, 1, g.pkey, g.segarr)
             wsp, wsn = (ws.data_ptr(), ws.numel()) if ws is not None else (None, 0)
@@ -292,11 +320,34 @@
             if True in masked:
                 marr = (ctypes.c_void_p * g.nseg)(*[x.data_ptr() if m else None for x, m in zip(inputs, masked)])
             with (L.timed("conv_dgrad", 2 * g.macs * frac, tag=g.tag) if timing else _NULL):
-                rc = lib.dvf_conv2d_dgrad(g.dref, dprep, pp, weight.data_ptr(), ginarr, g.segarr, g.nseg, wsp, wsn, marr, st)
-                if rc != 0:
-                    L.check(rc, "dvf_conv2d_dgrad")
+                rc = L.ERR_UNSUPPORTED
+                if roles is not None and 2 in roles:
+                    accarr = (ctypes.c_int * g.nseg)(*[(1 if ACCUMULATE_FUSED else 2) if r == 2 else 0 for r in roles])
+                    rc = lib.dvf_conv2d_dgrad_acc(g.dref, dprep, pp, weight.data_ptr(), ginarr, g.segarr, g.nseg, wsp, wsn, marr,
+                                                  accarr, st)
+                    if rc == 0:
+                        ACC_STATS["accumulated"] += roles.count(2)
+                    elif rc == L.ERR_UNSUPPORTED:
+                        ACC_STATS["fallbacks"] += 1
+                        for i, r in enumerate(roles):
+                            if r == 2:
+                                roles[i], gins[i] = 0, torch.empty_like(inputs[i])
+                                ctx.in_tags[i].park = (tid, st, None)
+                        ginarr = (ctypes.c_void_p * g.nseg)(*[t.data_ptr() if t is not None else None for t in gins])
+                    else:
+                        L.check(rc, "dvf_conv2d_dgrad_acc")
+                if rc == L.ERR_UNSUPPORTED:
+                    rc = lib.dvf_conv2d_dgrad(g.dref, dprep, pp, weight.data_ptr(), ginarr, g.segarr, g.nseg, wsp, wsn, marr, st)
+                    if rc != 0:
+                        L.check(rc, "dvf_conv2d_dgrad")
             if L.PLAN_LOG is not None:
                 L.note_plans("dgrad")
+            if roles is not None:
+                for i, r in enumerate(roles):
+                    if r == 1:
+                        ctx.in_tags[i].park = (tid, st, gins[i])
+                    elif r == 2:
+                        gins[i] = None
         dw = None
         if fused_out and need_b and not need_w:
             _bias_sums(lib, dpre, None, None, dbias, N, cout, oh * ow, L.ACT_NONE, 1.0, 0.0, acc_b)
diff --git a/depth-vo-feat_amd/dvf/lib.py b/depth-vo-feat_amd/dvf/lib.py
--- a/depth-vo-feat_amd/dvf/lib.py
+++ b/depth-vo-feat_amd/dvf/lib.py
@@ -70,6 +70,7 @@
     "dvf_smooth_loss_bwd": (c_i, [c_fp] * 3 + [c_i] * 3 + [c_f, c_fp]),
     "dvf_conv2d_fwd": (c_i, [c_desc, c_pp, c_ip, c_i] + [c_fp] * 5 + [c_i64, c_fp]),
     "dvf_conv2d_dgrad": (c_i, [c_desc, c_fp, c_fp, c_fp, c_pp, c_ip, c_i, c_fp, c_i64, c_pp, c_fp]),
+    "dvf_conv2d_dgrad_acc": (c_i, [c_desc, c_fp, c_fp, c_fp, c_pp, c_ip, c_i, c_fp, c_i64, c_pp, c_ip, c_fp]),
     "dvf_conv2d_wgrad": (c_i, [c_desc, c_pp, c_ip, c_i, c_fp, c_fp, c_i, c_fp, c_i, c_fp, c_i64, c_fp]),
     "dvf_conv2d_wgrad_ws_floats": (c_i64, [c_desc, c_ip, c_i]),
     "dvf_conv2d_packed_floats": (c_i64, [c_desc, c_ip, c_i, c_i]),
diff --git a/include/dvf_hip.h b/include/dvf_hip.h
--- a/include/dvf_hip.h
+++ b/include/dvf_hip.h
@@ -123,6 +123,9 @@
 int dvf_conv2d_dgrad(const dvf_conv_desc *d, const float *dpre, const float *packed, const float *w, float *const *din_segs,
                      const int *seg_channels, int nseg, float *ws, int64_t ws_floats, const float *const *mask_segs,
                      void *stream);
+int dvf_conv2d_dgrad_acc(const dvf_conv_desc *d, const float *dpre, const float *packed, const float *w, float *const *din_segs,
+                         const int *seg_channels, int nseg, float *ws, int64_t ws_floats, const float *const *mask_segs,
+                         const int *acc_segs, void *stream);
 int64_t dvf_conv2d_wgrad_ws_floats(const dvf_conv_desc *d, const int *seg_channels, int nseg);
 int dvf_conv2d_wgrad(const dvf_conv_desc *d, const float *const *in_segs, const int *seg_channels, int nseg,
                      const float *dpre, float *dw, int accumulate, float *dbias, int accumulate_dbias, float *ws,
```
